# rkhosrowshahi/MO-VAE

Hardware: AMD Instinct MI355X
Metric: training images/sec (higher is better)
Workload: dtype f32

## Files before the change

include/movae.h:

```cpp
#ifndef MOVAE_H
#define MOVAE_H

#include <stddef.h>
#include <stdint.h>

#ifdef __cplusplus
extern "C" {
#endif

typedef void* movae_stream_t;

enum movae_act { MOVAE_ACT_NONE = 0, MOVAE_ACT_LRELU = 1, MOVAE_ACT_RELU = 2, MOVAE_ACT_TANH = 3, MOVAE_ACT_SIGMOID = 4 };
enum movae_recon { MOVAE_RECON_MSE = 0, MOVAE_RECON_BCE = 1, MOVAE_RECON_L1 = 2, MOVAE_RECON_SMOOTH_L1 = 3 };
enum movae_mgda_norm { MOVAE_MGDA_NONE = 0, MOVAE_MGDA_L2 = 1, MOVAE_MGDA_LOSS = 2, MOVAE_MGDA_LOSS_PLUS = 3 };
enum movae_upgrad_norm { MOVAE_UPGRAD_TRACE = 0, MOVAE_UPGRAD_MIN_L2 = 1, MOVAE_UPGRAD_COSINE = 2 };
enum movae_amtl_scale { MOVAE_AMTL_MIN = 0, MOVAE_AMTL_MEDIAN = 1, MOVAE_AMTL_RMSE = 2 };

int movae_version(void);
const char* movae_last_error(void);

int movae_nchw_to_nhwc(const float* src, float* dst, int n, int c, int h, int w, movae_stream_t stream);
int movae_nhwc_to_nchw(const float* src, float* dst, int n, int c, int h, int w, movae_stream_t stream);

int movae_conv2d_fwd(const float* x, const float* w, const float* bias, float* y,
                     int n, int hi, int wi, int ci, int ho, int wo, int co, int kh, int kw, int stride, int pad,
                     int act, float slope, void* ws, size_t ws_bytes, movae_stream_t stream);
int movae_conv2d_dgrad(const float* dy, const float* w, float* dx,
                       int n, int hi, int wi, int ci, int ho, int wo, int co, int kh, int kw, int stride, int pad,
                       void* ws, size_t ws_bytes, movae_stream_t stream);
int movae_conv2d_wgrad(const float* dy, const float* x, float* dw, float* dbias,
                       int n, int hi, int wi, int ci, int ho, int wo, int co, int kh, int kw, int stride, int pad,
                       int accumulate, void* ws, size_t ws_bytes, movae_stream_t stream);
int movae_conv2d_wgrad_grouped(int groups, const float* dy, const float* x, float* const* dw, float* const* dbias,
                               int n, int hi, int wi, int ci, int ho, int wo, int co, int kh, int kw, int stride, int pad,
                               int accumulate, void* ws, size_t ws_bytes, movae_stream_t stream);
int movae_convT2d_fwd(const float* x, const float* w, const float* bias, float* y,
                      int n, int hi, int wi, int ci, int ho, int wo, int co, int kh, int kw, int stride, int pad,
                      int act, float slope, void* ws, size_t ws_bytes, movae_stream_t stream);
int movae_convT2d_dgrad(const float* dy, const float* w, float* dx,
                        int n, int hi, int wi, int ci, int ho, int wo, int co, int kh, int kw, int stride, int pad,
                        void* ws, size_t ws_bytes, movae_stream_t stream);
int movae_convT2d_wgrad(const float* dy, const float* x, float* dw, float* dbias,
                        int n, int hi, int wi, int ci, int ho, int wo, int co, int kh, int kw, int stride, int pad,
                        int accumulate, void* ws, size_t ws_bytes, movae_stream_t stream);
int movae_conv2d_dgrad_wgrad_grouped(int groups, const float* dy, const float* w, const float* x, float* dx, float* const* dw,
                                     float* const* dbias, int n, int hi, int wi, int ci, int ho, int wo, int co, int kh, int kw,
                                     int stride, int pad, int accumulate, void* ws, size_t ws_bytes, movae_stream_t stream);
int movae_convT2d_dgrad_wgrad_grouped(int groups, const float* dy, const float* w, const float* x, float* dx, float* const* dw,
                                      float* const* dbias, int n, int hi, int wi, int ci, int ho, int wo, int co, int kh, int kw,
                                      int stride, int pad, int accumulate, void* ws, size_t ws_bytes, movae_stream_t stream);
int movae_convT2d_wgrad_grouped(int groups, const float* dy, const float* x, float* const* dw, float* const* dbias,
                                int n, int hi, int wi, int ci, int ho, int wo, int co, int kh, int kw, int stride, int pad,
                                int accumulate, void* ws, size_t ws_bytes, movae_stream_t stream);
int movae_linear_pair_fwd(const float* x, const float* w1, const float* b1, const float* w2, const float* b2, float* y1, float* y2,
                          int m, int n, int k, movae_stream_t stream);
int movae_linear_pair_bwd(int groups, const float* dy1, const float* dy2, const float* w1, const float* w2, const float* x, float* dx,
                          float* const* dw1, float* const* dw2, float* const* db1, float* const* db2, int m, int n, int k,
                          movae_stream_t stream);

size_t movae_bn_ws_bytes(int rows, int c);
int movae_bn_act_fwd(const float* y, const float* gamma, const float* beta, float* out,
                     float* save_mean, float* save_rstd, float* running_mean, float* running_var,
                     long long* num_batches_tracked,
                     int rows, int c, float eps, float momentum, int training, int act, float slope,
                     void* ws, size_t ws_bytes, movae_stream_t stream);
int movae_bn_act_bwd(const float* dout, const float* y, const float* gamma, const float* beta,
                     const float* save_mean, const float* save_rstd, float* dy, float* dgamma, float* dbeta,
                     int rows, int c, int act, float slope, int accumulate,
                     void* ws, size_t ws_bytes, movae_stream_t stream);

int movae_bn_act_bwd_grouped(int groups, const float* dout, const float* y, const float* gamma, const float* beta,
                             const float* save_mean, const float* save_rstd, float* dy,
                             float* const* dgamma, float* const* dbeta,
                             int rows, int c, int act, float slope, int accumulate,
                             void* ws, size_t ws_bytes, movae_stream_t stream);

int movae_act_fwd(const float* x, float* y, size_t n, int act, float slope, movae_stream_t stream);
int movae_act_bwd(const float* dy, const float* out, float* dx, size_t n, int act, float slope, movae_stream_t stream);
int movae_act_bwd_bias_grouped(int groups, const float* dy, const float* out, float* dpre, float* const* dbias,
                               int rows, int c, int act, float slope, int accumulate,
                               void* ws, size_t ws_bytes, movae_stream_t stream);
int movae_add(const float* a, const float* b, float* y, size_t n, movae_stream_t stream);
int movae_axpby(float alpha, const float* a, float beta, const float* b, float* y, size_t n, movae_stream_t stream);
int movae_copy_channels(const float* src, float* dst, int rows, int c_src, int c_dst, int src_off, int dst_off, int c_copy, movae_stream_t stream);
int movae_colsum(const float* x, float* out, int rows, int c, int accumulate, void* ws, size_t ws_bytes, movae_stream_t stream);

int movae_reparam_fwd(const float* mu, const float* log_var, const float* eps, float* z, size_t n, movae_stream_t stream);
int movae_reparam_rng_fwd(const float* mu, const float* log_var, float* eps, float* z, size_t n, unsigned long long* state, int advance,
                          movae_stream_t stream);
int movae_reparam_prior_rng_fwd(const float* mu, const float* log_var, float* eps, float* z, size_t n, float* prior, size_t n_prior,
                                unsigned long long* state, int advance, movae_stream_t stream);
int movae_reparam_bwd(const float* dz, const float* log_var, const float* eps, float* dmu, float* dlog_var, size_t n, movae_stream_t stream);

size_t movae_reduce_ws_bytes(size_t n);
int movae_recon_loss_fwd(const float* recons, const float* inputs, float* out, size_t n, int kind, float scale,
                         void* ws, size_t ws_bytes, movae_stream_t stream);
int movae_recon_loss_bwd(const float* recons, const float* inputs, const float* gscale_dev, float* drecons,
                         size_t n, int kind, float scale, movae_stream_t stream);
int movae_recon_loss_bwd_act(const float* recons, const float* inputs, const float* gscale_dev, float* dpre, size_t n, int kind,
                             float scale, int act, float slope, movae_stream_t stream);
int movae_kl_fwd(const float* mu, const float* log_var, float* out, int b, int d, float scale,
                 void* ws, size_t ws_bytes, movae_stream_t stream);
int movae_combine_losses_fwd(int nterms, const float* const* terms, int nout, const float* coef, float* iter_dev, float anneal_steps,
                             int anneal_row, int training, float* out, float* anneal_out, movae_stream_t stream);
int movae_combine_losses_bwd(int nterms, int nout, const float* const* g, const float* coef, const float* anneal_dev, int anneal_row,
                             float* gterms, movae_stream_t stream);
int movae_vae_losses_fwd(const float* recons, const float* inputs, size_t n, int kind, float rec_scale,
                         const float* mu, const float* log_var, int b, int d, float kl_scale, float* out,
                         void* ws, size_t ws_bytes, movae_stream_t stream);
int movae_recursive_losses_fwd(const float* recons, const float* inputs, size_t n, int kind, const float* mu_hat, const float* log_var_hat,
                               const float* z_prior, const float* mu_gen, int b, int d, float w_rec, float w_kl, float w_cyc,
                               float* iter_dev, float anneal_host, float anneal_steps, int training, float* out, float* anneal_out,
                               void* ws, size_t ws_bytes, movae_stream_t stream);
int movae_recursive_losses_bwd(const float* recons, const float* inputs, size_t n, int kind, const float* mu_hat, const float* log_var_hat,
                               const float* z_prior, const float* mu_gen, int b, int d, float w_rec, float w_kl, float w_cyc,
                               const float* anneal_dev, const float* g_rec, const float* g_kl, const float* g_cyc, const float* g_tot,
                               float* drecons, float* dmu_hat, float* dlog_var_hat, float* dmu_gen, movae_stream_t stream);
int movae_sphere_latents_fwd(const float* z, float* e, float* u, const float* sigma_in, int sigma_rows, float sigma_val, int fixed_sigma,
                             unsigned long long* state, int advance, int b, int l, float angle_max_deg, float mix_prob, float mix_min_deg,
                             float mix_max_deg, float radius, float eps, float* v, float* v_noisy, float* v_noisy_small, float* sigma,
                             float* sigma_sub, float* inv_rms, movae_stream_t stream);
int movae_sphere_latents_bwd(const float* v, const float* e, const float* sigma, const float* sigma_sub, const float* inv_rms,
                             const float* g_v, const float* g_noisy, const float* g_small, float* dz, int b, int l, float radius,
                             movae_stream_t stream);
size_t movae_sphere_losses_ws_bytes(size_t n, int b);
int movae_sphere_losses_fwd(const float* recons, const float* inputs, const float* x_noisy, const float* recons_sg, size_t n, const float* v,
                            const float* v_enc_dec, int b, int l, float lam_rec, float w_rec_sl1, float lam_con, float w_con_sl1,
                            float lam_lat, float* out, void* ws, size_t ws_bytes, movae_stream_t stream);
int movae_sphere_losses_bwd(const float* recons, const float* inputs, const float* x_noisy, const float* recons_sg, size_t n, const float* v,
                            const float* v_enc_dec, int b, int l, float lam_rec, float w_rec_sl1, float lam_con, float w_con_sl1,
                            float lam_lat, const float* g_rec, const float* g_con, const float* g_lat, const float* g_tot, float* drecons,
                            float* dx_noisy, float* dv, float* dv_enc_dec, movae_stream_t stream);
int movae_kl_bwd(const float* mu, const float* log_var, const float* gscale_dev, float* dmu, float* dlog_var,
                 int b, int d, float scale, movae_stream_t stream);
int movae_tc_decomp_fwd(const float* z, const float* mu, const float* log_var, const float* log_iw, float* out,
                        float* lse_joint, float* lse_marg, int b, int d, void* ws, size_t ws_bytes, movae_stream_t stream);
int movae_tc_decomp_bwd(const float* z, const float* mu, const float* log_var, const float* log_iw,
                        const float* lse_joint, const float* lse_marg, const float* g,
                        float* dz, float* dmu, float* dlog_var, int b, int d, movae_stream_t stream);

enum movae_edge_match {
    MOVAE_EDGE_MAG = 0, MOVAE_EDGE_SIGNED_MSE = 1, MOVAE_EDGE_MAXNORM = 2, MOVAE_EDGE_ANGLE = 3, MOVAE_EDGE_MASKED = 4,
    MOVAE_EDGE_COSINE = 5
};
int movae_edge_weights(const float* inputs, float* w_raw, float* wmax, int n, int h, int w, int c,
                       void* ws, size_t ws_bytes, movae_stream_t stream);
int movae_edge_weighted_mse_fwd(const float* recons, const float* inputs, const float* w_raw, const float* wmax, float* out,
                                int n, int h, int w, int c, float scale, void* ws, size_t ws_bytes, movae_stream_t stream);
int movae_edge_weighted_mse_bwd(const float* recons, const float* inputs, const float* w_raw, const float* wmax,
                                const float* gscale_dev, float* drecons, int n, int h, int w, int c, float scale,
                                movae_stream_t stream);
int movae_edge_match_fwd(const float* recons, const float* inputs, float* out, int n, int h, int w, int c, float scale,
                         int mode, float* stats, void* ws, size_t ws_bytes, movae_stream_t stream);
int movae_edge_match_bwd(const float* recons, const float* inputs, const float* gscale_dev, float* drecons, float* tmp_a,
                         float* tmp_b, int n, int h, int w, int c, float scale, int mode, const float* stats,
                         movae_stream_t stream);

int movae_vq_nearest_fwd(const float* x, const float* e, float* q, int64_t* idx, float* sse, int32_t* used_count,
                         int rows, int k, int d, void* ws, size_t ws_bytes, movae_stream_t stream);
int movae_vq_nearest_fwd_mse(const float* x, const float* e, float* q, int64_t* idx, float* sse, int32_t* used_count, float* mse2,
                             int rows, int k, int d, void* ws, size_t ws_bytes, movae_stream_t stream);
size_t movae_vq_bwd_ws_bytes(int rows, int k, int d);
int movae_vq_bwd(const float* x, const float* q, const int64_t* idx, const float* dq, const float* gc, const float* ge,
                 float* dx, float* de, int rows, int k, int d, void* ws, size_t ws_bytes, movae_stream_t stream);

#define MOVAE_MAX_K 8
size_t movae_gram_ws_bytes(int k, size_t m);
int movae_gram(const float* J, size_t ldj, int k, size_t m, float* G, void* ws, size_t ws_bytes, movae_stream_t stream);
int movae_weights_upgrad(const float* G, int k, float norm_eps, float reg_eps, const float* pref, float* w, movae_stream_t stream);
int movae_weights_upgrad_norm(const float* G, int k, int norm_mode, float norm_eps, float reg_eps, const float* pref, float* w,
                              movae_stream_t stream);
int movae_gram_upgrad(const float* J, size_t ldj, int k, size_t m, float* G, int norm_mode, float norm_eps, float reg_eps,
                      const float* pref, float* w, int dual, void* ws, size_t ws_bytes, movae_stream_t stream);
int movae_weights_mgda(const float* G, int k, int norm, const float* losses, float epsilon, int max_iters,
                       float* w, int32_t* info, movae_stream_t stream);
int movae_weights_mgda_stable(const float* G, int k, int norm, const float* losses, float epsilon, int max_iters,
                              float min_eigenvalue, float* w, int32_t* info, movae_stream_t stream);
int movae_weights_amtl(const float* G, int k, int scale_mode, const float* pref, float* w, movae_stream_t stream);
int movae_weights_dualproj(const float* G, int k, float norm_eps, float reg_eps, const float* pref, float* w, movae_stream_t stream);
int movae_weights_pcgrad(const float* G, int k, const int32_t* perm, float* w, movae_stream_t stream);
int movae_weights_imtlg(const float* G, int k, float* w, movae_stream_t stream);
int movae_weights_cagrad(const float* G, int k, float c, float norm_eps, float* w, movae_stream_t stream);
int movae_weights_const(int k, float value, float* w, movae_stream_t stream);
int movae_combine(const float* J, size_t ldj, int k, size_t m, const float* w, float* g, int accumulate, movae_stream_t stream);
int movae_gd_similarity(const float* J, size_t ldj, int k, size_t m, const float* w, float* out,
                        void* ws, size_t ws_bytes, movae_stream_t stream);

int movae_adam_step(float* p, const float* g, float* m, float* v, size_t n, float lr, float beta1, float beta2,
                    float eps, float weight_decay, int decoupled_wd, int step, movae_stream_t stream);
int movae_adam_multi(int n_tensors, float* const* p, const float* const* g, float* const* m, float* const* v,
                     const size_t* numel, float lr, float beta1, float beta2, float eps, float weight_decay,
                     int decoupled_wd, int step, float* hyper_dev, movae_stream_t stream);
int movae_clip_grad_norm_multi(int n_tensors, float* const* g, const size_t* numel, float max_norm, float* total_sumsq_dev,
                               void* ws, size_t ws_bytes, movae_stream_t stream);
int movae_sumsq(const float* x, size_t n, float* out, void* ws, size_t ws_bytes, movae_stream_t stream);
int movae_scale_by_clip(float* g, size_t n, const float* sumsq_dev, float max_norm, movae_stream_t stream);

#define MOVAE_DTYPE_F32 0
#define MOVAE_DTYPE_BF16 1
int movae_set_compute_dtype(int dtype);

int movae_reduce_defer(int on);
int movae_reduce_flush(void);
int movae_reduce_defer_stats(long long* out3, int reset);
long long movae_reduce_defer_max_bytes(long long bytes);

int movae_bench_main_kernel_only(int on);
const char* movae_bench_last_kernel(void);
int movae_bench_force_split(int s);
int movae_bench_kgemm_bn_fin(int mode);
int movae_bench_force_kgemm(int mode);
int movae_bench_big_tile_min(int n);

typedef struct movae_fuse {
    const float* in_scale;
    const float* in_shift;
    float in_slope;
    float* stats;
    size_t stats_cap;
    int stats_parts;
    const float* bn_y;
    const float* bn_scale;
    const float* bn_shift;
    float bn_slope;
    float* bn_part;
    size_t bn_cap;
    int bn_ppg;
    const float* ep_act_y;
    int ep_act;
    float ep_slope;
    int ep_act_done;
    const float* ep_res;
    const float* fin_gamma;
    const float* fin_beta;
    float fin_eps;
    float fin_momentum;
    float* fin_out;
    float* fin_running_mean;
    float* fin_running_var;
    long long* fin_nbt;
    int fin_done;
} movae_fuse_t;
int movae_conv2d_fwd_f(const float* x, const float* w, const float* bias, float* y,
                       int n, int hi, int wi, int ci, int ho, int wo, int co, int kh, int kw, int stride, int pad,
                       int act, float slope, void* ws, size_t ws_bytes, movae_stream_t stream, movae_fuse_t* fuse);
int movae_convT2d_fwd_f(const float* x, const float* w, const float* bias, float* y,
                        int n, int hi, int wi, int ci, int ho, int wo, int co, int kh, int kw, int stride, int pad,
                        int act, float slope, void* ws, size_t ws_bytes, movae_stream_t stream, movae_fuse_t* fuse);
int movae_conv2d_wgrad_grouped_f(int groups, const float* dy, const float* x, float* const* dw, float* const* dbias,
                                 int n, int hi, int wi, int ci, int ho, int wo, int co, int kh, int kw, int stride, int pad,
                                 int accumulate, void* ws, size_t ws_bytes, movae_stream_t stream, const movae_fuse_t* fuse);
int movae_convT2d_wgrad_grouped_f(int groups, const float* dy, const float* x, float* const* dw, float* const* dbias,
                                  int n, int hi, int wi, int ci, int ho, int wo, int co, int kh, int kw, int stride, int pad,
                                  int accumulate, void* ws, size_t ws_bytes, movae_stream_t stream, const movae_fuse_t* fuse);
int movae_conv2d_dgrad_wgrad_grouped_f(int groups, const float* dy, const float* w, const float* x, float* dx,
                                       float* const* dw, float* const* dbias,
                                       int n, int hi, int wi, int ci, int ho, int wo, int co, int kh, int kw, int stride, int pad,
                                       int accumulate, void* ws, size_t ws_bytes, movae_stream_t stream, const movae_fuse_t* fuse);
int movae_convT2d_dgrad_wgrad_grouped_f(int groups, const float* dy, const float* w, const float* x, float* dx,
                                        float* const* dw, float* const* dbias,
                                        int n, int hi, int wi, int ci, int ho, int wo, int co, int kh, int kw, int stride, int pad,
                                        int accumulate, void* ws, size_t ws_bytes, movae_stream_t stream, const movae_fuse_t* fuse);
int movae_conv2d_dgrad_f(const float* dy, const float* w, float* dx,
                         int n, int hi, int wi, int ci, int ho, int wo, int co, int kh, int kw, int stride, int pad,
                         void* ws, size_t ws_bytes, movae_stream_t stream, movae_fuse_t* fuse, int groups);
int movae_convT2d_dgrad_f(const float* dy, const float* w, float* dx,
                          int n, int hi, int wi, int ci, int ho, int wo, int co, int kh, int kw, int stride, int pad,
                          void* ws, size_t ws_bytes, movae_stream_t stream, movae_fuse_t* fuse, int groups);
int movae_bn_bwd_finalize(const float* bn_part, size_t bn_cap, int ppg, int groups, int rows, int c, const float* gamma,
                          const float* save_mean, const float* save_rstd, float* const* dgamma, float* const* dbeta, float* coef,
                          int accumulate, movae_stream_t stream);
int movae_bn_bwd_apply(const float* dout, const float* y, const float* scale, const float* shift, float slope, const float* coef,
                       float* dy, int groups, size_t rows, int c, movae_stream_t stream);
int movae_bn_bwd_finalize_apply(const float* bn_part, size_t bn_cap, int ppg, int groups, size_t rows, int c, const float* gamma,
                                const float* save_mean, const float* save_rstd, float* const* dgamma, float* const* dbeta, float* coef,
                                int accumulate, const float* dout, const float* y, const float* scale, const float* shift, float slope,
                                float* dy, movae_stream_t stream);
int movae_bn_finalize(const float* stats, size_t stats_cap, int parts, int rows, int c, const float* gamma, const float* beta, float eps,
                      float momentum, float* save_mean, float* save_rstd, float* scale, float* shift, float* running_mean,
                      float* running_var, long long* num_batches_tracked, movae_stream_t stream);
int movae_bn_stats(const float* y, int rows, int c, float* stats, size_t stats_cap, int* parts_out, movae_stream_t stream);
int movae_scale_shift_act(const float* y, const float* scale, const float* shift, float* out, size_t rows, int c, float slope,
                          movae_stream_t stream);

int movae_embedding_fwd(const float* weight, const int64_t* idx, float* y, size_t rows, int k, int d, movae_stream_t stream);
int movae_embedding_bwd(const float* dy, const int64_t* idx, float* dweight, int rows, int k, int d,
                        void* ws, size_t ws_bytes, movae_stream_t stream);
int movae_gated_residual_fwd(const float* res, const float* gate, const float* feat, float* out, size_t n, movae_stream_t stream);
int movae_gated_residual_bwd(const float* dout, const float* gate, const float* feat, float* dgate, float* dfeat, size_t n,
                             movae_stream_t stream);
int movae_mul(const float* a, const float* b, float* y, size_t n, movae_stream_t stream);
size_t movae_cross_entropy_ws_bytes(size_t rows);
int movae_cross_entropy_fwd(const float* logits, const int64_t* target, float* loss, float* lse, size_t rows, int k,
                            void* ws, size_t ws_bytes, movae_stream_t stream);
int movae_cross_entropy_bwd(const float* logits, const int64_t* target, const float* lse, const float* gscale_dev, float* dlogits,
                            size_t rows, int k, movae_stream_t stream);

int movae_causal_attn_fwd(const float* q, const float* k, const float* v, long ld, float* out, float* lse, int B, int heads, int L,
                          int hd, float p, unsigned long long seed, unsigned long long draw, movae_stream_t stream);
size_t movae_causal_attn_ws_bytes(int B, int heads, int L);
int movae_causal_attn_bwd(const float* q, const float* k, const float* v, long ld, const float* out, const float* dout, const float* lse,
                          float* dq, float* dk, float* dv, int B, int heads, int L, int hd, float p, unsigned long long seed,
                          unsigned long long draw, void* ws, size_t ws_bytes, movae_stream_t stream);
int movae_causal_attn_dropout_mask(uint8_t* keep, int BH, int L, float p, unsigned long long seed, unsigned long long draw,
                                   movae_stream_t stream);

int movae_attn_fwd(const float* q, const float* k, const float* v, long ld, const float* rope_cos, const float* rope_sin, float* out,
                   float* lse, int B, int heads, int L, int hd, float p, movae_stream_t stream);
size_t movae_attn_ws_bytes(int B, int heads, int L);
int movae_attn_bwd(const float* q, const float* k, const float* v, long ld, const float* rope_cos, const float* rope_sin, const float* out,
                   const float* dout, const float* lse, float* dq, float* dk, float* dv, int B, int heads, int L, int hd, float p, void* ws,
                   size_t ws_bytes, movae_stream_t stream);

int movae_rownorm_fwd(const float* x, const float* weight, const float* bias, const float* pos, int pos_rows, float* out, float* mean,
                      float* rstd, long rows, int d, int mode, float eps, movae_stream_t stream);
size_t movae_rownorm_ws_bytes(long rows, int d);
int movae_rownorm_bwd(const float* dy, const float* x, const float* weight, const float* mean, const float* rstd, float* dx, float* dweight,
                      float* dbias, long rows, int d, int mode, void* ws, size_t ws_bytes, movae_stream_t stream);
int movae_bias_gelu_fwd(const float* x, const float* bias, float* y, long rows, int c, movae_stream_t stream);
int movae_bias_gelu_bwd(const float* dy, const float* x, const float* bias, float* dx, long rows, int c, movae_stream_t stream);
int movae_unpatchify_act_fwd(const float* x, float* out, int b, int h, int w, int c, int patch, movae_stream_t stream);
int movae_unpatchify_act_bwd(const float* dout, const float* out, float* dx, int b, int h, int w, int c, int patch, movae_stream_t stream);
int movae_add_rows_bcast(const float* x, const float* pos, float* y, long rows, int pos_rows, int d, movae_stream_t stream);

size_t movae_recon_metrics_ws_bytes(int n, int c, int h, int w);
int movae_recon_metrics(const float* real, long long rs_n, long long rs_c, long long rs_h, long long rs_w,
                        const float* recon, long long ps_n, long long ps_c, long long ps_h, long long ps_w,
                        int n, int c, int h, int w, int window_size, float max_val, float* out, void* ws, size_t ws_bytes,
                        movae_stream_t stream);

size_t movae_vgg_prep_ws_bytes(int g);
int movae_vgg_prep_fwd(int g, const float* const* x, float* const* y, int* flags, size_t n, void* ws, size_t ws_bytes,
                       movae_stream_t stream);
int movae_vgg_prep_bwd(int g, const float* const* dy, const float* const* x, const int* flags, float* const* dx, size_t n,
                       movae_stream_t stream);
int movae_maxpool2x2_fwd(const float* x, float* y, int n, int h, int w, int c, movae_stream_t stream);
int movae_maxpool2x2_bwd(const float* dy, const float* x, const float* y, float* dx, int n, int h, int w, int c, movae_stream_t stream);

size_t movae_lpips_ws_bytes(int n, int h, int w, int c);
int movae_lpips_layer(const float* f1, const float* f2, int n, int h, int w, int c, float scale, double* partials,
                      size_t partials_bytes, movae_stream_t stream);
int movae_lpips_finalize(int layers, const double* const* partials, const int* h, const int* w, const int* c, int n, float* out,
                         movae_stream_t stream);

int movae_batch_u8(const uint8_t* store, const int* idx, int b, int h, int w, int c, const float* lut, int flip,
// ... 7 lines not shown
```

mo-vae_amd/_lib.py:

```python
import ctypes as C
import os
import threading

import torch

HERE = os.path.dirname(os.path.abspath(__file__))
LIB_PATH = os.path.join(HERE, "libmovae_hip.so")

ACT = {"none": 0, None: 0, "lrelu": 1, "relu": 2, "tanh": 3, "sigmoid": 4}
RECON = {"mse": 0, "bce": 1, "l1": 2, "smooth_l1": 3}
UPGRAD_NORM = {"trace": 0, "min_l2": 1, "cosine": 2}
EDGE_MATCH = {"mag": 0, "signed_mse": 1, "maxnorm": 2, "angle": 3, "masked": 4, "cosine": 5}
MGDA_NORM = {"none": 0, "l2": 1, "loss": 2, "loss+": 3}
AMTL_SCALE = {"min": 0, "median": 1, "rmse": 2}
MAX_K = 8

_p, _i, _f, _z, _l = C.c_void_p, C.c_int, C.c_float, C.c_size_t, C.c_long

class MovaeFuse(C.Structure):
    _fields_ = [("in_scale", C.c_void_p), ("in_shift", C.c_void_p), ("in_slope", C.c_float), ("stats", C.c_void_p),
                ("stats_cap", C.c_size_t), ("stats_parts", C.c_int),
                ("bn_y", C.c_void_p), ("bn_scale", C.c_void_p), ("bn_shift", C.c_void_p), ("bn_slope", C.c_float), ("bn_part", C.c_void_p),
                ("bn_cap", C.c_size_t), ("bn_ppg", C.c_int),
                ("ep_act_y", C.c_void_p), ("ep_act", C.c_int), ("ep_slope", C.c_float), ("ep_act_done", C.c_int),
                ("ep_res", C.c_void_p),
                ("fin_gamma", C.c_void_p), ("fin_beta", C.c_void_p), ("fin_eps", C.c_float), ("fin_momentum", C.c_float),
                ("fin_out", C.c_void_p), ("fin_running_mean", C.c_void_p), ("fin_running_var", C.c_void_p), ("fin_nbt", C.c_void_p),
                ("fin_done", C.c_int)]


_conv_fwd = [_p, _p, _p, _p] + [_i] * 11 + [_i, _f, _p, _z, _p]
_conv_dgrad = [_p, _p, _p] + [_i] * 11 + [_p, _z, _p]
_conv_wgrad = [_p, _p, _p, _p] + [_i] * 11 + [_i, _p, _z, _p]

SIGNATURES = {
    "movae_version": ([], _i),
    "movae_last_error": ([], C.c_char_p),
    "movae_nchw_to_nhwc": ([_p, _p, _i, _i, _i, _i, _p], _i),
    "movae_nhwc_to_nchw": ([_p, _p, _i, _i, _i, _i, _p], _i),
    "movae_conv2d_fwd": (_conv_fwd, _i),
    "movae_conv2d_dgrad": (_conv_dgrad, _i),
    "movae_conv2d_wgrad": (_conv_wgrad, _i),
    "movae_convT2d_fwd": (_conv_fwd, _i),
    "movae_convT2d_dgrad": (_conv_dgrad, _i),
    "movae_convT2d_wgrad": (_conv_wgrad, _i),
    "movae_conv2d_wgrad_grouped": ([_i] + _conv_wgrad, _i),
    "movae_convT2d_wgrad_grouped": ([_i] + _conv_wgrad, _i),
    "movae_conv2d_dgrad_wgrad_grouped": ([_i, _p, _p, _p, _p, _p, _p] + [_i] * 11 + [_i, _p, _z, _p], _i),
    "movae_convT2d_dgrad_wgrad_grouped": ([_i, _p, _p, _p, _p, _p, _p] + [_i] * 11 + [_i, _p, _z, _p], _i),
    "movae_bn_ws_bytes": ([_i, _i], _z),
    "movae_bn_act_fwd": ([_p] * 9 + [_i, _i, _f, _f, _i, _i, _f, _p, _z, _p], _i),
    "movae_bn_act_bwd": ([_p] * 9 + [_i, _i, _i, _f, _i, _p, _z, _p], _i),
    "movae_bn_act_bwd_grouped": ([_i] + [_p] * 9 + [_i, _i, _i, _f, _i, _p, _z, _p], _i),
    "movae_act_fwd": ([_p, _p, _z, _i, _f, _p], _i),
    "movae_act_bwd": ([_p, _p, _p, _z, _i, _f, _p], _i),
    "movae_act_bwd_bias_grouped": ([_i, _p, _p, _p, _p, _i, _i, _i, _f, _i, _p, _z, _p], _i),
    "movae_add": ([_p, _p, _p, _z, _p], _i),
    "movae_axpby": ([_f, _p, _f, _p, _p, _z, _p], _i),
    "movae_copy_channels": ([_p, _p, _i, _i, _i, _i, _i, _i, _p], _i),
    "movae_colsum": ([_p, _p, _i, _i, _i, _p, _z, _p], _i),
    "movae_reparam_fwd": ([_p, _p, _p, _p, _z, _p], _i),
    "movae_reparam_rng_fwd": ([_p, _p, _p, _p, _z, _p, _i, _p], _i),
    "movae_reparam_bwd": ([_p, _p, _p, _p, _p, _z, _p], _i),
    "movae_reparam_prior_rng_fwd": ([_p, _p, _p, _p, _z, _p, _z, _p, _i, _p], _i),
    "movae_reduce_ws_bytes": ([_z], _z),
    "movae_recon_loss_fwd": ([_p, _p, _p, _z, _i, _f, _p, _z, _p], _i),
    "movae_recon_loss_bwd": ([_p, _p, _p, _p, _z, _i, _f, _p], _i),
    "movae_recon_loss_bwd_act": ([_p, _p, _p, _p, _z, _i, _f, _i, _f, _p], _i),
    "movae_kl_fwd": ([_p, _p, _p, _i, _i, _f, _p, _z, _p], _i),
    "movae_combine_losses_fwd": ([_i, _p, _i, _p, _p, _f, _i, _i, _p, _p, _p], _i),
    "movae_combine_losses_bwd": ([_i, _i, _p, _p, _p, _i, _p, _p], _i),
    "movae_vae_losses_fwd": ([_p, _p, _z, _i, _f, _p, _p, _i, _i, _f, _p, _p, _z, _p], _i),
    "movae_kl_bwd": ([_p, _p, _p, _p, _p, _i, _i, _f, _p], _i),
    "movae_recursive_losses_fwd": ([_p, _p, _z, _i, _p, _p, _p, _p, _i, _i, _f, _f, _f, _p, _f, _f, _i, _p, _p, _p, _z, _p], _i),
    "movae_recursive_losses_bwd": ([_p, _p, _z, _i, _p, _p, _p, _p, _i, _i, _f, _f, _f] + [_p] * 9 + [_p], _i),
    "movae_sphere_latents_fwd": ([_p, _p, _p, _p, _i, _f, _i, _p, _i, _i, _i, _f, _f, _f, _f, _f, _f] + [_p] * 6 + [_p], _i),
    "movae_sphere_latents_bwd": ([_p] * 9 + [_i, _i, _f, _p], _i),
    "movae_sphere_losses_ws_bytes": ([_z, _i], _z),
    "movae_sphere_losses_fwd": ([_p, _p, _p, _p, _z, _p, _p, _i, _i, _f, _f, _f, _f, _f, _p, _p, _z, _p], _i),
    "movae_sphere_losses_bwd": ([_p, _p, _p, _p, _z, _p, _p, _i, _i, _f, _f, _f, _f, _f] + [_p] * 8 + [_p], _i),
    "movae_tc_decomp_fwd": ([_p] * 7 + [_i, _i, _p, _z, _p], _i),
    "movae_tc_decomp_bwd": ([_p] * 10 + [_i, _i, _p], _i),
    "movae_edge_weights": ([_p, _p, _p, _i, _i, _i, _i, _p, _z, _p], _i),
    "movae_edge_weighted_mse_fwd": ([_p, _p, _p, _p, _p, _i, _i, _i, _i, _f, _p, _z, _p], _i),
    "movae_edge_weighted_mse_bwd": ([_p, _p, _p, _p, _p, _p, _i, _i, _i, _i, _f, _p], _i),
    "movae_edge_match_fwd": ([_p, _p, _p, _i, _i, _i, _i, _f, _i, _p, _p, _z, _p], _i),
    "movae_edge_match_bwd": ([_p, _p, _p, _p, _p, _p, _i, _i, _i, _i, _f, _i, _p, _p], _i),
    "movae_vq_nearest_fwd": ([_p] * 6 + [_i, _i, _i, _p, _z, _p], _i),
    "movae_vq_nearest_fwd_mse": ([_p] * 7 + [_i, _i, _i, _p, _z, _p], _i),
    "movae_vq_bwd_ws_bytes": ([_i, _i, _i], _z),
    "movae_vq_bwd": ([_p] * 8 + [_i, _i, _i, _p, _z, _p], _i),
    "movae_gram_ws_bytes": ([_i, _z], _z),
    "movae_gram": ([_p, _z, _i, _z, _p, _p, _z, _p], _i),
    "movae_weights_upgrad": ([_p, _i, _f, _f, _p, _p, _p], _i),
    "movae_weights_upgrad_norm": ([_p, _i, _i, _f, _f, _p, _p, _p], _i),
    "movae_gram_upgrad": ([_p, _z, _i, _z, _p, _i, _f, _f, _p, _p, _i, _p, _z, _p], _i),
    "movae_weights_mgda": ([_p, _i, _i, _p, _f, _i, _p, _p, _p], _i),
    "movae_weights_mgda_stable": ([_p, _i, _i, _p, _f, _i, _f, _p, _p, _p], _i),
    "movae_weights_amtl": ([_p, _i, _i, _p, _p, _p], _i),
    "movae_weights_dualproj": ([_p, _i, _f, _f, _p, _p, _p], _i),
    "movae_weights_pcgrad": ([_p, _i, _p, _p, _p], _i),
    "movae_weights_imtlg": ([_p, _i, _p, _p], _i),
    "movae_weights_cagrad": ([_p, _i, _f, _f, _p, _p], _i),
    "movae_weights_const": ([_i, _f, _p, _p], _i),
    "movae_combine": ([_p, _z, _i, _z, _p, _p, _i, _p], _i),
    "movae_gd_similarity": ([_p, _z, _i, _z, _p, _p, _p, _z, _p], _i),
    "movae_adam_step": ([_p, _p, _p, _p, _z, _f, _f, _f, _f, _f, _i, _i, _p], _i),
    "movae_adam_multi": ([_i, _p, _p, _p, _p, _p, _f, _f, _f, _f, _f, _i, _i, _p, _p], _i),
    "movae_clip_grad_norm_multi": ([_i, _p, _p, _f, _p, _p, _z, _p], _i),
    "movae_sumsq": ([_p, _z, _p, _p, _z, _p], _i),
    "movae_scale_by_clip": ([_p, _z, _p, _f, _p], _i),
    "movae_conv2d_fwd_f": (_conv_fwd + [_p], _i),
    "movae_convT2d_fwd_f": (_conv_fwd + [_p], _i),
    "movae_conv2d_wgrad_grouped_f": ([_i] + _conv_wgrad + [_p], _i),
    "movae_convT2d_wgrad_grouped_f": ([_i] + _conv_wgrad + [_p], _i),
    "movae_conv2d_dgrad_wgrad_grouped_f": ([_i, _p, _p, _p, _p, _p, _p] + [_i] * 11 + [_i, _p, _z, _p, _p], _i),
    "movae_convT2d_dgrad_wgrad_grouped_f": ([_i, _p, _p, _p, _p, _p, _p] + [_i] * 11 + [_i, _p, _z, _p, _p], _i),
    "movae_conv2d_dgrad_f": (_conv_dgrad + [_p, _i], _i),
    "movae_convT2d_dgrad_f": (_conv_dgrad + [_p, _i], _i),
    "movae_bn_bwd_finalize": ([_p, _z, _i, _i, _i, _i, _p, _p, _p, _p, _p, _p, _i, _p], _i),
    "movae_bn_bwd_apply": ([_p, _p, _p, _p, _f, _p, _p, _i, _z, _i, _p], _i),
    "movae_linear_pair_fwd": ([_p, _p, _p, _p, _p, _p, _p, _i, _i, _i, _p], _i),
    "movae_linear_pair_bwd": ([_i, _p, _p, _p, _p, _p, _p, _p, _p, _p, _p, _i, _i, _i, _p], _i),
    "movae_bn_bwd_finalize_apply": ([_p, _z, _i, _i, _z, _i, _p, _p, _p, _p, _p, _p, _i, _p, _p, _p, _p, _f, _p, _p], _i),
    "movae_bn_finalize": ([_p, _z, _i, _i, _i, _p, _p, _f, _f, _p, _p, _p, _p, _p, _p, _p, _p], _i),
    "movae_bn_stats": ([_p, _i, _i, _p, _z, _p, _p], _i),
    "movae_scale_shift_act": ([_p, _p, _p, _p, _z, _i, _f, _p], _i),
    "movae_embedding_fwd": ([_p, _p, _p, _z, _i, _i, _p], _i),
    "movae_embedding_bwd": ([_p, _p, _p, _i, _i, _i, _p, _z, _p], _i),
    "movae_gated_residual_fwd": ([_p, _p, _p, _p, _z, _p], _i),
    "movae_gated_residual_bwd": ([_p, _p, _p, _p, _p, _z, _p], _i),
    "movae_mul": ([_p, _p, _p, _z, _p], _i),
    "movae_cross_entropy_ws_bytes": ([_z], _z),
    "movae_cross_entropy_fwd": ([_p, _p, _p, _p, _z, _i, _p, _z, _p], _i),
    "movae_cross_entropy_bwd": ([_p, _p, _p, _p, _p, _z, _i, _p], _i),
    "movae_causal_attn_fwd": ([_p, _p, _p, _l, _p, _p, _i, _i, _i, _i, _f, C.c_ulonglong, C.c_ulonglong, _p], _i),
    "movae_causal_attn_ws_bytes": ([_i, _i, _i], _z),
    "movae_causal_attn_bwd": ([_p, _p, _p, _l, _p, _p, _p, _p, _p, _p, _i, _i, _i, _i, _f, C.c_ulonglong, C.c_ulonglong, _p, _z, _p], _i),
    "movae_causal_attn_dropout_mask": ([_p, _i, _i, _f, C.c_ulonglong, C.c_ulonglong, _p], _i),
    "movae_attn_fwd": ([_p, _p, _p, _l, _p, _p, _p, _p, _i, _i, _i, _i, _f, _p], _i),
    "movae_attn_ws_bytes": ([_i, _i, _i], _z),
    "movae_attn_bwd": ([_p, _p, _p, _l, _p, _p, _p, _p, _p, _p, _p, _p, _i, _i, _i, _i, _f, _p, _z, _p], _i),
    "movae_rownorm_fwd": ([_p, _p, _p, _p, _i, _p, _p, _p, _l, _i, _i, _f, _p], _i),
    "movae_rownorm_ws_bytes": ([_l, _i], _z),
    "movae_rownorm_bwd": ([_p, _p, _p, _p, _p, _p, _p, _p, _l, _i, _i, _p, _z, _p], _i),
    "movae_bias_gelu_fwd": ([_p, _p, _p, _l, _i, _p], _i),
    "movae_bias_gelu_bwd": ([_p, _p, _p, _p, _l, _i, _p], _i),
    "movae_unpatchify_act_fwd": ([_p, _p, _i, _i, _i, _i, _i, _p], _i),
    "movae_unpatchify_act_bwd": ([_p, _p, _p, _i, _i, _i, _i, _i, _p], _i),
    "movae_add_rows_bcast": ([_p, _p, _p, _l, _i, _i, _p], _i),
    "movae_vgg_prep_ws_bytes": ([_i], _z),
    "movae_vgg_prep_fwd": ([_i, _p, _p, _p, _z, _p, _z, _p], _i),
    "movae_vgg_prep_bwd": ([_i, _p, _p, _p, _p, _z, _p], _i),
    "movae_maxpool2x2_fwd": ([_p, _p, _i, _i, _i, _i, _p], _i),
    "movae_maxpool2x2_bwd": ([_p, _p, _p, _p, _i, _i, _i, _i, _p], _i),
    "movae_recon_metrics_ws_bytes": ([_i, _i, _i, _i], _z),
    "movae_recon_metrics": ([_p, C.c_longlong, C.c_longlong, C.c_longlong, C.c_longlong, _p, C.c_longlong, C.c_longlong, C.c_longlong,
                             C.c_longlong, _i, _i, _i, _i, _i, _f, _p, _p, _z, _p], _i),
    "movae_lpips_ws_bytes": ([_i, _i, _i, _i], _z),
    "movae_lpips_layer": ([_p, _p, _i, _i, _i, _i, _f, _p, _z, _p], _i),
    "movae_lpips_finalize": ([_i, _p, _p, _p, _p, _i, _p, _p], _i),
    "movae_batch_u8": ([_p, _p, _i, _i, _i, _i, _p, _i, C.c_ulonglong, C.c_ulonglong, _p, _p], _i),
    "movae_bench_main_kernel_only": ([_i], _i),
    "movae_bench_last_kernel": ([], C.c_char_p),
    "movae_reduce_defer": ([_i], _i),
    "movae_reduce_flush": ([], _i),
    "movae_reduce_defer_stats": ([_p, _i], _i),
    "movae_reduce_defer_max_bytes": ([C.c_longlong], C.c_longlong),
    "movae_bench_force_split": ([_i], _i),
    "movae_bench_kgemm_bn_fin": ([_i], _i),
    "movae_bench_force_kgemm": ([_i], _i),
    "movae_bench_big_tile_min": ([_i], _i),
    "movae_set_compute_dtype": ([_i], _i),
}

_lib = None
_lock = threading.Lock()


def load():
    global _lib
    if _lib is not None:
        return _lib
    with _lock:
        if _lib is not None:
            return _lib
        from . import build as _build

        have_hipcc = False
        try:
            _build._hipcc()
            have_hipcc = os.path.isdir(_build.CSRC)
        except RuntimeError:
            pass
        if have_hipcc and os.environ.get("MOVAE_NO_REBUILD") != "1":
            try:
                _build.build(verbose=False)
            except Exception as e:
                if not os.path.exists(LIB_PATH):
                    raise RuntimeError(
                        f"libmovae_hip.so is missing at {LIB_PATH} and could not be built ({e}); "
                        "the MI355X kernels are required -- there is no CPU fallback") from e
                raise RuntimeError(f"csrc/ changed but rebuilding libmovae_hip.so failed: {e}") from e
        elif not os.path.exists(LIB_PATH):
            raise RuntimeError(f"libmovae_hip.so is missing at {LIB_PATH} and hipcc is not available to build it; "
                               "the MI355X kernels are required -- there is no CPU fallback")
        try:
            lib = C.CDLL(LIB_PATH)
        except OSError as e:
            raise RuntimeError(f"cannot load {LIB_PATH}: {e}; the MI355X kernels are required") from e
        for name, (args, res) in SIGNATURES.items():
            fn = getattr(lib, name)
            fn.argtypes = args
            fn.restype = res
        _lib = lib
    return _lib


DTYPES = {"fp32": 0, "f32": 0, "float32": 0, "bf16": 1, "bfloat16": 1}


def set_compute_dtype(name):
    if name not in DTYPES:
        raise ValueError(f"compute dtype must be one of {sorted(set(DTYPES))}, got {name!r}")
    prev = load().movae_set_compute_dtype(DTYPES[name])
    return "bf16" if prev == 1 else "fp32"


def compute_dtype():
    lib = load()
    prev = lib.movae_set_compute_dtype(DTYPES["fp32"])
    lib.movae_set_compute_dtype(prev)
    return "bf16" if prev == 1 else "fp32"


TRACE = None

DEFER_ON = [False]
DEFER_PASS = frozenset(
    [f"movae_conv{t}2d_{k}" for t in ("", "T") for k in ("dgrad", "dgrad_f", "wgrad_grouped", "wgrad_grouped_f", "dgrad_wgrad_grouped",
                                                       "dgrad_wgrad_grouped_f")] +
    ["movae_bn_bwd_finalize", "movae_bn_bwd_apply", "movae_bn_bwd_finalize_apply", "movae_bn_act_bwd", "movae_bn_act_bwd_grouped",
     "movae_act_bwd", "movae_act_bwd_bias_grouped", "movae_colsum", "movae_add", "movae_axpby", "movae_copy_channels", "movae_mul",
     "movae_nchw_to_nhwc", "movae_nhwc_to_nchw", "movae_reparam_bwd", "movae_kl_bwd", "movae_recon_loss_bwd", "movae_recon_loss_bwd_act", "movae_recursive_losses_bwd",
     "movae_tc_decomp_bwd", "movae_sphere_latents_bwd", "movae_sphere_losses_bwd",
     "movae_combine_losses_bwd", "movae_vq_bwd", "movae_linear_pair_bwd", "movae_edge_weighted_mse_bwd", "movae_edge_match_bwd",
     "movae_gated_residual_bwd", "movae_attn_bwd", "movae_rownorm_bwd", "movae_bias_gelu_bwd", "movae_unpatchify_act_bwd",
     "movae_vgg_prep_bwd", "movae_maxpool2x2_bwd"])
_defer_arena = [0]


def defer_arm(device):
    _defer_arena[0] ^= 1
    w = workspace(device, slot=2 + _defer_arena[0])
    load().movae_reduce_defer(1)
    return w.data_ptr(), w.numel()


def defer_flush():
    if _lib is not None:
        check(load().movae_reduce_flush(), "movae_reduce_flush")
# ... 49 lines not shown
```

mo-vae_amd/aggregation.py:

```python
import os

import torch
import torch.nn as tnn

from . import _lib as L


def _st(t):
    return L.stream_ptr(t.device)


def _check_matrix(J):
    if J.dim() != 2:
        raise ValueError(f"Parameter `matrix` should be a tensor of dimension 2. Found `matrix.shape = {tuple(J.shape)}`.")
    if J.shape[0] > L.MAX_K:
        raise ValueError(f"at most {L.MAX_K} objectives are supported on device, got {J.shape[0]}")
    L.require_gpu(J)
    if J.dtype != torch.float32 or J.stride(1) != 1:
        raise ValueError("the Jacobian must be fp32 with unit column stride")


FUSE_GRAM = os.environ.get("MOVAE_FUSE_GRAM", "1") != "0"


def compute_gramian(J):
    _check_matrix(J)
    k, m = J.shape
    G = torch.empty((k, k), dtype=torch.float32, device=J.device)
    ws = L.workspace(J.device)
    L.call("movae_gram", J.data_ptr(), J.stride(0) if k > 1 else max(J.stride(0), m), k, m, G.data_ptr(),
                                ws.data_ptr(), ws.numel(), _st(J))
    return G


def combine(J, w):
    _check_matrix(J)
    k, m = J.shape
    g = torch.empty(m, dtype=torch.float32, device=J.device)
    L.call("movae_combine", J.data_ptr(), J.stride(0) if k > 1 else max(J.stride(0), m), k, m, w.data_ptr(),
                                   g.data_ptr(), 0, _st(J))
    return g


def gd_similarity(J, w):
    _check_matrix(J)
    k, m = J.shape
    out = torch.empty((), dtype=torch.float32, device=J.device)
    ws = L.workspace(J.device)
    L.call("movae_gd_similarity", J.data_ptr(), J.stride(0) if k > 1 else max(J.stride(0), m), k, m, w.data_ptr(),
                                         out.data_ptr(), ws.data_ptr(), ws.numel(), _st(J))
    return out


def _pref_tensor(pref, device):
    if pref is None:
        return None
    return torch.as_tensor(pref, dtype=torch.float32).to(device).contiguous()


class Weighting(tnn.Module):

    def forward(self, gramian):
        raise NotImplementedError


class _FromJacobian(tnn.Module):

    def __init__(self, gramian_weighting):
        super().__init__()
        self.gramian_weighting = gramian_weighting

    def forward(self, J):
        gw = self.gramian_weighting
        fused = getattr(gw, "from_jacobian", None)
        if fused is not None and FUSE_GRAM and not gw._forward_hooks and not gw._forward_pre_hooks:
            self.last_gramian, w = fused(J)
            return w
        self.last_gramian = compute_gramian(J)
        return gw(self.last_gramian)


class GramianWeightedAggregator(tnn.Module):
    def __init__(self, gramian_weighting):
        super().__init__()
        self.gramian_weighting = gramian_weighting
        self.weighting = _FromJacobian(gramian_weighting)

    def forward(self, J):
        w = self.weighting(J)
        return combine(J, w)


class UPGradWeighting(Weighting):

    def __init__(self, pref_vector=None, norm_eps=1e-4, reg_eps=1e-4, norm="trace"):
        super().__init__()
        self.pref_vector, self.norm_eps, self.reg_eps, self.norm = pref_vector, norm_eps, reg_eps, norm

    def _mode(self):
        return self.norm

    def forward(self, G):
        k = G.shape[0]
        w = torch.empty(k, dtype=torch.float32, device=G.device)
        pref = _pref_tensor(self.pref_vector, G.device)
        L.call("movae_weights_upgrad_norm", G.data_ptr(), k, L.UPGRAD_NORM[self._mode()], float(self.norm_eps),
               float(self.reg_eps), L.ptr(pref), w.data_ptr(), _st(G))
        return w

    def from_jacobian(self, J):
        _check_matrix(J)
        k, m = J.shape
        G = torch.empty((k, k), dtype=torch.float32, device=J.device)
        w = torch.empty(k, dtype=torch.float32, device=J.device)
        pref = _pref_tensor(self.pref_vector, J.device)
        ws = L.workspace(J.device)
        L.call("movae_gram_upgrad", J.data_ptr(), J.stride(0) if k > 1 else max(J.stride(0), m), k, m, G.data_ptr(),
               L.UPGRAD_NORM[self._mode()], float(self.norm_eps), float(self.reg_eps), L.ptr(pref), w.data_ptr(), 0, ws.data_ptr(),
               ws.numel(), _st(J))
        return G, w


class _PNUPGradWeighting(UPGradWeighting):

    def __init__(self, pref_vector=None, prob=0.5, norm_eps=1e-4, reg_eps=1e-4):
        super().__init__(pref_vector, norm_eps, reg_eps, norm="min_l2")
        self.prob = prob

    def _mode(self):
        return "cosine" if torch.rand(1).item() < self.prob else "min_l2"


class UPGrad(GramianWeightedAggregator):

    def __init__(self, pref_vector=None, norm_eps=0.0001, reg_eps=0.0001, solver="quadprog"):
        super().__init__(UPGradWeighting(pref_vector, norm_eps, reg_eps))
        self._pref_vector, self._norm_eps, self._reg_eps = pref_vector, norm_eps, reg_eps

    def __repr__(self):
        return f"UPGrad(pref_vector={self._pref_vector!r}, norm_eps={self._norm_eps}, reg_eps={self._reg_eps})"


class NUPGrad(GramianWeightedAggregator):

    def __init__(self, pref_vector=None, norm_eps=0.0001, reg_eps=0.0001, solver="quadprog"):
        super().__init__(UPGradWeighting(pref_vector, norm_eps, reg_eps, norm="min_l2"))
        self._pref_vector, self._norm_eps, self._reg_eps = pref_vector, norm_eps, reg_eps

    def __repr__(self):
        return f"NUPGrad(pref_vector={self._pref_vector!r}, norm_eps={self._norm_eps}, reg_eps={self._reg_eps}, solver='quadprog')"


class PNUPGrad(GramianWeightedAggregator):

    def __init__(self, pref_vector=None, prob=0.5, norm_eps=0.0001, reg_eps=0.0001, solver="quadprog"):
        super().__init__(_PNUPGradWeighting(pref_vector, prob, norm_eps, reg_eps))
        self._pref_vector, self._prob, self._norm_eps, self._reg_eps = pref_vector, prob, norm_eps, reg_eps

    def __repr__(self):
        return (f"PNUPGrad(pref_vector={self._pref_vector!r}, prob={self._prob}, norm_eps={self._norm_eps}, "
                f"reg_eps={self._reg_eps}, solver='quadprog')")


class MGDAWeighting(Weighting):
    def __init__(self, norm_type="none", epsilon=1e-5, max_iters=250, stable=False, min_eigenvalue_eps=1e-10):
        super().__init__()
        if norm_type not in ("none", "l2", "loss", "loss+"):
            raise ValueError("Parameter `norm_type` should be 'none', 'l2', 'loss', or 'loss+'. Found "
                             f"`norm_type = {norm_type!r}`.")
        self.norm_type, self.epsilon, self.max_iters = norm_type, epsilon, max_iters
        self.stable, self.min_eigenvalue_eps = stable, min_eigenvalue_eps
        self._losses = None
        self._info = None

    def set_losses(self, losses):
        if losses.dim() != 1:
            raise ValueError(f"Parameter `losses` should be a 1D tensor. Found `losses.shape = {losses.shape}`.")
        self._losses = losses.detach()

    @property
    def convergence_count(self):
        return None if self._info is None else int(self._info.item())

    def forward(self, G):
        k = G.shape[0]
        losses = None
        if self.norm_type in ("loss", "loss+"):
            if self._losses is None:
                raise RuntimeError(f"Losses must be set before calling forward() when using norm_type='{self.norm_type}'. "
                                   "Call set_losses() first.")
            if self._losses.shape[0] != k:
                raise ValueError(f"Number of losses ({self._losses.shape[0]}) must match the number of rows in the gramian ({k}).")
            losses = self._losses.to(device=G.device, dtype=torch.float32).contiguous()
        w = torch.empty(k, dtype=torch.float32, device=G.device)
        self._info = torch.empty(1, dtype=torch.int32, device=G.device)
        if self.stable:
            L.call("movae_weights_mgda_stable", G.data_ptr(), k, L.MGDA_NORM[self.norm_type], L.ptr(losses), float(self.epsilon),
                   int(self.max_iters), float(self.min_eigenvalue_eps), w.data_ptr(), self._info.data_ptr(), _st(G))
        else:
            L.call("movae_weights_mgda", G.data_ptr(), k, L.MGDA_NORM[self.norm_type], L.ptr(losses), float(self.epsilon),
                   int(self.max_iters), w.data_ptr(), self._info.data_ptr(), _st(G))
        return w


class StableMGDA(GramianWeightedAggregator):

    def __init__(self, norm_type="none", epsilon=1e-5, max_iters=250, min_eigenvalue_eps=1e-10):
        w = MGDAWeighting(norm_type, epsilon, max_iters, True, min_eigenvalue_eps)
        super().__init__(w)
        self._mgda_weighting = w

    @property
    def mgda_weighting(self):
        return self._mgda_weighting

    def set_losses(self, losses):
        self._mgda_weighting.set_losses(losses)


class MGDA(GramianWeightedAggregator):
    def __init__(self, norm_type="none", epsilon=1e-5, max_iters=250, stable=False, min_eigenvalue_eps=1e-10):
        w = MGDAWeighting(norm_type, epsilon, max_iters, stable, min_eigenvalue_eps)
        super().__init__(w)
        self._mgda_weighting = w
        self._norm_type, self._epsilon, self._max_iters, self._stable = norm_type, epsilon, max_iters, stable

    @property
    def mgda_weighting(self):
        return self._mgda_weighting

    def set_losses(self, losses):
        self._mgda_weighting.set_losses(losses)

    def __repr__(self):
        return (f"MGDA(norm_type={self._norm_type!r}, epsilon={self._epsilon}, max_iters={self._max_iters}, "
                f"stable={self._stable})")


class AlignedMTLWeighting(Weighting):
    def __init__(self, pref_vector=None, scale_mode="min"):
        super().__init__()
        self._pref_vector, self._scale_mode = pref_vector, scale_mode

# ... 220 lines not shown
```

mo-vae_amd/autojac.py:

```python
import os

import torch

from . import ops

BATCHED_VJP = os.environ.get("MOVAE_BATCHED_VJP", "1") != "0"


def _leaf_tensors(roots, excluded=()):
    stop = {t.grad_fn for t in excluded if t.grad_fn is not None}
    seen, leaves, stack = set(), [], [t.grad_fn for t in roots if t.grad_fn is not None]
    while stack:
        fn = stack.pop()
        if fn is None or fn in seen or fn in stop:
            continue
        seen.add(fn)
        var = getattr(fn, "variable", None)
        if var is not None:
            if var.requires_grad:
                leaves.append(var)
            continue
        stack.extend(nf for nf, _ in fn.next_functions)
    out, ids = [], set()
    for v in leaves:
# ... 110 lines not shown
                self.copied.add(dst.data_ptr())
                if g.data_ptr() != dst.data_ptr():
                    dst.copy_(_mem_flat(g))


def _group(t, g):
    return None if t is None else t[g]


def _dense(t):
    if t.is_contiguous():
        return True
    order = sorted(range(t.dim()), key=lambda i: (-t.stride(i), -t.shape[i]))
    return t.permute(order).is_contiguous()


def _restack(lst):
    t0 = lst[0]
    if not isinstance(t0, torch.Tensor) or t0.numel() == 0 or not _dense(t0):
        return lst
    nbytes = t0.numel() * t0.element_size()
    base = t0.untyped_storage().data_ptr()
    for g, t in enumerate(lst):
        if (not isinstance(t, torch.Tensor) or t.shape != t0.shape or t.dtype != t0.dtype or t.stride() != t0.stride() or
                t.untyped_storage().data_ptr() != base or t.data_ptr() != t0.data_ptr() + g * nbytes):
            return lst
    return t0.as_strided((len(lst),) + tuple(t0.shape), (t0.numel(),) + tuple(t0.stride()), t0.storage_offset())


def _accumulate_stacked(a, b, G):
    if a is None:
        return b
    if isinstance(a, (list, tuple)) or isinstance(b, (list, tuple)):
        return [a[g] + b[g] for g in range(G)]
    return a + b


def _expected_shape(node, input_nr):
    var = getattr(node, "variable", None)
    if var is not None:
        return tuple(var.shape)
    meta = getattr(node, "_input_metadata", None)
    if meta is not None and input_nr < len(meta):
        return tuple(meta[input_nr].shape)
    return None


def _fit_groups(t, shape, G):
    if shape is None:
        return t
    if isinstance(t, (list, tuple)):
        return [x if x is None or tuple(x.shape) == shape else x.sum_to_size(shape) for x in t]
    if tuple(t.shape[1:]) == shape:
        return t
    return [t[g].sum_to_size(shape) for g in range(G)]


@torch.no_grad()
def _batched_pullback(features, feat_grads, rows, jb):
    G = len(rows)
    roots = []
    for f, feat in enumerate(features):
        fn = feat.grad_fn
        if fn is None:
            continue
        gs = [feat_grads[g][f] for g in range(G)]
        if all(x is None for x in gs):
            continue
        ref = next(x for x in gs if x is not None)
        gs = [x if x is not None else torch.zeros_like(ref) for x in gs]
        roots.append((fn, feat.output_nr, _restack(gs)))
    deps, seen, stack = {}, set(), [fn for fn, _, _ in roots]
    while stack:
        fn = stack.pop()
        if fn in seen:
            continue
        seen.add(fn)
        for nf, _ in fn.next_functions:
            if nf is not None:
                deps[nf] = deps.get(nf, 0) + 1
                stack.append(nf)
    pending = {}
    for fn, nr, gs in roots:
        slot = pending.setdefault(fn, {})
        slot[nr] = _accumulate_stacked(slot.get(nr), gs, G)
    ready = [fn for fn in {r[0] for r in roots} if deps.get(fn, 0) == 0]
    col = {id(p): (p, off) for p, off in zip(jb.params, jb.offsets)}
    ops.GRAD_SINK_ROWS = [jb.sinks(r) for r in rows]
    try:
        while ready:
            fn = ready.pop()
            got = pending.pop(fn, {})
            var = getattr(fn, "variable", None)
            outs = None
            if var is not None:
                ent = col.get(id(var))
                if ent is not None and 0 in got:
                    p, off = ent
                    for g in range(G):
                        src = _group(got[0], g)
                        dst = jb.buf[rows[g]][off: off + p.numel()]
                        jb.copied.add(dst.data_ptr())
                        if src.data_ptr() != dst.data_ptr():
                            dst.copy_(_mem_flat(src))
                continue
            edges = list(fn.next_functions)
            if got:
                n_in = max(got) + 1
                args = [got.get(i) for i in range(n_in)]
                cls = getattr(fn, "_forward_cls", None)
                if cls is not None:
                    args += [None] * (len(getattr(fn, "_input_metadata", ())) - len(args))
                    if hasattr(cls, "backward_batched"):
                        outs = cls.backward_batched(fn, G, *args)
                    else:
                        per = []
                        for g in range(G):
                            r = cls.backward(fn, *[_group(a, g) for a in args])
                            per.append(r if isinstance(r, tuple) else (r,))
                        outs = tuple(None if all(per[g][i] is None for g in range(G)) else [per[g][i] for g in range(G)]
                                     for i in range(len(per[0])))
                    if not isinstance(outs, tuple):
                        outs = (outs,)
                    need = [i for i, nd in enumerate(fn.needs_input_grad) if nd]
                    live = [j for j, (nf, _) in enumerate(edges) if nf is not None]
                    if len(need) != len(live):
                        raise NotImplementedError("cannot align backward outputs with graph edges")
                    aligned = [None] * len(edges)
                    for j, i in zip(live, need):
                        aligned[j] = outs[i] if i < len(outs) else None
                    outs = tuple(aligned)
                else:
                    per = []
                    for g in range(G):
                        r = fn(*[_group(a, g) for a in args])
                        per.append(r if isinstance(r, tuple) else (r,))
                    outs = tuple(None if all(per[g][i] is None for g in range(G)) else _restack([per[g][i] for g in range(G)])
                                 for i in range(len(per[0])))
            for i, (nf, nr) in enumerate(edges):
                if nf is None:
                    continue
                o = outs[i] if outs is not None and i < len(outs) else None
                if o is not None:
                    o = _fit_groups(o, _expected_shape(nf, nr), G)
                    slot = pending.setdefault(nf, {})
                    slot[nr] = _accumulate_stacked(slot.get(nr), o, G)
                deps[nf] -= 1
                if deps[nf] == 0:
                    ready.append(nf)
    finally:
        ops.GRAD_SINK_ROWS = None


def _aggregate_into_grads(jb, aggregator):
    g = aggregator(jb.J)
    for p, off in zip(jb.params, jb.offsets):
        _accumulate(p, _view_like(g[off: off + p.numel()], p))
    return g


class _MtlState:
    __slots__ = ("jb", "feat_diff", "feat_grads", "shared_params", "aggregator", "task_params", "device")


def mtl_backward_begin(losses, features, aggregator, tasks_params=None, shared_params=None):
    losses, features = list(losses), list(features)
    if len(losses) == 0:
        raise ValueError("`losses` cannot be empty")
    if len(features) == 0:
        raise ValueError("`features` cannot be empty.")
    if shared_params is None:
        shared_params = _leaf_tensors(features)
    if tasks_params is None:
        tasks_params = [_leaf_tensors([l], excluded=features) for l in losses]
    if len(tasks_params) != len(losses):
        raise ValueError("`losses` and `tasks_params` should have the same size.")
    st = _MtlState()
    st.shared_params = list(shared_params)
    st.aggregator = aggregator
    st.jb = JacobianBuffer.persistent(st.shared_params, len(losses), features[0].device)
    st.feat_diff = [f for f in features if f.requires_grad]
    st.feat_grads = []
    st.task_params = []
    cot = [torch.empty_strided((len(losses),) + tuple(f.shape), (f.numel(),) + tuple(f.stride()), dtype=f.dtype, device=f.device)
           if _dense(f) else None for f in st.feat_diff]
    for i, (loss, tp) in enumerate(zip(losses, tasks_params)):
        tp = list(tp)
        seed = _ones_like(loss) if loss.dim() == 0 and loss.dtype == torch.float32 else None
        ops.GRAD_ACCUM.clear()
        ops.GRAD_ACCUM_TAKEN.clear()
        if i > 0:
            ops.GRAD_ACCUM.update({p.data_ptr(): p.grad for p in tp if p.grad is not None})
        ops.COT_SINK.clear()
        ops.COT_SINK.update({f.data_ptr(): c[i] for f, c in zip(st.feat_diff, cot) if c is not None})
        ops.GRAD_SINK.clear()
        owned = {}
        for p in tp:
            if p.grad is None:
                buf = ops.GRAD_SINK[p.data_ptr()] = _task_grad_buffer(p)
                owned[buf.data_ptr()] = p
        n_w, n_z = len(ops.SINK_LOG), len(ops.SINK_ZERO_LOG)
        try:
            with ops.deferred_reduces():
                got = torch.autograd.grad(loss, tp + st.feat_diff, grad_outputs=seed, retain_graph=True, allow_unused=True)
        finally:
            for ptr in ops.SINK_LOG[n_w:]:
                if ptr in owned:
                    owned[ptr]._movae_grad_written = True
            for ptr in ops.SINK_ZERO_LOG[n_z:]:
                if ptr in owned and getattr(owned[ptr], "_movae_grad_written", False):
                    owned[ptr]._movae_grad_buf.zero_()
                    owned[ptr]._movae_grad_written = False
            ops.GRAD_SINK.clear()
            ops.COT_SINK.clear()
            ops.GRAD_ACCUM.clear()
            taken = frozenset(ops.GRAD_ACCUM_TAKEN)
            ops.GRAD_ACCUM_TAKEN.clear()
        for p, g in zip(tp, got[: len(tp)]):
            if g is not None:
                _accumulate(p, g, taken)
                st.task_params.append(p)
        st.feat_grads.append(got[len(tp):])
    return st


def _task_grad_buffer(p):
    buf = getattr(p, "_movae_grad_buf", None)
    if buf is None or buf.numel() != p.numel() or buf.device != p.device:
        buf = torch.zeros(p.numel(), dtype=p.dtype, device=p.device)
        p._movae_grad_buf, p._movae_grad_written = buf, False
    return buf


def mtl_backward_finish(st):
    with ops.deferred_reduces():
        return _mtl_backward_finish(st)


def _mtl_backward_finish(st):
    jb, feat_diff, feat_grads, shared_params = st.jb, st.feat_diff, st.feat_grads, st.shared_params
    live_rows = [i for i, gf in enumerate(feat_grads) if any(g is not None for g in gf)]
    batched = BATCHED_VJP and shared_params and len(live_rows) > 1
    if batched:
        try:
            _batched_pullback(feat_diff, [feat_grads[i] for i in live_rows], live_rows, jb)
        except NotImplementedError:
            batched = False
    for i in ([] if batched else live_rows):
        gf = feat_grads[i]
        live = [(f, g) for f, g in zip(feat_diff, gf) if g is not None]
        if not live or not shared_params:
            continue
        ops.GRAD_SINK.clear()
        ops.GRAD_SINK.update(jb.sinks(i))
        try:
            js = torch.autograd.grad([f for f, _ in live], shared_params, grad_outputs=[g for _, g in live],
                                     retain_graph=True, allow_unused=True)
        finally:
            ops.GRAD_SINK.clear()
        jb.write_row(i, js)
    if shared_params:
        jb.settle()
        _aggregate_into_grads(jb, st.aggregator)


def mtl_backward(losses, features, aggregator, tasks_params=None, shared_params=None, retain_graph=False,
                 parallel_chunk_size=None):
    st = mtl_backward_begin(losses, features, aggregator, tasks_params, shared_params)
    mtl_backward_finish(st)
    if not retain_graph:
        del st


def backward(tensors, aggregator, inputs=None, retain_graph=False, parallel_chunk_size=None):
    tensors = list(tensors) if isinstance(tensors, (list, tuple)) else [tensors]
    if len(tensors) == 0:
        raise ValueError("`tensors` cannot be empty")
    if inputs is None:
        inputs = _leaf_tensors(tensors)
    inputs = list(inputs)
    if not inputs:
        return
    jb = JacobianBuffer(inputs, len(tensors), tensors[0].device)
    for i, t in enumerate(tensors):
        js = torch.autograd.grad(t, inputs, retain_graph=True, allow_unused=True)
        jb.write_row(i, js)
    _aggregate_into_grads(jb, aggregator)


BATCHED_FULL_JACOBIAN = os.environ.get("MOVAE_BATCHED_FULL_JACOBIAN", "0") == "1"


def backward_through(tensors, aggregator, inputs=None):
    tensors = list(tensors)
    if len(tensors) == 0:
        raise ValueError("`tensors` cannot be empty")
    if inputs is None:
        inputs = _leaf_tensors(tensors)
    inputs = list(inputs)
    if not inputs:
        return
    K = len(tensors)
    jb = JacobianBuffer(inputs, K, tensors[0].device)
    node = tensors[0].grad_fn
    cls = getattr(node, "_forward_cls", None)
    done = False
    if (BATCHED_FULL_JACOBIAN and BATCHED_VJP and K > 1 and hasattr(cls, "input_cotangents")
# ... 13 lines not shown
```

mo-vae_amd/csrc/agg.hip:

```cpp
#include "common.h"
#include <stdlib.h>

namespace {

constexpr int MAXK = MOVAE_MAX_K;
inline int gram_blocks(size_t m) {
    static const size_t cap = (size_t)env_long("MOVAE_GRAM_BLOCKS", 1024);
    size_t g = (m + 2047) / 2048;
    return (int)(g > cap ? cap : (g < 1 ? 1 : g));
}

template <int K, bool VEC>
__global__ __launch_bounds__(256) void gram_partial(const float* __restrict__ J, long ldj, long m, double* __restrict__ part) {
    constexpr int NP = K * (K + 1) / 2;
    double acc[NP];
#pragma unroll
    for (int q = 0; q < NP; ++q) acc[q] = 0.0;
    const long stride = (long)gridDim.x * blockDim.x;
    if (VEC) {
        const long nv = m / 4;
        for (long c = (long)blockIdx.x * blockDim.x + threadIdx.x; c < nv; c += stride) {
            f32x4 v[K];
#pragma unroll
            for (int i = 0; i < K; ++i) v[i] = reinterpret_cast<const f32x4*>(J + i * ldj)[c];
            int q = 0;
#pragma unroll
            for (int i = 0; i < K; ++i)
#pragma unroll
                for (int j = i; j < K; ++j) {
                    const f32x4 p = v[i] * v[j];
                    acc[q] += (double)p[0] + (double)p[1] + (double)p[2] + (double)p[3];
                    ++q;
                }
        }
        if (blockIdx.x == 0 && threadIdx.x == 0)
            for (long c = nv * 4; c < m; ++c) {
                int q = 0;
                for (int i = 0; i < K; ++i)
                    for (int j = i; j < K; ++j) acc[q++] += (double)(J[i * ldj + c] * J[j * ldj + c]);
            }
    } else {
        for (long c = (long)blockIdx.x * blockDim.x + threadIdx.x; c < m; c += stride) {
            float v[K];
#pragma unroll
            for (int i = 0; i < K; ++i) v[i] = J[i * ldj + c];
            int q = 0;
#pragma unroll
            for (int i = 0; i < K; ++i)
#pragma unroll
                for (int j = i; j < K; ++j) acc[q++] += (double)(v[i] * v[j]);
        }
    }
    __shared__ double sh[4];
#pragma unroll
    for (int q = 0; q < NP; ++q) {
        const double s = block_sum_256(acc[q], sh);
        if (threadIdx.x == 0) part[(long)blockIdx.x * NP + q] = s;
    }
}

__global__ __launch_bounds__(64) void gram_final(const double* __restrict__ part, int nblk, int K, float* __restrict__ G) {
    const int NP = K * (K + 1) / 2;
    const int q = blockIdx.x;
    double s = 0.0;
    for (int b = threadIdx.x; b < nblk; b += 64) s += part[(long)b * NP + q];
    s = wave_sum(s);
    if (threadIdx.x != 0) return;
    int i = 0, rem = q;
    while (rem >= K - i) {
        rem -= K - i;
        ++i;
    }
    const int j = i + rem;
    G[i * K + j] = (float)s;
    G[j * K + i] = (float)s;
}

template <int K, bool VEC>
__global__ __launch_bounds__(256) void combine_k(const float* __restrict__ J, long ldj, long m, const float* __restrict__ w,
                                                 float* __restrict__ g, int accumulate) {
    float wv[K];
#pragma unroll
    for (int i = 0; i < K; ++i) wv[i] = w[i];
    const long stride = (long)gridDim.x * blockDim.x;
    if (VEC) {
        const long nv = m / 4;
        for (long c = (long)blockIdx.x * blockDim.x + threadIdx.x; c < nv; c += stride) {
            f32x4 s = accumulate ? reinterpret_cast<const f32x4*>(g)[c] : f32x4{0.f, 0.f, 0.f, 0.f};
#pragma unroll
            for (int i = 0; i < K; ++i) s += wv[i] * reinterpret_cast<const f32x4*>(J + i * ldj)[c];
            reinterpret_cast<f32x4*>(g)[c] = s;
        }
        if (blockIdx.x == 0 && threadIdx.x == 0)
            for (long c = nv * 4; c < m; ++c) {
                float s = accumulate ? g[c] : 0.f;
                for (int i = 0; i < K; ++i) s += wv[i] * J[i * ldj + c];
                g[c] = s;
            }
    } else {
        for (long c = (long)blockIdx.x * blockDim.x + threadIdx.x; c < m; c += stride) {
            float s = accumulate ? g[c] : 0.f;
#pragma unroll
            for (int i = 0; i < K; ++i) s += wv[i] * J[i * ldj + c];
            g[c] = s;
        }
    }
}

__global__ __launch_bounds__(256) void similarity_partial(const float* __restrict__ J, long ldj, int K, long m,
                                                          const float* __restrict__ w, double* __restrict__ part) {
    __shared__ double sh[4];
    double ab = 0.0, aa = 0.0, bb = 0.0;
    const long stride = (long)gridDim.x * blockDim.x;
    for (long c = (long)blockIdx.x * blockDim.x + threadIdx.x; c < m; c += stride) {
        float a = 0.f, b = 0.f;
        for (int i = 0; i < K; ++i) {
            const float v = J[i * ldj + c];
            a += w[i] * v;
            b += v;
        }
        b /= (float)K;
        ab += (double)a * b;
        aa += (double)a * a;
        bb += (double)b * b;
    }
    ab = block_sum_256(ab, sh);
    aa = block_sum_256(aa, sh);
    bb = block_sum_256(bb, sh);
    if (threadIdx.x == 0) {
        part[blockIdx.x * 3 + 0] = ab;
        part[blockIdx.x * 3 + 1] = aa;
        part[blockIdx.x * 3 + 2] = bb;
    }
}

__global__ void similarity_final(const double* __restrict__ part, int nblk, float* __restrict__ out) {
    if (threadIdx.x != 0) return;
    double ab = 0, aa = 0, bb = 0;
    for (int b = 0; b < nblk; ++b) {
        ab += part[b * 3];
        aa += part[b * 3 + 1];
        bb += part[b * 3 + 2];
    }
    const double na = fmax(sqrt(aa), 1e-8), nb = fmax(sqrt(bb), 1e-8);
    out[0] = (float)(ab / (na * nb));
}

template <int KT>
__global__ __launch_bounds__(64) void upgrad_k(const float* __restrict__ Gptr, int norm_mode, float norm_eps, float reg_eps,
                                               const float* __restrict__ pref, float* __restrict__ wout, int dual,
                                               const double* __restrict__ gpart, int gnb, float* __restrict__ Gout) {
    constexpr int K = KT;
    const int lane = threadIdx.x;
    float Gin[K * K];
    if (gpart) {
        constexpr int NP = K * (K + 1) / 2;
        int q = 0;
#pragma unroll
        for (int i = 0; i < K; ++i)
#pragma unroll
            for (int j = i; j < K; ++j, ++q) {
                double s = 0.0;
                for (int b = lane; b < gnb; b += 64) s += gpart[(long)b * NP + q];
                s = wave_sum(s);
                Gin[i * K + j] = Gin[j * K + i] = (float)s;
            }
        if (lane == 0 && Gout)
#pragma unroll
            for (int i = 0; i < K * K; ++i) Gout[i] = Gin[i];
    } else {
#pragma unroll
        for (int i = 0; i < K * K; ++i) Gin[i] = Gptr[i];
    }
    double G[K][K];
    if (norm_mode == 0) {
        double tr = 0.0;
#pragma unroll
        for (int i = 0; i < K; ++i) tr += (double)Gin[i * K + i];
        const bool zero = tr < (double)norm_eps;
#pragma unroll
        for (int i = 0; i < K; ++i)
#pragma unroll
            for (int j = 0; j < K; ++j) G[i][j] = zero ? 0.0 : (double)Gin[i * K + j] / tr;
    } else {
        float l2[K], sf[K];
        float amin = 0.f;
        bool any = false;
#pragma unroll
        for (int i = 0; i < K; ++i) {
            l2[i] = sqrtf(fmaxf(Gin[i * K + i], norm_eps));
            if (l2[i] > norm_eps && (!any || l2[i] < amin)) {
                amin = l2[i];
                any = true;
            }
        }
#pragma unroll
        for (int i = 0; i < K; ++i) sf[i] = (any && l2[i] > norm_eps) ? amin / l2[i] : 0.f;
#pragma unroll
        for (int i = 0; i < K; ++i)
#pragma unroll
            for (int j = 0; j < K; ++j) {
                const float g = Gin[i * K + j];
                G[i][j] = norm_mode == 1 ? (double)(g * (sf[i] * sf[j])) : (double)(g / (l2[i] * l2[j]));
            }
    }
#pragma unroll
    for (int i = 0; i < K; ++i) G[i][i] += (double)reg_eps;
    double u[K], wsum[K];
#pragma unroll
    for (int i = 0; i < K; ++i) {
        u[i] = pref ? (double)pref[i] : 1.0 / K;
        wsum[i] = 0.0;
    }
    constexpr int nsub = 1 << K;
    for (int row = 0; row < (dual ? 1 : K); ++row) {
        double c[K];
#pragma unroll
        for (int i = 0; i < K; ++i) {
            double acc = 0.0;
#pragma unroll
            for (int j = 0; j < K; ++j) acc += G[i][j] * ((dual || j == row) ? u[j] : 0.0);
            c[i] = acc;
        }
        double best_viol = 1e300;
        int best_mask = 0;
        double best_v[K];
#pragma unroll
        for (int i = 0; i < K; ++i) best_v[i] = 0.0;
        for (int mask = lane; mask < nsub; mask += 64) {
            double L[K][K], y[K], v[K];
            bool ok = true;
#pragma unroll
            for (int a = 0; a < K; ++a) {
                const bool fa = mask >> a & 1;
#pragma unroll
                for (int b = 0; b <= a; ++b) {
                    const bool fb = mask >> b & 1;
                    double s = (fa && fb) ? G[a][b] : (a == b ? 1.0 : 0.0);
#pragma unroll
                    for (int q = 0; q < b; ++q) s -= L[a][q] * L[b][q];
                    if (a == b) {
                        if (s <= 0.0) {
                            ok = false;
                            s = 1.0;
                        }
                        L[a][a] = sqrt(s);
                    } else {
                        L[a][b] = s / L[b][b];
                    }
                }
            }
#pragma unroll
            for (int a = 0; a < K; ++a) {
                double s = (mask >> a & 1) ? -c[a] : 0.0;
#pragma unroll
                for (int q = 0; q < a; ++q) s -= L[a][q] * y[q];
                y[a] = s / L[a][a];
            }
#pragma unroll
            for (int a = K - 1; a >= 0; --a) {
                double s = y[a];
#pragma unroll
                for (int q = a + 1; q < K; ++q) s -= L[q][a] * v[q];
                v[a] = s / L[a][a];
            }
            double viol = ok ? 0.0 : 1e200;
#pragma unroll
            for (int i = 0; i < K; ++i) {
                if (mask >> i & 1) {
                    viol = fmax(viol, -v[i]);
                } else {
                    v[i] = 0.0;
                    double gr = c[i];
#pragma unroll
                    for (int j = 0; j < K; ++j) gr += G[i][j] * ((mask >> j & 1) ? v[j] : 0.0);
                    viol = fmax(viol, -gr);
                }
            }
            if (viol < best_viol) {
                best_viol = viol;
                best_mask = mask;
#pragma unroll
                for (int i = 0; i < K; ++i) best_v[i] = v[i];
            }
        }
        for (int o = 32; o > 0; o >>= 1) {
            const double ov = __shfl_xor(best_viol, o, 64);
            const int om = __shfl_xor(best_mask, o, 64);
            double tmp[K];
#pragma unroll
            for (int i = 0; i < K; ++i) tmp[i] = __shfl_xor(best_v[i], o, 64);
            if (ov < best_viol || (ov == best_viol && om < best_mask)) {
                best_viol = ov;
                best_mask = om;
#pragma unroll
                for (int i = 0; i < K; ++i) best_v[i] = tmp[i];
            }
        }
#pragma unroll
        for (int i = 0; i < K; ++i) wsum[i] += best_v[i] + ((dual || i == row) ? u[i] : 0.0);
    }
    if (lane == 0)
#pragma unroll
        for (int i = 0; i < K; ++i) wout[i] = (float)wsum[i];
}

template <int KT>
__global__ __launch_bounds__(64) void cagrad_k(const float* __restrict__ Gin, float c, float norm_eps, float* __restrict__ wout) {
    constexpr int K = KT;
    const int lane = threadIdx.x;
    double G[K][K], b[K];
    double tr = 0.0, uGu = 0.0;
#pragma unroll
    for (int i = 0; i < K; ++i) {
#pragma unroll
        for (int j = 0; j < K; ++j) {
            G[i][j] = 0.5 * ((double)Gin[i * K + j] + (double)Gin[j * K + i]);
            uGu += G[i][j];
        }
        tr += G[i][i];
    }
    uGu /= (double)K * K;
    const double kappa = (double)c * sqrt(fmax(uGu, 0.0)), jitter = 1e-14 * tr;
#pragma unroll
    for (int i = 0; i < K; ++i) {
        double acc = 0.0;
#pragma unroll
        for (int j = 0; j < K; ++j) acc += G[i][j];
        b[i] = acc / K;
    }
    double best_viol = 1e300;
    int best_mask = 0;
    double best_w[K];
#pragma unroll
    for (int i = 0; i < K; ++i) best_w[i] = 0.0;
    for (int mask = lane + 1; mask < (1 << K); mask += 64) {
        double L[K][K], yp[K], yq[K], p[K], q[K], w[K];
        bool ok = true;
#pragma unroll
        for (int a = 0; a < K; ++a) {
            const bool fa = mask >> a & 1;
#pragma unroll
            for (int bb = 0; bb <= a; ++bb) {
                const bool fb = mask >> bb & 1;
                double s = (fa && fb) ? G[a][bb] + (a == bb ? jitter : 0.0) : (a == bb ? 1.0 : 0.0);
#pragma unroll
                for (int r = 0; r < bb; ++r) s -= L[a][r] * L[bb][r];
                if (a == bb) {
                    if (s <= 0.0) {
                        ok = false;
                        s = 1.0;
                    }
                    L[a][a] = sqrt(s);
                } else {
                    L[a][bb] = s / L[bb][bb];
                }
            }
        }
#pragma unroll
        for (int a = 0; a < K; ++a) {
            const bool fa = mask >> a & 1;
            double sp = fa ? 1.0 : 0.0, sq = fa ? b[a] : 0.0;
#pragma unroll
            for (int r = 0; r < a; ++r) {
                sp -= L[a][r] * yp[r];
                sq -= L[a][r] * yq[r];
            }
            yp[a] = sp / L[a][a];
            yq[a] = sq / L[a][a];
        }
#pragma unroll
        for (int a = K - 1; a >= 0; --a) {
            double sp = yp[a], sq = yq[a];
#pragma unroll
            for (int r = a + 1; r < K; ++r) {
                sp -= L[r][a] * p[r];
                sq -= L[r][a] * q[r];
            }
            p[a] = sp / L[a][a];
            q[a] = sq / L[a][a];
        }
        double A = 0.0, B = 0.0, C = 0.0;
#pragma unroll
        for (int i = 0; i < K; ++i)
            if (mask >> i & 1) {
                A += p[i];
                B += q[i];
                C += b[i] * q[i];
            }
        const double disc = B * B - A * (C - kappa * kappa);
        ok = ok && disc >= 0.0 && A > 0.0;
        const double lam = ok ? (B + sqrt(disc)) / A : 0.0, den = lam * A - B;
        ok = ok && den > 0.0;
#pragma unroll
        for (int i = 0; i < K; ++i) w[i] = (ok && (mask >> i & 1)) ? (lam * p[i] - q[i]) / den : 0.0;
        double Gw[K], wGw = 0.0;
#pragma unroll
        for (int i = 0; i < K; ++i) {
            double acc = 0.0;
#pragma unroll
            for (int j = 0; j < K; ++j) acc += G[i][j] * w[j];
            Gw[i] = acc;
            wGw += w[i] * acc;
        }
        const double t = sqrt(fmax(wGw, 0.0));
        ok = ok && t > 0.0;
        double viol = ok ? 0.0 : 1e200;
        if (ok) {
#pragma unroll
            for (int i = 0; i < K; ++i) {
                if (mask >> i & 1) viol = fmax(viol, -w[i]);
                else viol = fmax(viol, -(b[i] + kappa * Gw[i] / t - lam));
            }
        }
        if (viol < best_viol) {
            best_viol = viol;
            best_mask = mask;
#pragma unroll
            for (int i = 0; i < K; ++i) best_w[i] = w[i];
        }
    }
    for (int o = 32; o > 0; o >>= 1) {
        const double ov = __shfl_xor(best_viol, o, 64);
        const int om = __shfl_xor(best_mask, o, 64);
        double tmp[K];
#pragma unroll
        for (int i = 0; i < K; ++i) tmp[i] = __shfl_xor(best_w[i], o, 64);
        if (ov < best_viol || (ov == best_viol && om < best_mask)) {
            best_viol = ov;
            best_mask = om;
#pragma unroll
            for (int i = 0; i < K; ++i) best_w[i] = tmp[i];
        }
    }
    if (lane == 0) {
        double wGw = 0.0;
#pragma unroll
        for (int i = 0; i < K; ++i)
#pragma unroll
            for (int j = 0; j < K; ++j) wGw += best_w[i] * G[i][j] * best_w[j];
        const double gw = sqrt(fmax(wGw, 0.0));
        const bool mean = kappa <= (double)norm_eps || best_viol >= 1e199 || gw <= (double)norm_eps;
#pragma unroll
        for (int i = 0; i < K; ++i) wout[i] = (float)(mean ? 1.0 / K : 1.0 / K + kappa / gw * best_w[i]);
    }
}

inline void launch_cagrad(const float* G, int k, float c, float norm_eps, float* w, hipStream_t st) {
#define MOVAE_CAG(KV) hipLaunchKernelGGL((cagrad_k<KV>), dim3(1), dim3(64), 0, st, G, c, norm_eps, w)
    switch (k) {
        case 1: MOVAE_CAG(1); break;
        case 2: MOVAE_CAG(2); break;
        case 3: MOVAE_CAG(3); break;
        case 4: MOVAE_CAG(4); break;
// ... 190 lines not shown
int launch_combine_k(const float* J, size_t ldj, size_t m, const float* w, float* g, int acc, bool vec, hipStream_t st) {
    const int nb = gram_blocks(m);
    if (vec)
        hipLaunchKernelGGL((combine_k<K, true>), dim3(nb), dim3(256), 0, st, J, (long)ldj, (long)m, w, g, acc);
    else
        hipLaunchKernelGGL((combine_k<K, false>), dim3(nb), dim3(256), 0, st, J, (long)ldj, (long)m, w, g, acc);
    MOVAE_CHECK_LAUNCH("combine");
    return MOVAE_OK;
}

#define DISPATCH_K(k, CALL)                                      \
    switch (k) {                                                 \
        case 1: return CALL(1);                                  \
        case 2: return CALL(2);                                  \
        case 3: return CALL(3);                                  \
        case 4: return CALL(4);                                  \
        case 5: return CALL(5);                                  \
        case 6: return CALL(6);                                  \
        case 7: return CALL(7);                                  \
        case 8: return CALL(8);                                  \
        default: break;                                          \
    }

__global__ __launch_bounds__(64) void pcgrad_k(const float* __restrict__ G, int K, const int32_t* __restrict__ perm,
                                               float* __restrict__ wout) {
    if (threadIdx.x != 0) return;
    float w[MAXK];
    for (int i = 0; i < K; ++i) w[i] = 0.f;
    for (int i = 0; i < K; ++i) {
        float cur[MAXK];
        for (int q = 0; q < K; ++q) cur[q] = q == i ? 1.f : 0.f;
        for (int t = 0; t < K; ++t) {
            const int j = perm[i * K + t];
            if (j == i || j < 0 || j >= K) continue;
            float ip = 0.f;
            for (int q = 0; q < K; ++q) ip += G[j * K + q] * cur[q];
            if (ip < 0.f) cur[j] -= ip / G[j * K + j];
        }
        for (int q = 0; q < K; ++q) w[q] += cur[q];
    }
    for (int i = 0; i < K; ++i) wout[i] = w[i];
}

__global__ __launch_bounds__(64) void imtlg_k(const float* __restrict__ Gin, int K, float* __restrict__ wout) {
    if (threadIdx.x != 0) return;
    double A[MAXK][MAXK], V[MAXK][MAXK], d[MAXK], v[MAXK];
    for (int i = 0; i < K; ++i)
        for (int j = 0; j < K; ++j) {
            A[i][j] = 0.5 * ((double)Gin[i * K + j] + (double)Gin[j * K + i]);
            V[i][j] = i == j ? 1.0 : 0.0;
        }
    for (int i = 0; i < K; ++i) d[i] = sqrt(fmax((double)Gin[i * K + i], 0.0));
    jacobi_eigh(A, V, K);
    double lmax = 0.0;
    for (int i = 0; i < K; ++i) lmax = fmax(lmax, fabs(A[i][i]));
    const double cut = (double)K * 1.1920928955078125e-07 * lmax;
    for (int i = 0; i < K; ++i) v[i] = 0.0;
    for (int e = 0; e < K; ++e) {
        if (fabs(A[e][e]) <= cut) continue;
        double proj = 0.0;
        for (int i = 0; i < K; ++i) proj += V[i][e] * d[i];
        proj /= A[e][e];
        for (int i = 0; i < K; ++i) v[i] += V[i][e] * proj;
    }
    double sum = 0.0;
    for (int i = 0; i < K; ++i) sum += v[i];
    for (int i = 0; i < K; ++i) wout[i] = fabs(sum) < 1e-12 ? 0.f : (float)(v[i] / sum);
}


}

extern "C" {

size_t movae_gram_ws_bytes(int k, size_t m) {
    if (k <= 0) return 0;
    return MOVAE_WS_HEADER_BYTES + (size_t)gram_blocks(m) * (size_t)(k * (k + 1) / 2) * sizeof(double);
}

int movae_gram(const float* J, size_t ldj, int k, size_t m, float* G, void* ws, size_t ws_bytes, movae_stream_t stream) {
    MOVAE_WS_SCRATCH(ws, ws_bytes);
    MOVAE_CHECK_ARG(J && G && m > 0 && ldj >= m, "movae_gram: bad argument");
    MOVAE_CHECK_ARG(k >= 1 && k <= MAXK, "movae_gram: k=%d outside 1..%d", k, MAXK);
    MOVAE_CHECK_ARG(ws && ws_bytes >= movae_gram_ws_bytes(k, m), "movae_gram: workspace too small");
    hipStream_t st = (hipStream_t)stream;
    double* part = static_cast<double*>(ws);
    const int nb = gram_blocks(m);
    const bool vec = (ldj % 4 == 0) && (reinterpret_cast<uintptr_t>(J) & 15) == 0;
    int rc = MOVAE_EINVAL;
#define CALL_GRAM(KK) launch_gram_k<KK>(J, ldj, m, part, nb, vec, st)
    rc = [&]() -> int { DISPATCH_K(k, CALL_GRAM) return MOVAE_EINVAL; }();
#undef CALL_GRAM
    if (rc) return rc;
    hipLaunchKernelGGL(gram_final, dim3(k * (k + 1) / 2), dim3(64), 0, st, part, nb, k, G);
    MOVAE_CHECK_LAUNCH("gram_final");
    return MOVAE_OK;
}

int movae_combine(const float* J, size_t ldj, int k, size_t m, const float* w, float* g, int accumulate, movae_stream_t stream) {
    MOVAE_CHECK_ARG(J && w && g && m > 0 && ldj >= m, "movae_combine: bad argument");
    MOVAE_CHECK_ARG(k >= 1 && k <= MAXK, "movae_combine: k=%d outside 1..%d", k, MAXK);
    hipStream_t st = (hipStream_t)stream;
    const bool vec = (ldj % 4 == 0) && ((reinterpret_cast<uintptr_t>(J) | reinterpret_cast<uintptr_t>(g)) & 15) == 0;
#define CALL_COMB(KK) launch_combine_k<KK>(J, ldj, m, w, g, accumulate, vec, st)
    return [&]() -> int { DISPATCH_K(k, CALL_COMB) return MOVAE_EINVAL; }();
#undef CALL_COMB
}

int movae_gd_similarity(const float* J, size_t ldj, int k, size_t m, const float* w, float* out, void* ws, size_t ws_bytes,
                        movae_stream_t stream) {
    MOVAE_WS_SCRATCH(ws, ws_bytes);
    MOVAE_CHECK_ARG(J && w && out && m > 0 && k >= 1 && k <= MAXK, "movae_gd_similarity: bad argument");
    const int nb = gram_blocks(m);
    MOVAE_CHECK_ARG(ws && ws_bytes >= (size_t)nb * 3 * sizeof(double), "movae_gd_similarity: workspace too small");
    double* part = static_cast<double*>(ws);
    hipLaunchKernelGGL(similarity_partial, dim3(nb), dim3(256), 0, (hipStream_t)stream, J, (long)ldj, k, (long)m, w, part);
    MOVAE_CHECK_LAUNCH("similarity_partial");
    hipLaunchKernelGGL(similarity_final, dim3(1), dim3(64), 0, (hipStream_t)stream, part, nb, out);
    MOVAE_CHECK_LAUNCH("similarity_final");
    return MOVAE_OK;
}

int movae_weights_upgrad_norm(const float* G, int k, int norm_mode, float norm_eps, float reg_eps, const float* pref, float* w,
                              movae_stream_t stream) {
    MOVAE_CHECK_ARG(G && w, "movae_weights_upgrad: null pointer");
    MOVAE_CHECK_ARG(k >= 1 && k <= MAXK, "movae_weights_upgrad: k=%d outside 1..%d", k, MAXK);
    MOVAE_CHECK_ARG(norm_mode >= 0 && norm_mode <= 2, "movae_weights_upgrad: unknown normalisation %d", norm_mode);
    launch_upgrad(G, k, norm_mode, norm_eps, reg_eps, pref, w, 0, (hipStream_t)stream);
    MOVAE_CHECK_LAUNCH("upgrad");
    return MOVAE_OK;
}

int movae_gram_upgrad(const float* J, size_t ldj, int k, size_t m, float* G, int norm_mode, float norm_eps, float reg_eps,
                      const float* pref, float* w, int dual, void* ws, size_t ws_bytes, movae_stream_t stream) {
    MOVAE_WS_SCRATCH(ws, ws_bytes);
    MOVAE_CHECK_ARG(J && G && w && m > 0 && ldj >= m, "movae_gram_upgrad: bad argument");
    MOVAE_CHECK_ARG(k >= 1 && k <= MAXK, "movae_gram_upgrad: k=%d outside 1..%d", k, MAXK);
    MOVAE_CHECK_ARG(norm_mode >= 0 && norm_mode <= 2, "movae_gram_upgrad: unknown normalisation %d", norm_mode);
    MOVAE_CHECK_ARG(ws && ws_bytes >= movae_gram_ws_bytes(k, m), "movae_gram_upgrad: workspace too small");
    hipStream_t st = (hipStream_t)stream;
    double* part = static_cast<double*>(ws);
    const int nb = gram_blocks(m);
    const bool vec = (ldj % 4 == 0) && (reinterpret_cast<uintptr_t>(J) & 15) == 0;
    int rc = MOVAE_EINVAL;
#define CALL_GRAM(KK) launch_gram_k<KK>(J, ldj, m, part, nb, vec, st)
    rc = [&]() -> int { DISPATCH_K(k, CALL_GRAM) return MOVAE_EINVAL; }();
#undef CALL_GRAM
    if (rc) return rc;
    launch_upgrad(nullptr, k, norm_mode, norm_eps, reg_eps, pref, w, dual ? 1 : 0, st, part, nb, G);
    MOVAE_CHECK_LAUNCH("upgrad (with the Gramian's final fold)");
    return MOVAE_OK;
}

int movae_weights_dualproj(const float* G, int k, float norm_eps, float reg_eps, const float* pref, float* w, movae_stream_t stream) {
    MOVAE_CHECK_ARG(G && w, "movae_weights_dualproj: null pointer");
    MOVAE_CHECK_ARG(k >= 1 && k <= MAXK, "movae_weights_dualproj: k=%d outside 1..%d", k, MAXK);
    launch_upgrad(G, k, 0, norm_eps, reg_eps, pref, w, 1, (hipStream_t)stream);
    MOVAE_CHECK_LAUNCH("dualproj");
    return MOVAE_OK;
}

int movae_weights_cagrad(const float* G, int k, float c, float norm_eps, float* w, movae_stream_t stream) {
    MOVAE_CHECK_ARG(G && w, "movae_weights_cagrad: null pointer");
    MOVAE_CHECK_ARG(k >= 1 && k <= MAXK, "movae_weights_cagrad: k=%d outside 1..%d", k, MAXK);
    MOVAE_CHECK_ARG(c >= 0.f, "Parameter `c` should be a non-negative float. Found `c = %g`.", (double)c);
    launch_cagrad(G, k, c, norm_eps, w, (hipStream_t)stream);
    MOVAE_CHECK_LAUNCH("cagrad");
    return MOVAE_OK;
}

int movae_weights_pcgrad(const float* G, int k, const int32_t* perm, float* w, movae_stream_t stream) {
    MOVAE_CHECK_ARG(G && w && perm, "movae_weights_pcgrad: null pointer");
    MOVAE_CHECK_ARG(k >= 1 && k <= MAXK, "movae_weights_pcgrad: k=%d outside 1..%d", k, MAXK);
    hipLaunchKernelGGL(pcgrad_k, dim3(1), dim3(64), 0, (hipStream_t)stream, G, k, perm, w);
    MOVAE_CHECK_LAUNCH("pcgrad");
    return MOVAE_OK;
}

int movae_weights_imtlg(const float* G, int k, float* w, movae_stream_t stream) {
    MOVAE_CHECK_ARG(G && w, "movae_weights_imtlg: null pointer");
    MOVAE_CHECK_ARG(k >= 1 && k <= MAXK, "movae_weights_imtlg: k=%d outside 1..%d", k, MAXK);
    hipLaunchKernelGGL(imtlg_k, dim3(1), dim3(64), 0, (hipStream_t)stream, G, k, w);
    MOVAE_CHECK_LAUNCH("imtlg");
    return MOVAE_OK;
}

int movae_weights_upgrad(const float* G, int k, float norm_eps, float reg_eps, const float* pref, float* w, movae_stream_t stream) {
    return movae_weights_upgrad_norm(G, k, MOVAE_UPGRAD_TRACE, norm_eps, reg_eps, pref, w, stream);
}

int movae_weights_mgda_stable(const float* G, int k, int norm, const float* losses, float epsilon, int max_iters, float min_eigenvalue,
                              float* w, int32_t* info, movae_stream_t stream) {
    MOVAE_CHECK_ARG(G && w, "movae_weights_mgda: null pointer");
    MOVAE_CHECK_ARG(k >= 1 && k <= MAXK, "movae_weights_mgda: k=%d outside 1..%d", k, MAXK);
    MOVAE_CHECK_ARG(norm >= 0 && norm <= 3, "movae_weights_mgda: unknown norm %d", norm);
    MOVAE_CHECK_ARG(!(norm >= MOVAE_MGDA_LOSS && !losses),
                    "Losses must be set before calling forward() when using norm_type='loss'/'loss+'");
    hipLaunchKernelGGL(mgda_k, dim3(1), dim3(64), 0, (hipStream_t)stream, G, k, norm, losses, epsilon, max_iters, w, info, 1,
                       min_eigenvalue);
    MOVAE_CHECK_LAUNCH("mgda");
    return MOVAE_OK;
}

int movae_weights_mgda(const float* G, int k, int norm, const float* losses, float epsilon, int max_iters, float* w,
                       int32_t* info, movae_stream_t stream) {
    MOVAE_CHECK_ARG(G && w, "movae_weights_mgda: null pointer");
    MOVAE_CHECK_ARG(k >= 1 && k <= MAXK, "movae_weights_mgda: k=%d outside 1..%d", k, MAXK);
    MOVAE_CHECK_ARG(norm >= 0 && norm <= 3, "movae_weights_mgda: unknown norm %d", norm);
    MOVAE_CHECK_ARG(!(norm >= MOVAE_MGDA_LOSS && !losses),
                    "Losses must be set before calling forward() when using norm_type='loss'/'loss+'");
    hipLaunchKernelGGL(mgda_k, dim3(1), dim3(64), 0, (hipStream_t)stream, G, k, norm, losses, epsilon, max_iters, w, info, 0, 0.f);
    MOVAE_CHECK_LAUNCH("mgda");
    return MOVAE_OK;
}

int movae_weights_amtl(const float* G, int k, int scale_mode, const float* pref, float* w, movae_stream_t stream) {
    MOVAE_CHECK_ARG(G && w, "movae_weights_amtl: null pointer");
    MOVAE_CHECK_ARG(k >= 1 && k <= MAXK, "movae_weights_amtl: k=%d outside 1..%d", k, MAXK);
    MOVAE_CHECK_ARG(scale_mode >= 0 && scale_mode <= 2, "Invalid scale_mode=%d. Expected 'min', 'median', or 'rmse'.", scale_mode);
    hipLaunchKernelGGL(amtl_k, dim3(1), dim3(64), 0, (hipStream_t)stream, G, k, scale_mode, pref, w);
    MOVAE_CHECK_LAUNCH("amtl");
    return MOVAE_OK;
}

int movae_weights_const(int k, float value, float* w, movae_stream_t stream) {
    MOVAE_CHECK_ARG(w && k >= 1 && k <= MAXK, "movae_weights_const: bad argument");
    hipLaunchKernelGGL(const_k, dim3(1), dim3(64), 0, (hipStream_t)stream, k, value, w);
    MOVAE_CHECK_LAUNCH("const_w");
    return MOVAE_OK;
}

}
```

mo-vae_amd/csrc/conv_thin.h:

```cpp
#pragma once

namespace thin {

__device__ __forceinline__ void thin_in_tile_out(float* __restrict__ Wl, float* __restrict__ Y, int M, int t, float* __restrict__ stats,
                                                 const BnBwd& bb, const ActMul& am, int N, int n0, int bx) {
    float* yb = Y + (long)bx * 256 * N + n0;
    const long rows_left = (long)M - (long)bx * 256;
    if (stats) {
        const int c = t & 31, r0 = (t >> 5) * 32;
        float sm = 0.f, sq = 0.f;
        for (int r = 0; r < 32; ++r)
            if (r0 + r < rows_left) {
                const float v = Wl[(r0 + r) * 33 + c];
                sm += v;
                sq = fmaf(v, v, sq);
            }
        sm += __shfl_xor(sm, 32, 64);
        sq += __shfl_xor(sq, 32, 64);
        if ((t & 63) < 32) {
            const long pidx = (long)bx * 4 + (t >> 6);
            stats[(pidx * 2 + 0) * 32 + c] = sm;
            stats[(pidx * 2 + 1) * 32 + c] = sq;
        }
    }
// ... 893 lines not shown
    const int lane = t & 63, half = lane >> 5, l31 = lane & 31, wave = t >> 6;
    int delta[NT];
    float keep[NT];
#pragma unroll
    for (int u = 0; u < NT; ++u) {
        const int n = u * 32 + l31, nn = n < NA ? n : 0;
        const int tap = nn / TC, j = nn - tap * TC, kh = tap / KW, kw = tap - kh * KW;
        delta[u] = ((REV ? KH - 1 - kh : kh) * BW + (REV ? KW - 1 - kw : kw)) * 4 + j;
        keep[u] = n < NA ? 1.f : 0.f;
    }
    f32x16 acc[NT];
#pragma unroll
    for (int u = 0; u < NT; ++u)
#pragma unroll
        for (int r = 0; r < 16; ++r) acc[u][r] = 0.f;
    const int step = REV ? 1 : stride;
    const int tw_shift = __ffs(TW) - 1;
    constexpr int WPF = 8, TPF = 5;
    f32x4 wv[WPF];
    float tv[TPF][TC];
    unsigned wok = 0;
    const int q = t & 7;
    auto fetch = [&](int tile) {
        int b = tile;
        const int tw = b % tiles_w;
        b /= tiles_w;
        const int th = b % tiles_h, img = b / tiles_h;
        const int y0 = th * TH, x0 = tw * TW;
        const float* Wb = Wide + (long)img * Hw * Ww * Cw + c0 + q * 4;
        wok = 0;
#pragma unroll
        for (int u = 0; u < WPF; ++u) {
            const int pix = (t >> 3) + 32 * u;
            const int py = fdiv(pix, fd_tw), px = pix - py * TW;
            const int y = y0 + py, x = x0 + px;
            const bool ok = pix < npix && y < Hw && x < Ww;
            wv[u] = ok ? *reinterpret_cast<const f32x4*>(Wb + ((long)y * Ww + x) * Cw) : f32x4{0.f, 0.f, 0.f, 0.f};
            wok |= ok ? 1u << u : 0u;
        }
        const float* Tb = Thin + (long)img * Ht * Wt * TC;
        const int ty0 = REV ? y0 + pad - (KH - 1) : y0 * stride - pad, tx0 = REV ? x0 + pad - (KW - 1) : x0 * stride - pad;
#pragma unroll
        for (int u = 0; u < TPF; ++u) {
            const int pix = t + 256 * u;
            const int r = fdiv(pix, fd_bw), c = pix - r * BW;
            const int y = ty0 + r, x = tx0 + c;
            const bool ok = pix < BH * BW && y >= 0 && y < Ht && x >= 0 && x < Wt;
            const float* src = Tb + ((long)y * Wt + x) * TC;
#pragma unroll
            for (int j = 0; j < TC; ++j) tv[u][j] = ok ? src[j] : 0.f;
        }
    };
    f32x4 nsc = f32x4{1.f, 1.f, 1.f, 1.f}, nsh = f32x4{0.f, 0.f, 0.f, 0.f};
    if (nrm.scale) {
        nsc = *reinterpret_cast<const f32x4*>(nrm.scale + c0 + q * 4);
        nsh = *reinterpret_cast<const f32x4*>(nrm.shift + c0 + q * 4);
    }
    if (t < 8) *reinterpret_cast<f32x4*>(wideT + npix * 32 + t * 4) = f32x4{0.f, 0.f, 0.f, 0.f};
    float csum[TC];
#pragma unroll
    for (int j = 0; j < TC; ++j) csum[j] = 0.f;
    const bool cs_here = REV && cs_on && by == 0;
    if (bx < ntiles) fetch(bx);
    for (int tile = bx; tile < ntiles; tile += gdx) {
        __syncthreads();
#pragma unroll
        for (int u = 0; u < WPF; ++u) {
            const int pix = (t >> 3) + 32 * u;
            f32x4 v = wv[u];
            if (nrm.scale && (wok >> u & 1)) v = norm_apply(v, nsc, nsh, nrm.slope);
            if (pix < npix) *reinterpret_cast<f32x4*>(wideT + pix * 32 + q * 4) = v;
        }
        int oy0 = 0, ox0 = 0;
        if (cs_here) {
            int b = tile;
            const int tw = b % tiles_w;
            b /= tiles_w;
            const int th = b % tiles_h;
            oy0 = min(TH, Hw - th * TH), ox0 = min(TW, Ww - tw * TW);
        }
#pragma unroll
        for (int u = 0; u < TPF; ++u) {
            const int pix = t + 256 * u;
            f32x4 v = f32x4{0.f, 0.f, 0.f, 0.f};
#pragma unroll
            for (int j = 0; j < TC; ++j) v[j] = tv[u][j];
            if (pix < BH * BW) *reinterpret_cast<f32x4*>(thinF + pix * 4) = v;
            if (cs_here) {
                const int r = fdiv(pix, fd_bw), c = pix - r * BW;
                const int ry = r - (KH - 1 - pad), rx = c - (KW - 1 - pad);
                if (pix < BH * BW && ry >= 0 && ry < oy0 && rx >= 0 && rx < ox0) {
#pragma unroll
                    for (int j = 0; j < TC; ++j) csum[j] += tv[u][j];
                }
            }
        }
        if (tile + gdx < ntiles) fetch(tile + gdx);
        __syncthreads();
        for (int p = 2 * wave + half; p < npix; p += 32) {
            float a[4], bv[4][NT];
#pragma unroll
            for (int k = 0; k < 4; ++k) {
                const int pk = p + 8 * k;
                a[k] = wideT[pk * 32 + l31];
                const int base = __mul24(__mul24(pk >> tw_shift, step), BW) + __mul24(pk & (TW - 1), step);
#pragma unroll
                for (int u = 0; u < NT; ++u) bv[k][u] = thinF[base * 4 + delta[u]] * keep[u];
            }
#pragma unroll
            for (int k = 0; k < 4; ++k)
#pragma unroll
                for (int u = 0; u < NT; ++u) acc[u] = __builtin_amdgcn_mfma_f32_32x32x2f32(a[k], bv[k][u], acc[u], 0, 0, 0);
        }
    }
    __syncthreads();
#pragma unroll
    for (int u = 0; u < NT; ++u)
#pragma unroll
        for (int r = 0; r < 16; ++r) wideT[((wave * NT + u) * 16 + r) * 64 + lane] = acc[u][r];
    __syncthreads();
    const int N = TAPS * Cb;
    float* out = slab + (long)bx * row_stride;
    if (cs_here) {
        __shared__ float csr[4][TC];
#pragma unroll
        for (int j = 0; j < TC; ++j) {
            float v = csum[j];
#pragma unroll
            for (int off = 32; off > 0; off >>= 1) v += __shfl_xor(v, off, 64);
            if (lane == 0) csr[wave][j] = v;
        }
        __syncthreads();
        if (t < TC) out[(long)Cs * N + t] = (csr[0][t] + csr[1][t]) + (csr[2][t] + csr[3][t]);
    }
    for (int idx = t; idx < NT * 1024; idx += 256) {
        const int u = idx >> 10, r = (idx >> 6) & 15, ln = idx & 63;
        const int n = u * 32 + (ln & 31);
        if (n >= NA) continue;
        float v = 0.f;
#pragma unroll
        for (int w = 0; w < 4; ++w) v += wideT[((w * NT + u) * 16 + r) * 64 + ln];
        const int m = (r & 3) + 8 * (r >> 2) + 4 * (ln >> 5);
        const int tap = n / TC, j = n - tap * TC, c = c0 + m;
        const long o = REV ? ((long)j * TAPS + tap) * Cb + c : ((long)c * TAPS + tap) * Cb + j;
        out[o] = v;
    }
}

template <int TC, int KH, int KW, bool REV>
__global__ __launch_bounds__(256) void thin_wgrad_mfma_k(const float* __restrict__ Wide, const float* __restrict__ Thin,
                                                         float* __restrict__ slab, int Hw, int Ww, int Cw, int Ht, int Wt,
                                                         int stride, int pad, int TH, int TW, int tiles_h, int tiles_w,
                                                         int Cs, int Cb, long wide_gs, long thin_gs, long slab_gs, Norm nrm, int ntiles,
                                                         FastDiv fd_tw, FastDiv fd_bw, int cs_on, long row_stride) {
    thin_wgrad_mfma_body<TC, KH, KW, REV>(Wide, Thin, slab, Hw, Ww, Cw, Ht, Wt, stride, pad, TH, TW, tiles_h, tiles_w, Cs, Cb, wide_gs,
                                          thin_gs, slab_gs, nrm, ntiles, fd_tw, fd_bw, cs_on, row_stride, blockIdx.x, blockIdx.y,
                                          blockIdx.z, gridDim.x);
}

inline bool thin_in_ok(const Geom& g) { return g.Cr <= 4 && g.Nn >= 8 && g.KH * g.KW * g.Cr * 64 * 4 <= 48 * 1024; }

template <bool BWD>
int launch_thin_in(const float* X, const float* W, float* Y, const Geom& g, const Epilogue& ep, hipStream_t st) {
    const long Ml = (long)g.Nimg * g.Ho * g.Wo;
    const int M = (int)Ml, K = g.KH * g.KW * g.Cr;
    const bool n32 = g.Nn == 32;
    dim3 grid(ceil_div(M, 256), 1);
    float* stats = nullptr;
    if (!BWD && n32 && ep.act == MOVAE_ACT_NONE) stats = fuse_stats_claim((long)grid.x * 4, 32);
    BnBwd bb{};
    if (BWD && n32 && g_fuse.bn_y && ep.act == MOVAE_ACT_NONE && !ep.bias && M % g_fuse.bn_groups == 0 && (M / g_fuse.bn_groups) % 256 == 0) {
        const long rpg = M / g_fuse.bn_groups;
        if (float* part = fuse_bn_claim(rpg / 256 * 4, 32))
            bb = BnBwd{g_fuse.bn_y, g_fuse.bn_scale, g_fuse.bn_shift, g_fuse.bn_slope, part, (int)rpg, (int)(rpg / 256 * 4)};
    }
    static const bool valu_only = getenv("MOVAE_THIN_IN_VALU") != nullptr;
    const int hw = g.Ho * g.Wo;
    const bool k33 = g.KH == 3 && g.KW == 3, k44 = g.KH == 4 && g.KW == 4;
    bool mfma = !valu_only && g.Nn % 32 == 0 && g.Cr == 3 && (k33 || k44) && (!BWD || g.stride == 1) && hw % 256 == 0 &&
                (256 % g.Wo == 0 || g.Wo % 256 == 0) && g.wrow == 0 && (reinterpret_cast<uintptr_t>(Y) & 15) == 0;
    const int ncols = g.Wo < 256 ? g.Wo : 256, nrows = 256 / ncols;
    const int RH = BWD ? nrows + g.KH - 1 : (nrows - 1) * g.stride + g.KH;
    const int RW = BWD ? ncols + g.KW - 1 : (ncols - 1) * g.stride + g.KW;
    size_t lf = (size_t)RH * RW * 3 + (BWD ? 0 : 32 * (g.KH * g.KW * 3 | 1));
    if (lf < 256 * 33) lf = 256 * 33;
    mfma = mfma && lf * sizeof(float) <= 60 * 1024;
    ActMul am{nullptr, 0, 0.f, 0, 0, nullptr};
    if ((g_fuse.am.y || g_fuse.am.res) && (n32 || mfma) && ep.act == MOVAE_ACT_NONE && (!ep.bias || !g_fuse.am.y) && !bb.y && !stats &&
        M % g_fuse.am_groups == 0 && (reinterpret_cast<uintptr_t>(Y) & 15) == 0) {
        am = g_fuse.am;
        am.per_group = (long)(M / g_fuse.am_groups) * g.Nn;
        g_fuse.am_done = true;
    }
    if (mfma) {
        grid.y = g.Nn / 32;
#define MOVAE_TI(K)                                                                                                                \
    hipLaunchKernelGGL((thin_in_mfma_k<K, K, BWD>), grid, dim3(256), lf * sizeof(float), st, X, W, ep.bias, Y, g, M, ep.act, ep.slope,  \
                       stats, bb, am, ncols, RH, RW, fastdiv_make(RW * 3), fastdiv_make(3), fastdiv_make(ncols), fastdiv_make(hw),  \
                       fastdiv_make(g.Wo))
        if (k33) MOVAE_TI(3); else MOVAE_TI(4);
#undef MOVAE_TI
        g_last_kernel = k33 ? (BWD ? "thin_in_mfma_k<3,3,true>" : "thin_in_mfma_k<3,3,false>")
                            : (BWD ? "thin_in_mfma_k<4,4,true>" : "thin_in_mfma_k<4,4,false>");
        MOVAE_CHECK_LAUNCH("thin_in_mfma");
        return MOVAE_OK;
    }
    if (g.Nn > 32) {
        grid.y = ceil_div(g.Nn, 64);
        hipLaunchKernelGGL((thin_in_k<64, BWD>), grid, dim3(256), (size_t)K * 64 * sizeof(float), st, X, W, ep.bias, Y, g, M,
                           ep.act, ep.slope, (float*)nullptr, BnBwd{}, ActMul{nullptr, 0, 0.f, 0, 0, nullptr});
        g_last_kernel = BWD ? "thin_in_k<64,true>" : "thin_in_k<64,false>";
    } else {
        size_t lds_floats = (size_t)K * 32;
        if (n32 && lds_floats < 256 * 33) lds_floats = 256 * 33;
        hipLaunchKernelGGL((thin_in_k<32, BWD>), grid, dim3(256), lds_floats * sizeof(float), st, X, W, ep.bias, Y, g, M,
                           ep.act, ep.slope, stats, bb, am);
        g_last_kernel = BWD ? "thin_in_k<32,true>" : "thin_in_k<32,false>";
    }
    MOVAE_CHECK_LAUNCH("thin_in");
    return MOVAE_OK;
}

inline bool thin_out_ok(const Geom& g, const float* X) {
    return g.Nn <= 4 && g.Cr % 4 == 0 && (reinterpret_cast<uintptr_t>(X) & 15) == 0 &&
           (size_t)4 * g.KH * g.KW * g.Cr * sizeof(float) <= 60 * 1024;
}

int launch_thin_out_fwd(const float* X, const float* W, float* Y, const Geom& g, const Epilogue& ep, hipStream_t st) {
    const int M = g.Nimg * g.Ho * g.Wo, K = g.KH * g.KW * g.Cr;
    hipLaunchKernelGGL((thin_out_fwd_k<4>), dim3(ceil_div(M, 256)), dim3(256), (size_t)4 * K * sizeof(float), st, X, W, ep.bias,
                       Y, g, M, ep.act, ep.slope);
    g_last_kernel = "thin_out_fwd_k<4>";
    MOVAE_CHECK_LAUNCH("thin_out_fwd");
    return MOVAE_OK;
}

template <bool BWD>
inline bool thin_out_tile_plan(const Geom& g, const float* X, int& TH, int& TW, int& IH, int& IW, int& CC, int& PPT) {
    if (g.Nn > 4 || g.Cr % 4 != 0 || (reinterpret_cast<uintptr_t>(X) & 15) != 0) return false;
    if (BWD && g.stride != 2) return false;
    if (g.KH * g.KW > 16) return false;
    TW = g.Wo < 32 ? (BWD ? (g.Wo + 1) / 2 * 2 : g.Wo) : 32;
    if (TW < 1) return false;
    const long px_total = (long)g.Nimg * g.Ho * g.Wo;
    static const int force_ppt = env_long("MOVAE_THIN_PPT", 0);
    for (int ppt = force_ppt ? force_ppt : (px_total >= 200000L ? 2 : 1); ppt >= 1; --ppt) {
        int th = 256 * ppt / TW;
        if (BWD) th = th / 2 * 2;
        if (th < (BWD ? 2 : 1)) continue;
        if (BWD && (256 * ppt) % (TW * 2) != 0) continue;
        if (!BWD && (256 * ppt) % TW != 0) continue;
        for (int cc = 32; cc >= 16; cc -= 16) {
            const int ih = BWD ? (th + g.KH - 2) / 2 + 2 : (th - 1) * g.stride + g.KH;
            const int iw = BWD ? (TW + g.KW - 2) / 2 + 2 : (TW - 1) * g.stride + g.KW;
            const long bytes = ((long)ih * iw * (cc + 4) + (long)g.KH * g.KW * 4 * cc) * 4;
            if (bytes <= 62 * 1024) {
                TH = th; IH = ih; IW = iw; CC = cc; PPT = ppt;
                return true;
            }
        }
    }
    return false;
}

template <bool BWD>
int launch_thin_out_tile(const float* X, const float* W, float* Y, const Geom& g, const Epilogue& ep, hipStream_t st, bool* handled) {
    static const bool valu_only = getenv("MOVAE_THIN_OUT_VALU") != nullptr;
    if (!BWD && !valu_only && g.Nn == 3 && g.Cr % 32 == 0 && g.stride == 1 && g.KH == 3 && g.KW == 3 && g.wrow == 0 &&
        g.Ho == g.Hi + 2 * g.pad - 2 && g.Wo == g.Wi + 2 * g.pad - 2 &&
        ((reinterpret_cast<uintptr_t>(X) | reinterpret_cast<uintptr_t>(W) | reinterpret_cast<uintptr_t>(g_fuse.nrm.scale) |
          reinterpret_cast<uintptr_t>(g_fuse.nrm.shift)) & 15) == 0) {
        const int tiles_h = ceil_div(g.Ho, 8), tiles_w = ceil_div(g.Wo, 32);
        const long nblk = (long)g.Nimg * tiles_h * tiles_w;
        if (nblk <= 0x7fffffffL) {
            constexpr int NG = (10 * 34 + 31) / 32;
            if (g.Cr == 32)
                hipLaunchKernelGGL((thin_out_mfma_k<3, 3, true>), dim3((unsigned)nblk), dim3(256), (size_t)NG * 32 * 27 * sizeof(float), st,
                                   X, W, ep.bias, Y, g, tiles_h, tiles_w, ep.act, ep.slope, g_fuse.nrm);
            else
                hipLaunchKernelGGL((thin_out_mfma_k<3, 3, false>), dim3((unsigned)nblk), dim3(256), (size_t)NG * 32 * 27 * sizeof(float), st,
                                   X, W, ep.bias, Y, g, tiles_h, tiles_w, ep.act, ep.slope, g_fuse.nrm);
            g_last_kernel = g.Cr == 32 ? "thin_out_mfma_k<3,3,true>" : "thin_out_mfma_k<3,3,false>";
            MOVAE_CHECK_LAUNCH("thin_out_mfma");
            *handled = true;
            return MOVAE_OK;
        }
    }
    if (BWD && !valu_only && g.Nn == 3 && g.Cr % 32 == 0 && g.stride == 2 && g.KH == 4 && g.KW == 4 && g.pad == 1 && g.Ho == 2 * g.Hi &&
        g.Wo == 2 * g.Wi && ((reinterpret_cast<uintptr_t>(X) | reinterpret_cast<uintptr_t>(g_fuse.nrm.scale) |
                              reinterpret_cast<uintptr_t>(g_fuse.nrm.shift)) & 15) == 0) {
        const int tiles_h = ceil_div(g.Hi, 8), tiles_w = ceil_div(g.Wi, 32);
        const long nblk = (long)g.Nimg * tiles_h * tiles_w;
        const size_t wt = (size_t)48 * (g.Cr + 4), pt = (size_t)11 * 32 * 49;
        const size_t shb = (wt > pt ? wt : pt) * sizeof(float);
        if (nblk <= 0x7fffffffL && shb <= 80 * 1024) {
            hipLaunchKernelGGL(thin_outT_mfma_k, dim3((unsigned)nblk), dim3(256), shb, st, X, W, ep.bias, Y, g, tiles_h, tiles_w, ep.act,
                               ep.slope, g_fuse.nrm);
            g_last_kernel = "thin_outT_mfma_k";
            MOVAE_CHECK_LAUNCH("thin_outT_mfma");
            *handled = true;
            return MOVAE_OK;
        }
    }
    int TH, TW, IH, IW, CC, PPT;
    *handled = thin_out_tile_plan<BWD>(g, X, TH, TW, IH, IW, CC, PPT);
    if (!*handled) return MOVAE_OK;
    const int tiles_h = ceil_div(g.Ho, TH), tiles_w = ceil_div(g.Wo, TW);
    const long nblk = (long)g.Nimg * tiles_h * tiles_w;
    if (nblk > 0x7fffffffL) {
        *handled = false;
        return MOVAE_OK;
    }
    const size_t shb = ((size_t)IH * IW * (CC + 4) + (size_t)g.KH * g.KW * 4 * CC) * sizeof(float);
#define MOVAE_TO(CCV, PPTV)                                                                                                                            \
    do {                                                                                                                                               \
        hipLaunchKernelGGL((thin_out_tile_k<BWD, CCV, PPTV>), dim3((unsigned)nblk), dim3(256), shb, st, X, W, ep.bias, Y, g, TH, TW, tiles_h,          \
                           tiles_w, IH, IW, ep.act, ep.slope, g_fuse.nrm);                                                                             \
        g_last_kernel = BWD ? "thin_out_tile_k<true," #CCV "," #PPTV ">" : "thin_out_tile_k<false," #CCV "," #PPTV ">";                                \
    } while (0)
    if (CC == 32) {
        if (PPT == 2) MOVAE_TO(32, 2); else MOVAE_TO(32, 1);
    } else {
        if (PPT == 2) MOVAE_TO(16, 2); else MOVAE_TO(16, 1);
    }
#undef MOVAE_TO
    MOVAE_CHECK_LAUNCH("thin_out_tile");
    return MOVAE_OK;
}

inline bool thin_wgrad_ok(const WGeom& g) { return g.Cs <= 4 || g.Cb <= 4; }

int launch_thin_wgrad(const float* S, const float* Bg, float* dW, const WGeom& g, int K, int accumulate, void* ws,
                      size_t ws_bytes, hipStream_t st);

int launch_thin_wgrad_grouped(const float* S, const float* Bg, float* const* dW, int G, long s_gs, long b_gs, const WGeom& g, int K,
                              int accumulate, void* ws, size_t ws_bytes, hipStream_t st, float* const* colsum = nullptr,
                              bool* colsum_done = nullptr);

int launch_thin_wgrad_impl(const float* S, const float* Bg, float* const* dW, int G, long s_gs, long b_gs, const WGeom& g, int K,
                           int accumulate, void* ws, size_t ws_bytes, hipStream_t st, bool* handled, float* const* colsum = nullptr,
                           bool* colsum_done = nullptr) {
    const int M = g.Cs, N = g.KH * g.KW * g.Cb;
    *handled = true;
    const bool thin_small = g.Cs <= 4;
    const int wide = thin_small ? g.Cb : g.Cs;
    {
        const int tc = thin_small ? g.Cs : g.Cb;
        const bool k33 = g.KH == 3 && g.KW == 3, k44 = g.KH == 4 && g.KW == 4;
        const bool aligned = (reinterpret_cast<uintptr_t>(thin_small ? Bg : S) & 15) == 0;
        if ((k33 || k44) && wide % 32 == 0 && tc == 3 && aligned && (!thin_small || g.stride == 1) && ws) {
            const int Hw = thin_small ? g.Hb : g.Hs, Ww = thin_small ? g.Wb : g.Ws;
            const int Ht = thin_small ? g.Hs : g.Hb, Wt = thin_small ? g.Ws : g.Wb;
            const int TW = Ww < 32 ? Ww : 32;
            static const int tile_px = env_long("MOVAE_THIN_TILE_PX", 256);
            int TH = tile_px / TW;
            if (TH < 1) TH = 1;
            if (TH > Hw) TH = Hw;
            const int TH0 = TH;
            const int taps = g.KH * g.KW, na = taps * 3;
            static const bool mfma_env = !getenv("MOVAE_THIN_WGRAD_SWEEP");
            bool use_mfma = mfma_env;
            auto lds_bytes = [&](int th, int tw) {
                const int bh = thin_small ? th + g.KH - 1 : (th - 1) * g.stride + g.KH;
                const int bw = thin_small ? tw + g.KW - 1 : (tw - 1) * g.stride + g.KW;
                long tile_f = (long)th * tw * 32, fold_f = 8L * 32 * ((na + 1) / 2);
                if (use_mfma) tile_f += 32, fold_f = 4L * ((na + 31) / 32) * 1024;
                const long wide_f = tile_f > fold_f ? tile_f : fold_f;
                return (wide_f + (long)bh * bw * 4) * 4;
            };
            auto thin_px = [&](int th, int tw) {
                return (thin_small ? th + g.KH - 1 : (th - 1) * g.stride + g.KH) * (thin_small ? tw + g.KW - 1 : (tw - 1) * g.stride + g.KW);
            };
            while ((lds_bytes(TH, TW) > 60 * 1024 || (use_mfma && (TH * TW > 256 || thin_px(TH, TW) > 1280))) && TH > 1) TH = (TH + 1) / 2;
            if (use_mfma && !(TH * TW <= 256 && thin_px(TH, TW) <= 1280 && (TW & (TW - 1)) == 0 && (TH * TW) % 32 == 0)) {
                use_mfma = false;
                TH = TH0;
                while (lds_bytes(TH, TW) > 60 * 1024 && TH > 1) TH = (TH + 1) / 2;
            }
            const int tiles_h = ceil_div(Hw, TH), tiles_w = ceil_div(Ww, TW);
            const long ntiles = (long)g.Nimg * tiles_h * tiles_w;
            static const int persist = env_long("MOVAE_THIN_PERSIST", 768);
            long nblk = ntiles;
            if (use_mfma) {
                const long cap = persist / ((long)(wide / 32) * G) > 64 ? persist / ((long)(wide / 32) * G) : 64;
                if (nblk > cap) nblk = cap;
            }
            static const long cs_min = env_long("MOVAE_THIN_CS_MIN", 1L << 18);
            bool cs_on = use_mfma && thin_small && colsum && g.Hs == g.Hb && g.Ws == g.Wb && (long)K >= cs_min;
            for (int i = 0; cs_on && i < G; ++i) cs_on = colsum[i] != nullptr;
            const long row = (long)M * N + (cs_on ? M : 0);
            const size_t per1 = (size_t)row * sizeof(float);
            if (lds_bytes(TH, TW) <= 60 * 1024 && ntiles <= 0x7fffffffL && per1 * (size_t)nblk * G <= ws_bytes) {
                float* slab = static_cast<float*>(ws);
                const dim3 grid((unsigned)nblk, wide / 32, G);
                const long slab_gs = (long)nblk * row;
                const long wide_gs = thin_small ? b_gs : s_gs, thin_gs = thin_small ? s_gs : b_gs;
                const size_t shb = (size_t)lds_bytes(TH, TW);
                const float* Wd = thin_small ? Bg : S;
                const float* Tn = thin_small ? S : Bg;
                Norm wide_nrm{nullptr, nullptr, 1.f};
                if (fuse_norm()) {
                    if (g_fuse.nrm_side != (thin_small ? 2 : 1)) {
                        movae_set_error("thin wgrad: the fused input transform applies to the wide operand only");
                        return MOVAE_EUNSUPPORTED;
                    }
                    wide_nrm = g_fuse.nrm;
                }
#define MOVAE_SW(K, REVV)                                                                                                                              \
    do {                                                                                                                                               \
        hipLaunchKernelGGL((thin_wgrad_sweep_k<3, K, K, REVV>), grid, dim3(256), shb, st, Wd, Tn, slab, Hw, Ww, wide, Ht, Wt, g.stride,                \
                           g.pad, TH, TW, tiles_h, tiles_w, g.Cs, g.Cb, wide_gs, thin_gs, slab_gs, wide_nrm);                                          \
        g_last_kernel = "thin_wgrad_sweep_k<3," #K "," #K "," #REVV ">";                                                                               \
    } while (0)
#define MOVAE_MF(K, REVV)                                                                                                                              \
    do {                                                                                                                                               \
        hipLaunchKernelGGL((thin_wgrad_mfma_k<3, K, K, REVV>), grid, dim3(256), shb, st, Wd, Tn, slab, Hw, Ww, wide, Ht, Wt, g.stride,                 \
                           g.pad, TH, TW, tiles_h, tiles_w, g.Cs, g.Cb, wide_gs, thin_gs, slab_gs, wide_nrm, (int)ntiles, fastdiv_make(TW),            \
                           fastdiv_make(thin_small ? TW + g.KW - 1 : (TW - 1) * g.stride + g.KW), cs_on ? 1 : 0, row);                                 \
        g_last_kernel = "thin_wgrad_mfma_k<3," #K "," #K "," #REVV ">";                                                                                \
    } while (0)
                if (use_mfma) {
                    if (thin_small) {
                        if (k33) MOVAE_MF(3, true); else MOVAE_MF(4, true);
                    } else {
                        if (k33) MOVAE_MF(3, false); else MOVAE_MF(4, false);
                    }
                } else if (thin_small) {
                    if (k33) MOVAE_SW(3, true); else MOVAE_SW(4, true);
                } else {
                    if (k33) MOVAE_SW(3, false); else MOVAE_SW(4, false);
                }
#undef MOVAE_SW
#undef MOVAE_MF
                MOVAE_CHECK_LAUNCH("thin_wgrad_sweep");
                {
                    RGroups rg{};
                    for (int i = 0; i < G; ++i) rg.out[i] = dW[i], rg.out2[i] = cs_on ? colsum[i] : nullptr;
                    rg.slab_gs = slab_gs;
                    if (int rc = launch_reduce_groups(slab, rg, G, (long)M * N, cs_on ? M : 0, (int)nblk, N, nullptr, 0, 0.f, accumulate, st,
                                                      ActMul{nullptr, 0, 0.f, 0, 0, nullptr}, true))
                        return rc;
                }
                if (colsum_done) *colsum_done = cs_on;
                return MOVAE_OK;
            }
        }
    }
    *handled = false;
    MOVAE_NO_NORM("thin wgrad (non-sweep kernels)");
    return MOVAE_OK;
}

int launch_thin_wgrad_grouped(const float* S, const float* Bg, float* const* dW, int G, long s_gs, long b_gs, const WGeom& g, int K,
                              int accumulate, void* ws, size_t ws_bytes, hipStream_t st, float* const* colsum, bool* colsum_done) {
    bool handled = false;
    if (int rc = launch_thin_wgrad_impl(S, Bg, dW, G, s_gs, b_gs, g, K, accumulate, ws, ws_bytes, st, &handled, colsum, colsum_done))
        return rc;
    if (handled) return MOVAE_OK;
    for (int i = 0; i < G; ++i)
        if (int rc = launch_thin_wgrad(S + i * s_gs, Bg + i * b_gs, dW[i], g, K, accumulate, ws, ws_bytes, st)) return rc;
    return MOVAE_OK;
}

int launch_thin_wgrad(const float* S, const float* Bg, float* dW, const WGeom& g, int K, int accumulate, void* ws,
                      size_t ws_bytes, hipStream_t st) {
    const int M = g.Cs, N = g.KH * g.KW * g.Cb;
    const bool thin_small = g.Cs <= 4;
    const int wide = thin_small ? g.Cb : g.Cs;
    {
        float* one[1] = {dW};
        bool handled = false;
        if (int rc = launch_thin_wgrad_impl(S, Bg, one, 1, 0, 0, g, K, accumulate, ws, ws_bytes, st, &handled)) return rc;
        if (handled) return MOVAE_OK;
    }
    {
        int TW = g.Ws < 32 ? g.Ws : 32, TH = g.Hs < 16 ? g.Hs : 16;
        auto lds_floats = [&](int th, int tw) {
            return (long)th * tw * g.Cs + (long)((th - 1) * g.stride + g.KH) * ((tw - 1) * g.stride + g.KW) * g.Cb;
        };
        while (lds_floats(TH, TW) * 4 > 48 * 1024 && (TH > 1 || TW > 1)) {
            if (TH >= TW && TH > 1) TH = (TH + 1) / 2;
            else TW = (TW + 1) / 2;
        }
        const int tiles_h = ceil_div(g.Hs, TH), tiles_w = ceil_div(g.Ws, TW);
        const long nblk = (long)g.Nimg * tiles_h * tiles_w;
        const size_t per1 = (size_t)M * N * sizeof(float);
        if (lds_floats(TH, TW) * 4 <= 48 * 1024 && nblk <= 65535L * 16 && ws && per1 * (size_t)nblk <= ws_bytes) {
            const int items = g.KH * g.KW * wide;
            int nth = ceil_div(items, 64) * 64;
            if (nth > 1024) nth = 1024;
            float* slab = static_cast<float*>(ws);
            const size_t shb = (size_t)lds_floats(TH, TW) * sizeof(float);
            const int tc = thin_small ? g.Cs : g.Cb;
#define MOVAE_TW(SM, TCV)                                                                                                                              \
    do {                                                                                                                                               \
        hipLaunchKernelGGL((thin_wgrad_tiled_k<SM, TCV>), dim3((unsigned)nblk), dim3(nth), shb, st, S, Bg, slab, g, TH, TW,                            \
                           tiles_h, tiles_w);                                                                                                          \
        g_last_kernel = "thin_wgrad_tiled_k<" #SM "," #TCV ">";                                                                                        \
    } while (0)
            if (thin_small) {
                if (tc == 1) MOVAE_TW(true, 1); else if (tc == 2) MOVAE_TW(true, 2); else if (tc == 3) MOVAE_TW(true, 3); else MOVAE_TW(true, 4);
            } else {
                if (tc == 1) MOVAE_TW(false, 1); else if (tc == 2) MOVAE_TW(false, 2); else if (tc == 3) MOVAE_TW(false, 3); else MOVAE_TW(false, 4);
            }
#undef MOVAE_TW
            MOVAE_CHECK_LAUNCH("thin_wgrad_tiled");
            return launch_reduce(slab, dW, (long)M * N, (int)nblk, N, nullptr, 0, 0.f, accumulate, st);
        }
    }
    int WL = 1;
    while (WL < wide && WL < 256) WL *= 2;
    const int PL = 256 / WL;
    int nch = ceil_div(K, PL * 16);
    if (nch > 1024) nch = 1024;
    const size_t per = (size_t)M * N * sizeof(float);
    while (nch > 1 && per * nch > ws_bytes) nch /= 2;
    if (!ws || per * nch > ws_bytes) {
        movae_set_error("thin wgrad: workspace too small");
        return MOVAE_EINVAL;
    }
    const int chunk = ceil_div(K, nch);
    nch = ceil_div(K, chunk);
    float* slab = static_cast<float*>(ws);
    dim3 grid(nch, g.KH * g.KW);
    if (thin_small)
        hipLaunchKernelGGL((thin_wgrad_k<true>), grid, dim3(256), 0, st, S, Bg, slab, g, K, chunk, WL);
    else
        hipLaunchKernelGGL((thin_wgrad_k<false>), grid, dim3(256), 0, st, S, Bg, slab, g, K, chunk, WL);
    g_last_kernel = thin_small ? "thin_wgrad_k<true>" : "thin_wgrad_k<false>";
    MOVAE_CHECK_LAUNCH("thin_wgrad_k");
    return launch_reduce(slab, dW, (long)M * N, nch, N, nullptr, 0, 0.f, accumulate, st);
}

}
```

mo-vae_amd/csrc/optim.hip:

```cpp
#include "common.h"

namespace {

__global__ __launch_bounds__(256) void adam_k(float* __restrict__ p, const float* __restrict__ g, float* __restrict__ m,
                                              float* __restrict__ v, long n, float lr, float b1, float b2, float eps,
                                              float wd, int decoupled, float bc1, float bc2_sqrt) {
    const long stride = (long)gridDim.x * blockDim.x;
    for (long i = (long)blockIdx.x * blockDim.x + threadIdx.x; i < n; i += stride) {
        float gi = g[i], pi = p[i];
        if (wd != 0.f) {
            if (decoupled) pi *= 1.f - lr * wd;
            else gi += wd * pi;
        }
        const float mi = m[i] + (gi - m[i]) * (1.f - b1);
        const float vi = v[i] * b2 + (1.f - b2) * gi * gi;
        m[i] = mi;
        v[i] = vi;
        const float denom = sqrtf(vi) / bc2_sqrt + eps;
        p[i] = pi - (lr / bc1) * (mi / denom);
    }
}

constexpr int ADAM_MT = 64;
struct AdamTable {
    float* p[ADAM_MT];
    const float* g[ADAM_MT];
    float* m[ADAM_MT];
    float* v[ADAM_MT];
    unsigned n[ADAM_MT];
    unsigned first[ADAM_MT + 1];
};
constexpr unsigned ADAM_BLK = 4096;

__device__ __forceinline__ void adam_one(float& pi, float gi, float& mi, float& vi, float lr, float b1, float b2, float eps,
                                         float wd, int decoupled, float step_size, float bc2_sqrt) {
    if (wd != 0.f) {
        if (decoupled) pi *= 1.f - lr * wd;
        else gi += wd * pi;
    }
    mi = mi + (gi - mi) * (1.f - b1);
    vi = vi * b2 + (1.f - b2) * gi * gi;
    const float denom = sqrtf(vi) / bc2_sqrt + eps;
    pi = pi - step_size * (mi / denom);
}

__device__ unsigned g_adam_done = 0;

__global__ __launch_bounds__(256) void adam_multi_k(AdamTable tab, int cnt, float lr, float b1, float b2, float eps, float wd,
                                                    int decoupled, float bc1, float bc2_sqrt, float* __restrict__ hyper, int tick) {
    int t = 0;
    while (t + 1 < cnt && blockIdx.x >= tab.first[t + 1]) ++t;
    const unsigned n = tab.n[t], base = (blockIdx.x - tab.first[t]) * ADAM_BLK;
    float step_f = 0.f;
    if (hyper) {
        step_f = hyper[0] + 1.f;
        const double step = (double)step_f;
        lr = hyper[1];
        bc1 = (float)(1.0 - pow((double)b1, step));
        bc2_sqrt = (float)sqrt(1.0 - pow((double)b2, step));
    }
    const float step_size = lr / bc1;
    float* __restrict__ p = tab.p[t];
    const float* __restrict__ g = tab.g[t];
    float* __restrict__ m = tab.m[t];
    float* __restrict__ v = tab.v[t];
    const bool vec = ((reinterpret_cast<uintptr_t>(p) | reinterpret_cast<uintptr_t>(g) | reinterpret_cast<uintptr_t>(m) |
                       reinterpret_cast<uintptr_t>(v)) & 15) == 0;
    if (vec && base + ADAM_BLK <= n) {
        f32x4 pv[4], mv[4], vv[4], gv[4];
#pragma unroll
        for (int u = 0; u < 4; ++u) {
            const unsigned i = base + u * 1024u + threadIdx.x * 4;
            pv[u] = *reinterpret_cast<f32x4*>(p + i), mv[u] = *reinterpret_cast<f32x4*>(m + i), vv[u] = *reinterpret_cast<f32x4*>(v + i);
            gv[u] = *reinterpret_cast<const f32x4*>(g + i);
        }
#pragma unroll
        for (int u = 0; u < 4; ++u) {
            const unsigned i = base + u * 1024u + threadIdx.x * 4;
#pragma unroll
            for (int j = 0; j < 4; ++j) {
                float pj = pv[u][j], mj = mv[u][j], vj = vv[u][j];
                adam_one(pj, gv[u][j], mj, vj, lr, b1, b2, eps, wd, decoupled, step_size, bc2_sqrt);
                pv[u][j] = pj; mv[u][j] = mj; vv[u][j] = vj;
            }
            *reinterpret_cast<f32x4*>(p + i) = pv[u];
            *reinterpret_cast<f32x4*>(m + i) = mv[u];
            *reinterpret_cast<f32x4*>(v + i) = vv[u];
        }
    } else
    for (unsigned u = 0; u < 4; ++u) {
        const unsigned i = base + u * 1024u + threadIdx.x * 4;
        if (i >= n) break;
        if (vec && i + 4 <= n) {
            f32x4 pv = *reinterpret_cast<f32x4*>(p + i), mv = *reinterpret_cast<f32x4*>(m + i), vv = *reinterpret_cast<f32x4*>(v + i);
            const f32x4 gv = *reinterpret_cast<const f32x4*>(g + i);
#pragma unroll
            for (int j = 0; j < 4; ++j) {
                float pj = pv[j], mj = mv[j], vj = vv[j];
                adam_one(pj, gv[j], mj, vj, lr, b1, b2, eps, wd, decoupled, step_size, bc2_sqrt);
                pv[j] = pj; mv[j] = mj; vv[j] = vj;
            }
            *reinterpret_cast<f32x4*>(p + i) = pv;
            *reinterpret_cast<f32x4*>(m + i) = mv;
            *reinterpret_cast<f32x4*>(v + i) = vv;
        } else {
            const unsigned e = min(i + 4, n);
            for (unsigned k = i; k < e; ++k) {
                float pj = p[k], mj = m[k], vj = v[k];
                adam_one(pj, g[k], mj, vj, lr, b1, b2, eps, wd, decoupled, step_size, bc2_sqrt);
                p[k] = pj; m[k] = mj; v[k] = vj;
            }
        }
    }
    if (hyper) {
        __syncthreads();
        if (threadIdx.x == 0) {
            const unsigned done = atomicAdd(&g_adam_done, 1u);
            if (done == gridDim.x - 1) {
                g_adam_done = 0;
                if (tick) hyper[0] = step_f;
            }
        }
    }
}

__global__ __launch_bounds__(256) void sumsq_partial(const float* __restrict__ x, long n, double* __restrict__ part) {
    __shared__ double sh[4];
    double s = 0.0;
    const long stride = (long)gridDim.x * blockDim.x;
    for (long i = (long)blockIdx.x * blockDim.x + threadIdx.x; i < n; i += stride) s += (double)x[i] * x[i];
    s = block_sum_256(s, sh);
    if (threadIdx.x == 0) part[blockIdx.x] = s;
}

__global__ __launch_bounds__(256) void sumsq_final(const double* __restrict__ part, int nblk, float* __restrict__ out) {
    __shared__ double sh[4];
    double s = 0.0;
    for (int i = threadIdx.x; i < nblk; i += 256) s += part[i];
    s = block_sum_256(s, sh);
    if (threadIdx.x == 0) out[0] = (float)s;
}

__global__ void clip_scale_k(float* __restrict__ g, long n, const float* __restrict__ sumsq, float max_norm) {
    const float coef = fminf(max_norm / (sqrtf(sumsq[0]) + 1e-6f), 1.f);
    const long stride = (long)gridDim.x * blockDim.x;
    for (long i = (long)blockIdx.x * blockDim.x + threadIdx.x; i < n; i += stride) g[i] *= coef;
}

struct ClipTable {
    float* g[ADAM_MT];
    unsigned n[ADAM_MT];
};

__global__ __launch_bounds__(256) void sumsq_multi_k(ClipTable tab, double* __restrict__ part) {
    __shared__ double sh[4];
    const float* __restrict__ g = tab.g[blockIdx.y];
    const unsigned n = tab.n[blockIdx.y];
    double s = 0.0;
    for (unsigned i = blockIdx.x * 256u + threadIdx.x; i < n; i += gridDim.x * 256u) s += (double)g[i] * g[i];
    s = block_sum_256(s, sh);
    if (threadIdx.x == 0) part[blockIdx.y * gridDim.x + blockIdx.x] = s;
}

__global__ __launch_bounds__(256) void sumsq_multi_final(const double* __restrict__ part, int nparts, float* __restrict__ sumsq,
                                                         int accumulate) {
    __shared__ double sh[4];
    double s = 0.0;
    for (int i = threadIdx.x; i < nparts; i += 256) s += part[i];
    s = block_sum_256(s, sh);
    if (threadIdx.x == 0) sumsq[0] = accumulate ? sumsq[0] + (float)s : (float)s;
}

__global__ __launch_bounds__(256) void clip_multi_k(ClipTable tab, const float* __restrict__ sumsq, float max_norm) {
    const float coef = fminf(max_norm / (sqrtf(sumsq[0]) + 1e-6f), 1.f);
    if (coef >= 1.f) return;
    float* __restrict__ g = tab.g[blockIdx.y];
    const unsigned n = tab.n[blockIdx.y];
    for (unsigned i = blockIdx.x * 256u + threadIdx.x; i < n; i += gridDim.x * 256u) g[i] *= coef;
}

inline int blocks_for(size_t n) {
    size_t b = (n + 1023) / 1024;
    return (int)(b > 2048 ? 2048 : (b < 1 ? 1 : b));
}

}

extern "C" {

int movae_adam_step(float* p, const float* g, float* m, float* v, size_t n, float lr, float beta1, float beta2, float eps,
                    float weight_decay, int decoupled_wd, int step, movae_stream_t stream) {
    MOVAE_CHECK_ARG(p && g && m && v && n > 0 && step >= 1, "movae_adam_step: bad argument");
    const double bc1 = 1.0 - pow((double)beta1, step), bc2 = 1.0 - pow((double)beta2, step);
    hipLaunchKernelGGL(adam_k, dim3(blocks_for(n)), dim3(256), 0, (hipStream_t)stream, p, g, m, v, (long)n, lr, beta1, beta2, eps,
                       weight_decay, decoupled_wd, (float)bc1, (float)sqrt(bc2));
    MOVAE_CHECK_LAUNCH("adam");
    return MOVAE_OK;
}

int movae_adam_multi(int n_tensors, float* const* p, const float* const* g, float* const* m, float* const* v, const size_t* numel,
                     float lr, float beta1, float beta2, float eps, float weight_decay, int decoupled_wd, int step,
                     float* hyper_dev, movae_stream_t stream) {
    MOVAE_CHECK_ARG(n_tensors >= 0 && (n_tensors == 0 || (p && g && m && v && numel)), "movae_adam_multi: null table");
    MOVAE_CHECK_ARG(hyper_dev || step >= 1, "movae_adam_multi: step must be >= 1 when no device counter is given");
    float bc1 = 1.f, bc2_sqrt = 1.f;
    if (!hyper_dev) {
        bc1 = (float)(1.0 - pow((double)beta1, step));
        bc2_sqrt = (float)sqrt(1.0 - pow((double)beta2, step));
    }
    for (int t0 = 0; t0 < n_tensors; t0 += ADAM_MT) {
        AdamTable tab;
        const int cnt = n_tensors - t0 < ADAM_MT ? n_tensors - t0 : ADAM_MT;
        unsigned nblk = 0;
        for (int i = 0; i < cnt; ++i) {
            MOVAE_CHECK_ARG(p[t0 + i] && g[t0 + i] && m[t0 + i] && v[t0 + i], "movae_adam_multi: null tensor");
            MOVAE_CHECK_ARG(numel[t0 + i] > 0 && numel[t0 + i] < 0xffffffffUL, "movae_adam_multi: tensor size out of range");
            tab.p[i] = p[t0 + i]; tab.g[i] = g[t0 + i]; tab.m[i] = m[t0 + i]; tab.v[i] = v[t0 + i];
            tab.n[i] = (unsigned)numel[t0 + i];
            tab.first[i] = nblk;
            nblk += (unsigned)((numel[t0 + i] + ADAM_BLK - 1) / ADAM_BLK);
        }
        for (int i = cnt; i < ADAM_MT; ++i) { tab.p[i] = nullptr; tab.g[i] = nullptr; tab.m[i] = nullptr; tab.v[i] = nullptr; tab.n[i] = 0; }
        for (int i = cnt; i <= ADAM_MT; ++i) tab.first[i] = nblk;
        hipLaunchKernelGGL(adam_multi_k, dim3(nblk), dim3(256), 0, (hipStream_t)stream, tab, cnt, lr, beta1, beta2, eps, weight_decay,
                           decoupled_wd, bc1, bc2_sqrt, hyper_dev, t0 + ADAM_MT >= n_tensors ? 1 : 0);
        MOVAE_CHECK_LAUNCH("adam_multi");
    }
    return MOVAE_OK;
}

int movae_clip_grad_norm_multi(int n_tensors, float* const* g, const size_t* numel, float max_norm, float* total_sumsq_dev, void* ws,
                               size_t ws_bytes, movae_stream_t stream) {
    MOVAE_WS_SCRATCH(ws, ws_bytes);
    MOVAE_CHECK_ARG(n_tensors >= 1 && g && numel && total_sumsq_dev && max_norm > 0.f, "movae_clip_grad_norm_multi: bad argument");
    constexpr int BX = 32;
    MOVAE_CHECK_ARG(ws && ws_bytes >= (size_t)ADAM_MT * BX * sizeof(double), "movae_clip_grad_norm_multi: workspace too small");
    double* part = static_cast<double*>(ws);
    hipStream_t st = (hipStream_t)stream;
    for (int pass = 0; pass < 2; ++pass)
        for (int t0 = 0; t0 < n_tensors; t0 += ADAM_MT) {
            ClipTable tab;
            const int cnt = n_tensors - t0 < ADAM_MT ? n_tensors - t0 : ADAM_MT;
            for (int i = 0; i < ADAM_MT; ++i) {
                tab.g[i] = i < cnt ? g[t0 + i] : nullptr;
                tab.n[i] = i < cnt ? (unsigned)numel[t0 + i] : 0;
                if (i < cnt) MOVAE_CHECK_ARG(g[t0 + i] && numel[t0 + i] < 0xffffffffUL, "movae_clip_grad_norm_multi: bad tensor");
            }
            if (pass == 0) {
                hipLaunchKernelGGL(sumsq_multi_k, dim3(BX, cnt), dim3(256), 0, st, tab, part);
                MOVAE_CHECK_LAUNCH("sumsq_multi");
                hipLaunchKernelGGL(sumsq_multi_final, dim3(1), dim3(256), 0, st, part, BX * cnt, total_sumsq_dev, t0 > 0 ? 1 : 0);
                MOVAE_CHECK_LAUNCH("sumsq_multi_final");
            } else {
                hipLaunchKernelGGL(clip_multi_k, dim3(BX, cnt), dim3(256), 0, st, tab, total_sumsq_dev, max_norm);
                MOVAE_CHECK_LAUNCH("clip_multi");
            }
        }
    return MOVAE_OK;
}

int movae_sumsq(const float* x, size_t n, float* out, void* ws, size_t ws_bytes, movae_stream_t stream) {
    MOVAE_WS_SCRATCH(ws, ws_bytes);
    MOVAE_CHECK_ARG(x && out && n > 0, "movae_sumsq: bad argument");
    const int nb = blocks_for(n);
    MOVAE_CHECK_ARG(ws && ws_bytes >= (size_t)nb * sizeof(double), "movae_sumsq: workspace too small");
    double* part = static_cast<double*>(ws);
    hipLaunchKernelGGL(sumsq_partial, dim3(nb), dim3(256), 0, (hipStream_t)stream, x, (long)n, part);
    MOVAE_CHECK_LAUNCH("sumsq_partial");
    hipLaunchKernelGGL(sumsq_final, dim3(1), dim3(256), 0, (hipStream_t)stream, part, nb, out);
    MOVAE_CHECK_LAUNCH("sumsq_final");
    return MOVAE_OK;
}

int movae_scale_by_clip(float* g, size_t n, const float* sumsq_dev, float max_norm, movae_stream_t stream) {
    MOVAE_CHECK_ARG(g && sumsq_dev && n > 0 && max_norm > 0.f, "movae_scale_by_clip: bad argument");
    hipLaunchKernelGGL(clip_scale_k, dim3(blocks_for(n)), dim3(256), 0, (hipStream_t)stream, g, (long)n, sumsq_dev, max_norm);
    MOVAE_CHECK_LAUNCH("clip_scale");
    return MOVAE_OK;
}

}
```

mo-vae_amd/optim.py:

```python
import ctypes as C

import torch

from . import _lib as L


def _dense(t):
    return t.is_contiguous() or (t.dim() == 4 and t.is_contiguous(memory_format=torch.channels_last))


def _layout_differs(a, p):
    return a.shape != p.shape or any(n > 1 and x != y for n, x, y in zip(p.shape, a.stride(), p.stride()))


class FusedAdam(torch.optim.Adam):

    def __init__(self, params, lr=1e-3, betas=(0.9, 0.999), eps=1e-8, weight_decay=0.0, decoupled_weight_decay=False,
                 device_step=False):
        super().__init__(params, lr=lr, betas=betas, eps=eps, weight_decay=weight_decay, foreach=False, capturable=False)
        self._decoupled = bool(decoupled_weight_decay)
        self._device_step = bool(device_step)
        self._hyper = {}
        self._hyper_lr = {}

    def _group_hyper(self, gi, group, device):
        h = self._hyper.get(gi)
        if h is None:
            h = torch.tensor([0.0, float(group["lr"])], dtype=torch.float32, device=device)
            self._hyper[gi] = h
            self._hyper_lr[gi] = float(group["lr"])
        return h

    def sync_hyper(self):
        for gi, group in enumerate(self.param_groups):
            h = self._hyper.get(gi)
            if h is not None and self._hyper_lr[gi] != float(group["lr"]):
                h[1].fill_(float(group["lr"]))
                self._hyper_lr[gi] = float(group["lr"])

    @torch.no_grad()
    def step(self, closure=None):
        loss = None
        if closure is not None:
            with torch.enable_grad():
                loss = closure()
        for gi, group in enumerate(self.param_groups):
            if group.get("amsgrad") or group.get("maximize"):
                raise NotImplementedError("FusedAdam: amsgrad / maximize are not part of the reference's configuration")
            beta1, beta2 = group["betas"]
            buckets = {}
            hyper = None
            for p in group["params"]:
                g = p.grad
                if g is None:
                    continue
                L.require_gpu(p)
                if g.is_sparse:
                    raise RuntimeError("Adam does not support sparse gradients")
                if p.dtype != torch.float32 or not _dense(p):
                    raise NotImplementedError("FusedAdam: parameters must be dense fp32 tensors")
                if g.dtype != p.dtype or _layout_differs(g, p):
                    g = torch.empty_like(p).copy_(g)
                st = self.state[p]
                if len(st) == 0:
                    if self._device_step:
                        hyper = self._group_hyper(gi, group, p.device)
                        st["step"] = hyper[0]
                    else:
                        st["step"] = torch.tensor(0.0, dtype=torch.float32)
                    st["exp_avg"] = torch.zeros_like(p, memory_format=torch.preserve_format)
                    st["exp_avg_sq"] = torch.zeros_like(p, memory_format=torch.preserve_format)
                m, v = st["exp_avg"], st["exp_avg_sq"]
                if _layout_differs(m, p) or _layout_differs(v, p):
                    m = st["exp_avg"] = torch.empty_like(p).copy_(m)
                    v = st["exp_avg_sq"] = torch.empty_like(p).copy_(v)
                if self._device_step:
                    key = 0
                    if hyper is None:
                        hyper = self._group_hyper(gi, group, p.device)
                    if st["step"].data_ptr() != hyper.data_ptr():
                        hyper[0].copy_(st["step"])
                        st["step"] = hyper[0]
                else:
                    st["step"] += 1
                    key = int(st["step"].item())
                buckets.setdefault(key, []).append((p, g, m, v))
            for key, rows in buckets.items():
                n = len(rows)
                arr = C.c_void_p * n
                ps = arr(*[r[0].data_ptr() for r in rows])
                gs = arr(*[r[1].data_ptr() for r in rows])
                ms = arr(*[r[2].data_ptr() for r in rows])
                vs = arr(*[r[3].data_ptr() for r in rows])
                ns = (C.c_size_t * n)(*[r[0].numel() for r in rows])
                dev = rows[0][0].device
                if self._device_step and not torch.cuda.is_current_stream_capturing():
                    self.sync_hyper()
                L.call("movae_adam_multi", n, ps, gs, ms, vs, ns, float(group["lr"]), float(beta1), float(beta2),
                       float(group["eps"]), float(group["weight_decay"]), 1 if self._decoupled else 0,
                       max(1, key), L.ptr(hyper) if self._device_step else 0, L.stream_ptr(dev))
        return loss


class FusedAdamW(FusedAdam):

    def __init__(self, params, lr=1e-3, betas=(0.9, 0.999), eps=1e-8, weight_decay=1e-2, device_step=False):
        super().__init__(params, lr=lr, betas=betas, eps=eps, weight_decay=weight_decay, decoupled_weight_decay=True,
                         device_step=device_step)


def clip_grad_norm_(parameters, max_norm, norm_type=2.0):
    if float(norm_type) != 2.0:
        raise NotImplementedError("clip_grad_norm_: only the L2 norm of the reference's call is implemented")
    if isinstance(parameters, torch.Tensor):
        parameters = [parameters]
    grads = [p.grad for p in parameters if p.grad is not None]
    if not grads:
        return torch.tensor(0.0)
    for g in grads:
        L.require_gpu(g)
        if g.dtype != torch.float32 or not _dense(g):
            raise NotImplementedError("clip_grad_norm_: gradients must be dense fp32 tensors")
    dev = grads[0].device
    n = len(grads)
    sumsq = torch.empty((), dtype=torch.float32, device=dev)
    ws = L.workspace(dev)
    L.call("movae_clip_grad_norm_multi", n, (C.c_void_p * n)(*[g.data_ptr() for g in grads]),
           (C.c_size_t * n)(*[g.numel() for g in grads]), float(max_norm), sumsq.data_ptr(), ws.data_ptr(), ws.numel(),
           L.stream_ptr(dev))
    return sumsq.sqrt()
```

mo-vae_amd/parallel.py:

```python
import os

import torch
import torch.distributed as dist


def flatten_grads(params, out=None):
    chunks = []
    for p in params:
        if p.grad is None:
            chunks.append(torch.zeros(p.numel(), dtype=p.dtype, device=p.device))
            continue
        g = p.grad
        if g.shape != p.shape:
            raise RuntimeError(f"gradient shape {tuple(g.shape)} does not match its parameter {tuple(p.shape)}")
        if any(n > 1 and a != b for n, a, b in zip(p.shape, g.stride(), p.stride())):
            g = torch.empty_like(p).copy_(g)
        if g.dim() == 4 and not g.is_contiguous() and g.permute(0, 2, 3, 1).is_contiguous():
            chunks.append(g.permute(0, 2, 3, 1).reshape(-1))
        else:
            chunks.append(g.contiguous().reshape(-1))
    if out is not None:
        return torch.cat(chunks, out=out)
    return torch.cat(chunks)


def unflatten_into_grads(flat, params):
    off = 0
    for p in params:
        n = p.numel()
        p.grad = flat[off: off + n].as_strided(p.shape, p.stride())
        off += n


class DataParallelGrads:
    def __init__(self, rank, world_size, local_rank, backend):
        self.rank, self.world_size, self.local_rank, self.backend = rank, world_size, local_rank, backend
        self.params = []
        self.flat, self.views, self._arena_sig = None, None, None

    def _arena(self):
        if self.flat is None or self.flat.device != self.params[0].device or self._arena_sig != [(id(p), p.numel()) for p in self.params]:
            n = sum(p.numel() for p in self.params)
            self.flat = torch.zeros(n, dtype=torch.float32, device=self.params[0].device)
            self.views, off = [], 0
            for p in self.params:
                self.views.append(self.flat[off: off + p.numel()].as_strided(p.shape, p.stride()))
                off += p.numel()
            self._arena_sig = [(id(p), p.numel()) for p in self.params]
        return self.flat, self.views

    @classmethod
    def from_env(cls, backend=None):
        ws = int(os.environ.get("WORLD_SIZE", "1"))
        if ws <= 1 and not os.environ.get("MOVAE_FORCE_DP"):
            return None
        os.environ.setdefault("RANK", "0")
        os.environ.setdefault("MASTER_PORT", "29533")
        rank, local_rank = int(os.environ["RANK"]), int(os.environ.get("LOCAL_RANK", os.environ["RANK"]))
        backend = backend or os.environ.get("MOVAE_DIST_BACKEND") or ("nccl" if torch.cuda.is_available() else "gloo")
        if torch.cuda.is_available():
            local_rank = local_rank % torch.cuda.device_count()
            torch.cuda.set_device(local_rank)
        if not dist.is_initialized():
            os.environ.setdefault("MASTER_ADDR", "127.0.0.1")
            dist.init_process_group(backend=backend, rank=rank, world_size=ws)
        return cls(rank, ws, local_rank, backend)

    def attach(self, net):
        self.params = [p for p in net.parameters() if p.requires_grad]
        for t in list(net.parameters()) + list(net.buffers()):
            dist.broadcast(t.data, src=0)

    @torch.no_grad()
    def all_reduce_grads(self):
        flat, views = self._arena()
        src, dst = [], []
        for p, v in zip(self.params, views):
            if p.grad is None:
                v.zero_()
            elif p.grad.data_ptr() != v.data_ptr():
                if p.grad.shape != p.shape:
                    raise RuntimeError(f"gradient shape {tuple(p.grad.shape)} does not match its parameter {tuple(p.shape)}")
                src.append(p.grad)
                dst.append(v)
        if src:
            torch._foreach_copy_(dst, src)
        if self.backend == "nccl":
            dist.all_reduce(flat, op=dist.ReduceOp.AVG)
        else:
            dist.all_reduce(flat, op=dist.ReduceOp.SUM)
            flat.div_(self.world_size)
        for p, v in zip(self.params, views):
            p.grad = v
        return flat

    def barrier(self):
        dist.barrier()

    def shutdown(self):
        if dist.is_initialized():
            dist.destroy_process_group()
```

mo-vae_amd/train.py:

```python
import json
import math
import os
import time
from argparse import ArgumentParser

import torch
import torch.optim as optim

from . import _lib as L
from . import aggregation
from . import autojac
from . import ops
from .aggregation import COMFORT, MGDA
from .data import ALIASES, NPY_SETS, DeviceBatchLoader, ResidentImages, get_real_dataset
from .metrics import ReconMetricAccumulator, build_hv_indicator
from .models import get_network
from .optim import FusedAdam, FusedAdamW, clip_grad_norm_
from .parallel import DataParallelGrads

_current_step = 0
_hook_values = {}


class AverageMeter:

    def __init__(self):
        self.reset()

    def reset(self):
        self.val = self.avg = self.sum = 0.0
        self.count = 0

    def update(self, val, n=1):
        self.val = val
        self.sum += val * n
        self.count += n
        self.avg = self.sum / self.count


def set_seed(seed):
    import numpy as np

    np.random.seed(seed)
    torch.manual_seed(seed)
    if torch.cuda.is_available():
        torch.cuda.manual_seed(seed)
        torch.cuda.manual_seed_all(seed)


def print_weights(_, __, weights):
    _hook_values["weights"] = weights


def print_gd_similarity(_, inputs, weights):
    _hook_values["similarity"] = aggregation.gd_similarity(inputs[0], weights)


def _stacked(losses):
    first = losses[0]
    if all(c.dim() == 0 and c.dtype == first.dtype and c.untyped_storage().data_ptr() == first.untyped_storage().data_ptr()
           and c.storage_offset() == first.storage_offset() + i for i, c in enumerate(losses)):
        return first.detach().as_strided((len(losses),), (1,))
    return torch.stack([c.detach() for c in losses])


def forward_backward_begin(net, images, optimizer, aggregator):
    optimizer.zero_grad()
    outputs = net(images)
    loss_dict = net.loss_function(images, args=outputs)
    if aggregator is None or aggregator == "sum":
        loss_dict["total_loss"].backward()
        return loss_dict, outputs, None
    features = [outputs[f] for f in net.features] if net.features is not None else None
    component_losses = [v for k, v in loss_dict.items() if k != "total_loss"]
    if isinstance(aggregator, (MGDA, COMFORT)):
        aggregator.set_losses(_stacked(component_losses))
    if features is None:
        if getattr(net, "_jacobian_from_loss_op", False):
            autojac.backward_through(component_losses, aggregator)
        else:
            autojac.backward(component_losses, aggregator=aggregator)
        return loss_dict, outputs, None
    pending = autojac.mtl_backward_begin(component_losses, features, aggregator)
    pending.device = images.device
    return loss_dict, outputs, pending


def forward_backward_finish(pending):
    if pending is not None:
        autojac.mtl_backward_finish(pending)


def forward_backward(net, images, optimizer, aggregator):
    loss_dict, outputs, pending = forward_backward_begin(net, images, optimizer, aggregator)
    forward_backward_finish(pending)
    return loss_dict, outputs


def train_step(net, images, optimizer, aggregator, args, dp=None):
    loss_dict, outputs = forward_backward(net, images, optimizer, aggregator)
    if dp is not None:
        dp.all_reduce_grads()
    if getattr(args, "max_grad_norm", None) is not None:
        clip_grad_norm_(net.parameters(), max_norm=args.max_grad_norm)
    optimizer.step()
    return loss_dict, outputs




DP_OVERLAP_MIN_BYTES = 32 << 20


def _state_tensors(net):
    extra = [t for t in (getattr(net, "_iter_dev", None), getattr(net, "_noise_state_t", None)) if isinstance(t, torch.Tensor)]
    return list(net.parameters()) + list(net.buffers()) + extra


def _snapshot_state(net, optimizer, device):
    return {"tensors": [t.detach().clone() for t in _state_tensors(net)],
            "opt": {id(p): {k: v.detach().clone() for k, v in st.items() if torch.is_tensor(v)} for p, st in optimizer.state.items()},
            "cuda_rng": torch.cuda.get_rng_state(device), "cpu_rng": torch.get_rng_state()}


@torch.no_grad()
def _restore_state(snap, net, optimizer, device):
    torch.cuda.synchronize(device)
    for t, s in zip(_state_tensors(net), snap["tensors"]):
        t.copy_(s)
    for p, st in optimizer.state.items():
        old = snap["opt"].get(id(p), {})
        for k, v in st.items():
            if torch.is_tensor(v):
                if k in old:
                    v.copy_(old[k])
                else:
                    v.zero_()
    torch.cuda.set_rng_state(snap["cuda_rng"], device)
    torch.set_rng_state(snap["cpu_rng"])


class GraphedTrainStep:

    def __init__(self, net, optimizer, aggregator, args, example, warmup=3, dp=None, record_calls=False, preserve_state=False):
        if not getattr(net, "graph_safe", False):
            raise NotImplementedError(f"{type(net).__name__}: forward syncs with the host; use the eager train_step")
        if dp is not None and getattr(net, "features", ()) is None:
            raise NotImplementedError(f"{type(net).__name__}: the data-parallel graphed step is not supported for models whose Jacobian "
                                      "spans all parameters (features is None); use the eager step")
        net.prepare_for_graph()
        snap = _snapshot_state(net, optimizer, example.device) if preserve_state else None
        try:
            self._build(net, optimizer, aggregator, args, example, warmup, dp, record_calls)
        finally:
            if snap is not None:
                _restore_state(snap, net, optimizer, example.device)

    def _build(self, net, optimizer, aggregator, args, example, warmup, dp, record_calls):
        self.net, self.opt, self.agg, self.args, self.dp = net, optimizer, aggregator, args, dp
        self.static_x = example.clone()
        from . import _lib as L
        from .parallel import flatten_grads, unflatten_into_grads

        L.workspace(example.device)
        side = torch.cuda.Stream()
        side.wait_stream(torch.cuda.current_stream())
        with torch.cuda.stream(side):
            for _ in range(warmup):
                train_step(net, self.static_x, optimizer, aggregator, args, dp)
        torch.cuda.current_stream().wait_stream(side)
        torch.cuda.synchronize()
        self.graph = torch.cuda.CUDAGraph()
        self.graph2 = None
        self.dp_form = "single device"
        optimizer.zero_grad(set_to_none=True)
        self.calls = []
        if record_calls:
            L.TRACE = lambda name, cargs: self.calls.append((name, cargs))
        try:
            if dp is None:
                ops.forget_nhwc()
                with torch.cuda.graph(self.graph):
                    self.loss_dict, self.outputs = train_step(net, self.static_x, optimizer, aggregator, args)
                ops.forget_nhwc()
                return
        finally:
            L.TRACE = None
        params = [p for p in net.parameters() if p.requires_grad]
        self.flat = torch.zeros(sum(p.numel() for p in params) + 64, dtype=torch.float32, device=example.device)
        self._avg = dp.backend == "nccl"
        cap = dict(capture_error_mode="thread_local")
        torch.cuda.synchronize()
        mode = os.environ.get("MOVAE_DP_OVERLAP", "auto")
        overlap = mode == "1" or (mode == "auto" and self.flat.numel() * 4 >= DP_OVERLAP_MIN_BYTES)
        cc_mode = os.environ.get("MOVAE_DP_CAPTURE_COLLECTIVE", "auto")
        self.dp_form = "graph | all-reduce | graph"
        if not overlap and dp.backend == "nccl" and cc_mode != "0":
            err = None
            try:
                ops.forget_nhwc()
                whole = torch.cuda.CUDAGraph()
                with torch.cuda.graph(whole, **cap):
                    self.loss_dict, self.outputs = forward_backward(net, self.static_x, optimizer, aggregator)
                    self.flat_a = self.flat[: sum(p.numel() for p in params)]
                    flatten_grads(params, out=self.flat_a)
                    self.reduce(self.flat_a)
                    unflatten_into_grads(self.flat_a, params)
                    if getattr(args, "max_grad_norm", None) is not None:
                        clip_grad_norm_(params, max_norm=args.max_grad_norm)
                    optimizer.step()
                ops.forget_nhwc()
            except Exception as e:
                if cc_mode != "auto":
                    raise
                err = e
            ok = torch.tensor([0 if err is not None else 1], device=example.device, dtype=torch.int32)
            if cc_mode == "auto":
                torch.cuda.synchronize()
                torch.distributed.all_reduce(ok, op=torch.distributed.ReduceOp.MIN)
            if int(ok.item()) == 1:
                self.graph, self.graph_b, self.flat_b = whole, None, None
                self.dp_form = "1 graph + captured all-reduce"
                return
            print(f"[movae] capturing the all-reduce failed on some rank ({type(err).__name__ if err else 'peer'}: {err}); "
                  "all ranks use graph / all-reduce / graph", flush=True)
            torch.cuda.synchronize()
            optimizer.zero_grad(set_to_none=True)
            self.graph = torch.cuda.CUDAGraph()
        ops.forget_nhwc()
        with torch.cuda.graph(self.graph, **cap):
            self.loss_dict, self.outputs, pending = forward_backward_begin(net, self.static_x, optimizer, aggregator)
            if pending is not None and overlap:
                shared = {id(p) for p in pending.shared_params}
                early = [p for p in params if p.grad is not None and id(p) not in shared]
            else:
                forward_backward_finish(pending)
                pending, early = None, list(params)
            n_early = sum(p.numel() for p in early)
            self.flat_a = self.flat[:n_early]
            flatten_grads(early, out=self.flat_a)
        ops.forget_nhwc()
        taken = {id(p) for p in early}
        late = [p for p in params if id(p) not in taken]
        self.graph_b, self.flat_b = None, None
        if late:
            self.dp_form = "3 graphs, two overlapped all-reduces"
            off = (n_early + 63) // 64 * 64
            self.flat_b = self.flat[off: off + sum(p.numel() for p in late)]
            self.graph_b = torch.cuda.CUDAGraph()
            with torch.cuda.graph(self.graph_b, pool=self.graph.pool(), **cap):
                forward_backward_finish(pending)
                flatten_grads(late, out=self.flat_b)
        self._reduced_replay()
# ... 535 lines not shown
```

Measured before the change: 334,900.

## Defer UPGrad aggregation and fuse weight solve and gradient combine into Adam

After the Jacobian is built, only the Gram partial sums are launched. The UPGrad weight solve, the combine of Jacobian rows into a gradient, and the Adam update are deferred into one multi-tensor kernel that reads J directly. This removes separate gram-finalize/solve, combine and Adam launches, plus a write and re-read of the full gradient vector. The cost is added complexity: pending-state bookkeeping, finish() fallbacks in zero_grad, clip, DP and state_dict, and an in-kernel solve that every block repeats. It applies only to k<=4, a single param group, no clipping and no DP.

```diff
diff --git a/include/movae.h b/include/movae.h
--- a/include/movae.h
+++ b/include/movae.h
@@ -172,6 +172,8 @@
                               movae_stream_t stream);
 int movae_gram_upgrad(const float* J, size_t ldj, int k, size_t m, float* G, int norm_mode, float norm_eps, float reg_eps,
                       const float* pref, float* w, int dual, void* ws, size_t ws_bytes, movae_stream_t stream);
+int movae_gram_partials(const float* J, size_t ldj, int k, size_t m, double* part, size_t part_bytes, int* n_blocks,
+                        movae_stream_t stream);
 int movae_weights_mgda(const float* G, int k, int norm, const float* losses, float epsilon, int max_iters,
                        float* w, int32_t* info, movae_stream_t stream);
 int movae_weights_mgda_stable(const float* G, int k, int norm, const float* losses, float epsilon, int max_iters,
@@ -191,6 +193,11 @@
 int movae_adam_multi(int n_tensors, float* const* p, const float* const* g, float* const* m, float* const* v,
                      const size_t* numel, float lr, float beta1, float beta2, float eps, float weight_decay,
                      int decoupled_wd, int step, float* hyper_dev, movae_stream_t stream);
+int movae_adam_multi_agg(int n_tensors, float* const* p, float* const* g, float* const* m, float* const* v, const size_t* numel,
+                         float lr, float beta1, float beta2, float eps, float weight_decay, int decoupled_wd, int step,
+                         float* hyper_dev, const float* J, size_t ldj, size_t m_cols, int k, const long long* joff, const double* gram_part,
+                         int gram_blocks, int norm_mode, float norm_eps, float reg_eps, const float* pref, int dual, float* wout,
+                         float* Gout, movae_stream_t stream);
 int movae_clip_grad_norm_multi(int n_tensors, float* const* g, const size_t* numel, float max_norm, float* total_sumsq_dev,
                                void* ws, size_t ws_bytes, movae_stream_t stream);
 int movae_sumsq(const float* x, size_t n, float* out, void* ws, size_t ws_bytes, movae_stream_t stream);
diff --git a/mo-vae_amd/_lib.py b/mo-vae_amd/_lib.py
--- a/mo-vae_amd/_lib.py
+++ b/mo-vae_amd/_lib.py
@@ -95,6 +95,7 @@
     "movae_weights_upgrad": ([_p, _i, _f, _f, _p, _p, _p], _i),
     "movae_weights_upgrad_norm": ([_p, _i, _i, _f, _f, _p, _p, _p], _i),
     "movae_gram_upgrad": ([_p, _z, _i, _z, _p, _i, _f, _f, _p, _p, _i, _p, _z, _p], _i),
+    "movae_gram_partials": ([_p, _z, _i, _z, _p, _z, _p, _p], _i),
     "movae_weights_mgda": ([_p, _i, _i, _p, _f, _i, _p, _p, _p], _i),
     "movae_weights_mgda_stable": ([_p, _i, _i, _p, _f, _i, _f, _p, _p, _p], _i),
     "movae_weights_amtl": ([_p, _i, _i, _p, _p, _p], _i),
@@ -107,6 +108,8 @@
     "movae_gd_similarity": ([_p, _z, _i, _z, _p, _p, _p, _z, _p], _i),
     "movae_adam_step": ([_p, _p, _p, _p, _z, _f, _f, _f, _f, _f, _i, _i, _p], _i),
     "movae_adam_multi": ([_i, _p, _p, _p, _p, _p, _f, _f, _f, _f, _f, _i, _i, _p, _p], _i),
+    "movae_adam_multi_agg": ([_i, _p, _p, _p, _p, _p, _f, _f, _f, _f, _f, _i, _i, _p, _p, _z, _z, _i, _p, _p, _i, _i, _f, _f, _p, _i, _p,
+                              _p, _p], _i),
     "movae_clip_grad_norm_multi": ([_i, _p, _p, _f, _p, _p, _z, _p], _i),
     "movae_sumsq": ([_p, _z, _p, _p, _z, _p], _i),
     "movae_scale_by_clip": ([_p, _z, _p, _f, _p], _i),
diff --git a/mo-vae_amd/aggregation.py b/mo-vae_amd/aggregation.py
--- a/mo-vae_amd/aggregation.py
+++ b/mo-vae_amd/aggregation.py
@@ -80,6 +80,52 @@
         return gw(self.last_gramian)
 
 
+class PendingAggregation:
+
+    def __init__(self, J, part, n_blocks, norm_mode, norm_eps, reg_eps, pref):
+        self.J, self.part, self.n_blocks = J, part, n_blocks
+        self.norm_mode, self.norm_eps, self.reg_eps, self.pref = norm_mode, norm_eps, reg_eps, pref
+        k, m = J.shape
+        self.k, self.m, self.ldj = k, m, J.stride(0) if k > 1 else max(J.stride(0), m)
+        self.g = torch.empty(m, dtype=torch.float32, device=J.device)
+        self.w = torch.empty(k, dtype=torch.float32, device=J.device)
+        self.G = torch.empty((k, k), dtype=torch.float32, device=J.device)
+        self.offsets = {}
+        self.done = False
+
+    def finish(self):
+        if self.done:
+            return
+        self.done = True
+        ws = L.workspace(self.J.device)
+        L.call("movae_gram_upgrad", self.J.data_ptr(), self.ldj, self.k, self.m, self.G.data_ptr(), self.norm_mode, self.norm_eps,
+               self.reg_eps, L.ptr(self.pref), self.w.data_ptr(), 0, ws.data_ptr(), ws.numel(), _st(self.J))
+        L.call("movae_combine", self.J.data_ptr(), self.ldj, self.k, self.m, self.w.data_ptr(), self.g.data_ptr(), 0, _st(self.J))
+
+
+_PENDING = [None]
+
+
+def pending():
+    return _PENDING[0]
+
+
+def consumed(rec):
+    rec.done = True
+    if _PENDING[0] is rec:
+        _PENDING[0] = None
+
+
+def finish():
+    rec, _PENDING[0] = _PENDING[0], None
+    if rec is not None:
+        rec.finish()
+
+
+DEFER_MAX_K = 2
+DEFER_MAX_COLS = 1 << 22
+
+
 class GramianWeightedAggregator(tnn.Module):
     def __init__(self, gramian_weighting):
         super().__init__()
@@ -89,6 +135,31 @@
     def forward(self, J):
         w = self.weighting(J)
         return combine(J, w)
+
+    def unhooked(self):
+        return not any(mod._forward_hooks or mod._forward_pre_hooks for mod in (self, self.weighting, self.gramian_weighting))
+
+    def deferred(self, J):
+        gw = self.gramian_weighting
+        if type(gw) is not UPGradWeighting or gw.norm not in ("trace", "min_l2") or not FUSE_GRAM or not self.unhooked():
+            return None
+        _check_matrix(J)
+        k, m = J.shape
+        if k > DEFER_MAX_K or m > DEFER_MAX_COLS:
+            return None
+        finish()
+        import ctypes as C
+
+        nbytes = L.load().movae_gram_ws_bytes(k, m) - L.WS_HEADER_BYTES
+        part = torch.empty(nbytes, dtype=torch.uint8, device=J.device)
+        nb = C.c_int(0)
+        L.call("movae_gram_partials", J.data_ptr(), J.stride(0) if k > 1 else max(J.stride(0), m), k, m, part.data_ptr(), nbytes,
+               C.byref(nb), _st(J))
+        rec = PendingAggregation(J, part, nb.value, L.UPGRAD_NORM[gw.norm], float(gw.norm_eps), float(gw.reg_eps),
+                                 _pref_tensor(gw.pref_vector, J.device))
+        self.weighting.last_gramian = rec.G
+        _PENDING[0] = rec
+        return rec
 
 
 class UPGradWeighting(Weighting):
diff --git a/mo-vae_amd/autojac.py b/mo-vae_amd/autojac.py
--- a/mo-vae_amd/autojac.py
+++ b/mo-vae_amd/autojac.py
@@ -286,7 +286,18 @@
         ops.GRAD_SINK_ROWS = None
 
 
+DEFER_AGGREGATION = [False]
+
+
 def _aggregate_into_grads(jb, aggregator):
+    rec = None
+    if DEFER_AGGREGATION[0] and hasattr(aggregator, "deferred") and all(p.grad is None for p in jb.params):
+        rec = aggregator.deferred(jb.J)
+    if rec is not None:
+        for p, off in zip(jb.params, jb.offsets):
+            rec.offsets[id(p)] = off
+            p.grad = _view_like(rec.g[off: off + p.numel()], p)
+        return rec.g
     g = aggregator(jb.J)
     for p, off in zip(jb.params, jb.offsets):
         _accumulate(p, _view_like(g[off: off + p.numel()], p))
diff --git a/mo-vae_amd/csrc/agg.hip b/mo-vae_amd/csrc/agg.hip
--- a/mo-vae_amd/csrc/agg.hip
+++ b/mo-vae_amd/csrc/agg.hip
@@ -1,4 +1,5 @@
 #include "common.h"
+#include "agg_solve.h"
 #include <stdlib.h>
 
 namespace {
@@ -86,23 +87,25 @@
     if (VEC) {
         const long nv = m / 4;
         for (long c = (long)blockIdx.x * blockDim.x + threadIdx.x; c < nv; c += stride) {
-            f32x4 s = accumulate ? reinterpret_cast<const f32x4*>(g)[c] : f32x4{0.f, 0.f, 0.f, 0.f};
-#pragma unroll
-            for (int i = 0; i < K; ++i) s += wv[i] * reinterpret_cast<const f32x4*>(J + i * ldj)[c];
-            reinterpret_cast<f32x4*>(g)[c] = s;
+            const f32x4 s = accumulate ? reinterpret_cast<const f32x4*>(g)[c] : f32x4{0.f, 0.f, 0.f, 0.f};
+            f32x4 j[K];
+#pragma unroll
+            for (int i = 0; i < K; ++i) j[i] = reinterpret_cast<const f32x4*>(J + i * ldj)[c];
+            reinterpret_cast<f32x4*>(g)[c] = combine_fma<K>(s, wv, j);
         }
         if (blockIdx.x == 0 && threadIdx.x == 0)
             for (long c = nv * 4; c < m; ++c) {
-                float s = accumulate ? g[c] : 0.f;
-                for (int i = 0; i < K; ++i) s += wv[i] * J[i * ldj + c];
-                g[c] = s;
+                float j[K];
+#pragma unroll
+                for (int i = 0; i < K; ++i) j[i] = J[i * ldj + c];
+                g[c] = combine_pairs<K>(accumulate ? g[c] : 0.f, wv, j);
             }
     } else {
         for (long c = (long)blockIdx.x * blockDim.x + threadIdx.x; c < m; c += stride) {
-            float s = accumulate ? g[c] : 0.f;
-#pragma unroll
-            for (int i = 0; i < K; ++i) s += wv[i] * J[i * ldj + c];
-            g[c] = s;
+            float j[K];
+#pragma unroll
+            for (int i = 0; i < K; ++i) j[i] = J[i * ldj + c];
+            g[c] = combine_pairs<K>(accumulate ? g[c] : 0.f, wv, j);
         }
     }
 }
@@ -154,17 +157,7 @@
     const int lane = threadIdx.x;
     float Gin[K * K];
     if (gpart) {
-        constexpr int NP = K * (K + 1) / 2;
-        int q = 0;
-#pragma unroll
-        for (int i = 0; i < K; ++i)
-#pragma unroll
-            for (int j = i; j < K; ++j, ++q) {
-                double s = 0.0;
-                for (int b = lane; b < gnb; b += 64) s += gpart[(long)b * NP + q];
-                s = wave_sum(s);
-                Gin[i * K + j] = Gin[j * K + i] = (float)s;
-            }
+        gram_fold<K>(gpart, gnb, lane, Gin);
         if (lane == 0 && Gout)
 #pragma unroll
             for (int i = 0; i < K * K; ++i) Gout[i] = Gin[i];
@@ -172,134 +165,8 @@
 #pragma unroll
         for (int i = 0; i < K * K; ++i) Gin[i] = Gptr[i];
     }
-    double G[K][K];
-    if (norm_mode == 0) {
-        double tr = 0.0;
-#pragma unroll
-        for (int i = 0; i < K; ++i) tr += (double)Gin[i * K + i];
-        const bool zero = tr < (double)norm_eps;
-#pragma unroll
-        for (int i = 0; i < K; ++i)
-#pragma unroll
-            for (int j = 0; j < K; ++j) G[i][j] = zero ? 0.0 : (double)Gin[i * K + j] / tr;
-    } else {
-        float l2[K], sf[K];
-        float amin = 0.f;
-        bool any = false;
-#pragma unroll
-        for (int i = 0; i < K; ++i) {
-            l2[i] = sqrtf(fmaxf(Gin[i * K + i], norm_eps));
-            if (l2[i] > norm_eps && (!any || l2[i] < amin)) {
-                amin = l2[i];
-                any = true;
-            }
-        }
-#pragma unroll
-        for (int i = 0; i < K; ++i) sf[i] = (any && l2[i] > norm_eps) ? amin / l2[i] : 0.f;
-#pragma unroll
-        for (int i = 0; i < K; ++i)
-#pragma unroll
-            for (int j = 0; j < K; ++j) {
-                const float g = Gin[i * K + j];
-                G[i][j] = norm_mode == 1 ? (double)(g * (sf[i] * sf[j])) : (double)(g / (l2[i] * l2[j]));
-            }
-    }
-#pragma unroll
-    for (int i = 0; i < K; ++i) G[i][i] += (double)reg_eps;
-    double u[K], wsum[K];
-#pragma unroll
-    for (int i = 0; i < K; ++i) {
-        u[i] = pref ? (double)pref[i] : 1.0 / K;
-        wsum[i] = 0.0;
-    }
-    constexpr int nsub = 1 << K;
-    for (int row = 0; row < (dual ? 1 : K); ++row) {
-        double c[K];
-#pragma unroll
-        for (int i = 0; i < K; ++i) {
-            double acc = 0.0;
-#pragma unroll
-            for (int j = 0; j < K; ++j) acc += G[i][j] * ((dual || j == row) ? u[j] : 0.0);
-            c[i] = acc;
-        }
-        double best_viol = 1e300;
-        int best_mask = 0;
-        double best_v[K];
-#pragma unroll
-        for (int i = 0; i < K; ++i) best_v[i] = 0.0;
-        for (int mask = lane; mask < nsub; mask += 64) {
-            double L[K][K], y[K], v[K];
-            bool ok = true;
-#pragma unroll
-            for (int a = 0; a < K; ++a) {
-                const bool fa = mask >> a & 1;
-#pragma unroll
-                for (int b = 0; b <= a; ++b) {
-                    const bool fb = mask >> b & 1;
-                    double s = (fa && fb) ? G[a][b] : (a == b ? 1.0 : 0.0);
-#pragma unroll
-                    for (int q = 0; q < b; ++q) s -= L[a][q] * L[b][q];
-                    if (a == b) {
-                        if (s <= 0.0) {
-                            ok = false;
-                            s = 1.0;
-                        }
-                        L[a][a] = sqrt(s);
-                    } else {
-                        L[a][b] = s / L[b][b];
-                    }
-                }
-            }
-#pragma unroll
-            for (int a = 0; a < K; ++a) {
-                double s = (mask >> a & 1) ? -c[a] : 0.0;
-#pragma unroll
-                for (int q = 0; q < a; ++q) s -= L[a][q] * y[q];
-                y[a] = s / L[a][a];
-            }
-#pragma unroll
-            for (int a = K - 1; a >= 0; --a) {
-                double s = y[a];
-#pragma unroll
-                for (int q = a + 1; q < K; ++q) s -= L[q][a] * v[q];
-                v[a] = s / L[a][a];
-            }
-            double viol = ok ? 0.0 : 1e200;
-#pragma unroll
-            for (int i = 0; i < K; ++i) {
-                if (mask >> i & 1) {
-                    viol = fmax(viol, -v[i]);
-                } else {
-                    v[i] = 0.0;
-                    double gr = c[i];
-#pragma unroll
-                    for (int j = 0; j < K; ++j) gr += G[i][j] * ((mask >> j & 1) ? v[j] : 0.0);
-                    viol = fmax(viol, -gr);
-                }
-            }
-            if (viol < best_viol) {
-                best_viol = viol;
-                best_mask = mask;
-#pragma unroll
-                for (int i = 0; i < K; ++i) best_v[i] = v[i];
-            }
-        }
-        for (int o = 32; o > 0; o >>= 1) {
-            const double ov = __shfl_xor(best_viol, o, 64);
-            const int om = __shfl_xor(best_mask, o, 64);
-            double tmp[K];
-#pragma unroll
-            for (int i = 0; i < K; ++i) tmp[i] = __shfl_xor(best_v[i], o, 64);
-            if (ov < best_viol || (ov == best_viol && om < best_mask)) {
-                best_viol = ov;
-                best_mask = om;
-#pragma unroll
-                for (int i = 0; i < K; ++i) best_v[i] = tmp[i];
-            }
-        }
-#pragma unroll
-        for (int i = 0; i < K; ++i) wsum[i] += best_v[i] + ((dual || i == row) ? u[i] : 0.0);
-    }
+    double wsum[K];
+    upgrad_solve<K>(Gin, norm_mode, norm_eps, reg_eps, pref, dual, lane, wsum);
     if (lane == 0)
 #pragma unroll
         for (int i = 0; i < K; ++i) wout[i] = (float)wsum[i];
@@ -796,6 +663,23 @@
     return MOVAE_OK;
 }
 
+int movae_gram_partials(const float* J, size_t ldj, int k, size_t m, double* part, size_t part_bytes, int* n_blocks,
+                        movae_stream_t stream) {
+    MOVAE_CHECK_ARG(J && part && n_blocks && m > 0 && ldj >= m, "movae_gram_partials: bad argument");
+    MOVAE_CHECK_ARG(k >= 1 && k <= MAXK, "movae_gram_partials: k=%d outside 1..%d", k, MAXK);
+    const int nb = gram_blocks(m);
+    MOVAE_CHECK_ARG(part_bytes >= (size_t)nb * (size_t)(k * (k + 1) / 2) * sizeof(double), "movae_gram_partials: buffer too small");
+    hipStream_t st = (hipStream_t)stream;
+    const bool vec = (ldj % 4 == 0) && (reinterpret_cast<uintptr_t>(J) & 15) == 0;
+    int rc = MOVAE_EINVAL;
+#define CALL_GRAM(KK) launch_gram_k<KK>(J, ldj, m, part, nb, vec, st)
+    rc = [&]() -> int { DISPATCH_K(k, CALL_GRAM) return MOVAE_EINVAL; }();
+#undef CALL_GRAM
+    if (rc) return rc;
+    *n_blocks = nb;
+    return MOVAE_OK;
+}
+
 int movae_weights_dualproj(const float* G, int k, float norm_eps, float reg_eps, const float* pref, float* w, movae_stream_t stream) {
     MOVAE_CHECK_ARG(G && w, "movae_weights_dualproj: null pointer");
     MOVAE_CHECK_ARG(k >= 1 && k <= MAXK, "movae_weights_dualproj: k=%d outside 1..%d", k, MAXK);
diff --git a/mo-vae_amd/csrc/agg_solve.h b/mo-vae_amd/csrc/agg_solve.h
--- /dev/null
+++ b/mo-vae_amd/csrc/agg_solve.h
@@ -0,0 +1,175 @@
+#pragma once
+#include "common.h"
+
+template <int K>
+__device__ __forceinline__ void gram_fold(const double* __restrict__ gpart, int gnb, int lane, float (&Gin)[K * K]) {
+    constexpr int NP = K * (K + 1) / 2;
+    double s[NP];
+#pragma unroll
+    for (int q = 0; q < NP; ++q) s[q] = 0.0;
+#pragma unroll 2
+    for (int b = lane; b < gnb; b += 64)
+#pragma unroll
+        for (int q = 0; q < NP; ++q) s[q] += gpart[(long)b * NP + q];
+    int q = 0;
+#pragma unroll
+    for (int i = 0; i < K; ++i)
+#pragma unroll
+        for (int j = i; j < K; ++j, ++q) {
+            const double t = wave_sum(s[q]);
+            Gin[i * K + j] = Gin[j * K + i] = (float)t;
+        }
+}
+
+template <int K>
+__device__ __forceinline__ void upgrad_solve(const float (&Gin)[K * K], int norm_mode, float norm_eps, float reg_eps,
+                                             const float* __restrict__ pref, int dual, int lane, double (&wsum)[K]) {
+    double G[K][K];
+    if (norm_mode == 0) {
+        double tr = 0.0;
+#pragma unroll
+        for (int i = 0; i < K; ++i) tr += (double)Gin[i * K + i];
+        const bool zero = tr < (double)norm_eps;
+#pragma unroll
+        for (int i = 0; i < K; ++i)
+#pragma unroll
+            for (int j = 0; j < K; ++j) G[i][j] = zero ? 0.0 : (double)Gin[i * K + j] / tr;
+    } else {
+        float l2[K], sf[K];
+        float amin = 0.f;
+        bool any = false;
+#pragma unroll
+        for (int i = 0; i < K; ++i) {
+            l2[i] = sqrtf(fmaxf(Gin[i * K + i], norm_eps));
+            if (l2[i] > norm_eps && (!any || l2[i] < amin)) {
+                amin = l2[i];
+                any = true;
+            }
+        }
+#pragma unroll
+        for (int i = 0; i < K; ++i) sf[i] = (any && l2[i] > norm_eps) ? amin / l2[i] : 0.f;
+#pragma unroll
+        for (int i = 0; i < K; ++i)
+#pragma unroll
+            for (int j = 0; j < K; ++j) {
+                const float g = Gin[i * K + j];
+                G[i][j] = norm_mode == 1 ? (double)(g * (sf[i] * sf[j])) : (double)(g / (l2[i] * l2[j]));
+            }
+    }
+#pragma unroll
+    for (int i = 0; i < K; ++i) G[i][i] += (double)reg_eps;
+    double u[K];
+#pragma unroll
+    for (int i = 0; i < K; ++i) {
+        u[i] = pref ? (double)pref[i] : 1.0 / K;
+        wsum[i] = 0.0;
+    }
+    constexpr int nsub = 1 << K;
+    for (int row = 0; row < (dual ? 1 : K); ++row) {
+        double c[K];
+#pragma unroll
+        for (int i = 0; i < K; ++i) {
+            double acc = 0.0;
+#pragma unroll
+            for (int j = 0; j < K; ++j) acc += G[i][j] * ((dual || j == row) ? u[j] : 0.0);
+            c[i] = acc;
+        }
+        double best_viol = 1e300;
+        int best_mask = 0;
+        double best_v[K];
+#pragma unroll
+        for (int i = 0; i < K; ++i) best_v[i] = 0.0;
+        for (int mask = lane; mask < nsub; mask += 64) {
+            double L[K][K], y[K], v[K];
+            bool ok = true;
+#pragma unroll
+            for (int a = 0; a < K; ++a) {
+                const bool fa = mask >> a & 1;
+#pragma unroll
+                for (int b = 0; b <= a; ++b) {
+                    const bool fb = mask >> b & 1;
+                    double s = (fa && fb) ? G[a][b] : (a == b ? 1.0 : 0.0);
+#pragma unroll
+                    for (int q = 0; q < b; ++q) s -= L[a][q] * L[b][q];
+                    if (a == b) {
+                        if (s <= 0.0) {
+                            ok = false;
+                            s = 1.0;
+                        }
+                        L[a][a] = sqrt(s);
+                    } else {
+                        L[a][b] = s / L[b][b];
+                    }
+                }
+            }
+#pragma unroll
+            for (int a = 0; a < K; ++a) {
+                double s = (mask >> a & 1) ? -c[a] : 0.0;
+#pragma unroll
+                for (int q = 0; q < a; ++q) s -= L[a][q] * y[q];
+                y[a] = s / L[a][a];
+            }
+#pragma unroll
+            for (int a = K - 1; a >= 0; --a) {
+                double s = y[a];
+#pragma unroll
+                for (int q = a + 1; q < K; ++q) s -= L[q][a] * v[q];
+                v[a] = s / L[a][a];
+            }
+            double viol = ok ? 0.0 : 1e200;
+#pragma unroll
+            for (int i = 0; i < K; ++i) {
+                if (mask >> i & 1) {
+                    viol = fmax(viol, -v[i]);
+                } else {
+                    v[i] = 0.0;
+                    double gr = c[i];
+#pragma unroll
+                    for (int j = 0; j < K; ++j) gr += G[i][j] * ((mask >> j & 1) ? v[j] : 0.0);
+                    viol = fmax(viol, -gr);
+                }
+            }
+            if (viol < best_viol) {
+                best_viol = viol;
+                best_mask = mask;
+#pragma unroll
+                for (int i = 0; i < K; ++i) best_v[i] = v[i];
+            }
+        }
+        for (int o = 32; o > 0; o >>= 1) {
+            const double ov = __shfl_xor(best_viol, o, 64);
+            const int om = __shfl_xor(best_mask, o, 64);
+            double tmp[K];
+#pragma unroll
+            for (int i = 0; i < K; ++i) tmp[i] = __shfl_xor(best_v[i], o, 64);
+            if (ov < best_viol || (ov == best_viol && om < best_mask)) {
+                best_viol = ov;
+                best_mask = om;
+#pragma unroll
+                for (int i = 0; i < K; ++i) best_v[i] = tmp[i];
+            }
+        }
+#pragma unroll
+        for (int i = 0; i < K; ++i) wsum[i] += best_v[i] + ((dual || i == row) ? u[i] : 0.0);
+    }
+}
+
+template <int K, typename T>
+__device__ __forceinline__ T combine_fma(T s, const float (&w)[K], const T (&j)[K]) {
+#pragma unroll
+    for (int i = 0; i < K; ++i) s = __builtin_elementwise_fma((T)w[i], j[i], s);
+    return s;
+}
+template <int K>
+__device__ __forceinline__ float combine_pairs(float s, const float (&w)[K], const float (&j)[K]) {
+    if (K & 1) s = __builtin_fmaf(w[0], j[0], s);
+    {
+#pragma clang fp contract(off)
+#pragma unroll
+        for (int i = K & 1; i < K; ++i) {
+            const float p = w[i] * j[i];
+            s = s + p;
+        }
+    }
+    return s;
+}
diff --git a/mo-vae_amd/csrc/conv_thin.h b/mo-vae_amd/csrc/conv_thin.h
--- a/mo-vae_amd/csrc/conv_thin.h
+++ b/mo-vae_amd/csrc/conv_thin.h
@@ -1069,7 +1069,13 @@
                                                          float* __restrict__ slab, int Hw, int Ww, int Cw, int Ht, int Wt,
                                                          int stride, int pad, int TH, int TW, int tiles_h, int tiles_w,
                                                          int Cs, int Cb, long wide_gs, long thin_gs, long slab_gs, Norm nrm, int ntiles,
-                                                         FastDiv fd_tw, FastDiv fd_bw, int cs_on, long row_stride) {
+                                                         FastDiv fd_tw, FastDiv fd_bw, int cs_on, long row_stride, RSide sd, int gz) {
+    if ((int)blockIdx.z >= gz) {
+        extern __shared__ __attribute__((aligned(16))) float lds[];
+        const int bid = (((int)blockIdx.z - gz) * (int)gridDim.y + (int)blockIdx.y) * (int)gridDim.x + (int)blockIdx.x;
+        if (bid < sd.nblk) side_reduce(sd, bid, lds);
+        return;
+    }
     thin_wgrad_mfma_body<TC, KH, KW, REV>(Wide, Thin, slab, Hw, Ww, Cw, Ht, Wt, stride, pad, TH, TW, tiles_h, tiles_w, Cs, Cb, wide_gs,
                                           thin_gs, slab_gs, nrm, ntiles, fd_tw, fd_bw, cs_on, row_stride, blockIdx.x, blockIdx.y,
                                           blockIdx.z, gridDim.x);
@@ -1309,7 +1315,10 @@
             const size_t per1 = (size_t)row * sizeof(float);
             if (lds_bytes(TH, TW) <= 60 * 1024 && ntiles <= 0x7fffffffL && per1 * (size_t)nblk * G <= ws_bytes) {
                 float* slab = static_cast<float*>(ws);
-                const dim3 grid((unsigned)nblk, wide / 32, G);
+                dim3 grid((unsigned)nblk, wide / 32, G);
+                int gz = G;
+                RSide sd{};
+                if (use_mfma) sd = defer_take_3d(st, &grid, &gz);
                 const long slab_gs = (long)nblk * row;
                 const long wide_gs = thin_small ? b_gs : s_gs, thin_gs = thin_small ? s_gs : b_gs;
                 const size_t shb = (size_t)lds_bytes(TH, TW);
@@ -1333,7 +1342,7 @@
     do {                                                                                                                                               \
         hipLaunchKernelGGL((thin_wgrad_mfma_k<3, K, K, REVV>), grid, dim3(256), shb, st, Wd, Tn, slab, Hw, Ww, wide, Ht, Wt, g.stride,                 \
                            g.pad, TH, TW, tiles_h, tiles_w, g.Cs, g.Cb, wide_gs, thin_gs, slab_gs, wide_nrm, (int)ntiles, fastdiv_make(TW),            \
-                           fastdiv_make(thin_small ? TW + g.KW - 1 : (TW - 1) * g.stride + g.KW), cs_on ? 1 : 0, row);                                 \
+                           fastdiv_make(thin_small ? TW + g.KW - 1 : (TW - 1) * g.stride + g.KW), cs_on ? 1 : 0, row, sd, gz);                         \
         g_last_kernel = "thin_wgrad_mfma_k<3," #K "," #K "," #REVV ">";                                                                                \
     } while (0)
                 if (use_mfma) {
diff --git a/mo-vae_amd/csrc/optim.hip b/mo-vae_amd/csrc/optim.hip
--- a/mo-vae_amd/csrc/optim.hip
+++ b/mo-vae_amd/csrc/optim.hip
@@ -1,4 +1,5 @@
 #include "common.h"
+#include "agg_solve.h"
 
 namespace {
 
@@ -46,34 +47,49 @@
 
 __device__ unsigned g_adam_done = 0;
 
+__device__ __forceinline__ void adam_bias_corrections(float b1, float b2, float step_f, int wave, float* sh) {
+    if ((int)(threadIdx.x >> 6) == wave) {
+        const double step = (double)step_f;
+        const float c1 = (float)(1.0 - pow((double)b1, step));
+        const float c2 = (float)sqrt(1.0 - pow((double)b2, step));
+        if ((threadIdx.x & 63) == 0) sh[0] = c1, sh[1] = c2;
+    }
+}
+
 __global__ __launch_bounds__(256) void adam_multi_k(AdamTable tab, int cnt, float lr, float b1, float b2, float eps, float wd,
                                                     int decoupled, float bc1, float bc2_sqrt, float* __restrict__ hyper, int tick) {
+    __shared__ float sh_bc[2];
     int t = 0;
     while (t + 1 < cnt && blockIdx.x >= tab.first[t + 1]) ++t;
     const unsigned n = tab.n[t], base = (blockIdx.x - tab.first[t]) * ADAM_BLK;
     float step_f = 0.f;
     if (hyper) {
         step_f = hyper[0] + 1.f;
-        const double step = (double)step_f;
         lr = hyper[1];
-        bc1 = (float)(1.0 - pow((double)b1, step));
-        bc2_sqrt = (float)sqrt(1.0 - pow((double)b2, step));
-    }
-    const float step_size = lr / bc1;
+        adam_bias_corrections(b1, b2, step_f, 0, sh_bc);
+    }
     float* __restrict__ p = tab.p[t];
     const float* __restrict__ g = tab.g[t];
     float* __restrict__ m = tab.m[t];
     float* __restrict__ v = tab.v[t];
     const bool vec = ((reinterpret_cast<uintptr_t>(p) | reinterpret_cast<uintptr_t>(g) | reinterpret_cast<uintptr_t>(m) |
                        reinterpret_cast<uintptr_t>(v)) & 15) == 0;
-    if (vec && base + ADAM_BLK <= n) {
-        f32x4 pv[4], mv[4], vv[4], gv[4];
+    const bool whole = vec && base + ADAM_BLK <= n;
+    f32x4 pv[4], mv[4], vv[4], gv[4];
+    if (whole) {
 #pragma unroll
         for (int u = 0; u < 4; ++u) {
             const unsigned i = base + u * 1024u + threadIdx.x * 4;
             pv[u] = *reinterpret_cast<f32x4*>(p + i), mv[u] = *reinterpret_cast<f32x4*>(m + i), vv[u] = *reinterpret_cast<f32x4*>(v + i);
             gv[u] = *reinterpret_cast<const f32x4*>(g + i);
         }
+    }
+    if (hyper) {
+        __syncthreads();
+        bc1 = sh_bc[0], bc2_sqrt = sh_bc[1];
+    }
+    const float step_size = lr / bc1;
+    if (whole) {
 #pragma unroll
         for (int u = 0; u < 4; ++u) {
             const unsigned i = base + u * 1024u + threadIdx.x * 4;
@@ -109,6 +125,168 @@
                 float pj = p[k], mj = m[k], vj = v[k];
                 adam_one(pj, g[k], mj, vj, lr, b1, b2, eps, wd, decoupled, step_size, bc2_sqrt);
                 p[k] = pj; m[k] = mj; v[k] = vj;
+            }
+        }
+    }
+    if (hyper) {
+        __syncthreads();
+        if (threadIdx.x == 0) {
+            const unsigned done = atomicAdd(&g_adam_done, 1u);
+            if (done == gridDim.x - 1) {
+                g_adam_done = 0;
+                if (tick) hyper[0] = step_f;
+            }
+        }
+    }
+}
+
+struct AggOffsets {
+    long long off[ADAM_MT];
+};
+
+template <int K>
+__device__ __forceinline__ f32x4 agg_combine4(const float (&wv)[K], const f32x4 (&j4)[K], long long col, long fma_cols) {
+    if (col < fma_cols) return combine_fma<K>(f32x4{0.f, 0.f, 0.f, 0.f}, wv, j4);
+    f32x4 r;
+#pragma unroll
+    for (int e = 0; e < 4; ++e) {
+        float j1[K];
+#pragma unroll
+        for (int k = 0; k < K; ++k) j1[k] = j4[k][e];
+        r[e] = combine_pairs<K>(0.f, wv, j1);
+    }
+    return r;
+}
+
+template <int K>
+__global__ __launch_bounds__(256) void adam_agg_k(AdamTable tab, AggOffsets jo, int cnt, float lr, float b1, float b2, float eps, float wd,
+                                                  int decoupled, float bc1, float bc2_sqrt, float* __restrict__ hyper, int tick,
+                                                  const float* __restrict__ J, long ldj, long fma_cols,
+                                                  const double* __restrict__ gpart, int gnb,
+                                                  int norm_mode, float norm_eps, float reg_eps, const float* __restrict__ pref, int dual,
+                                                  float* __restrict__ wout, float* __restrict__ Gout) {
+    __shared__ float sh_bc[2];
+    __shared__ float sh_w[K];
+    int t = 0;
+    while (t + 1 < cnt && blockIdx.x >= tab.first[t + 1]) ++t;
+    const unsigned n = tab.n[t], base = (blockIdx.x - tab.first[t]) * ADAM_BLK;
+    const long long off = jo.off[t];
+    const bool jb = off >= 0;
+    const bool solve = jb || blockIdx.x == 0;
+    float step_f = 0.f;
+    if (hyper) {
+        step_f = hyper[0] + 1.f;
+        lr = hyper[1];
+    }
+    float* __restrict__ p = tab.p[t];
+    float* __restrict__ g = const_cast<float*>(tab.g[t]);
+    float* __restrict__ m = tab.m[t];
+    float* __restrict__ v = tab.v[t];
+    const float* __restrict__ Jt = jb ? J + off : nullptr;
+    const bool vec = ((reinterpret_cast<uintptr_t>(p) | reinterpret_cast<uintptr_t>(g) | reinterpret_cast<uintptr_t>(m) |
+                       reinterpret_cast<uintptr_t>(v)) & 15) == 0 &&
+                     (!jb || ((reinterpret_cast<uintptr_t>(Jt) & 15) == 0 && ldj % 4 == 0));
+    const bool whole = vec && base + ADAM_BLK <= n;
+    f32x4 pv[4], mv[4], vv[4], gv[4], jv[K][4];
+    if (whole) {
+#pragma unroll
+        for (int u = 0; u < 4; ++u) {
+            const unsigned i = base + u * 1024u + threadIdx.x * 4;
+            pv[u] = *reinterpret_cast<f32x4*>(p + i), mv[u] = *reinterpret_cast<f32x4*>(m + i), vv[u] = *reinterpret_cast<f32x4*>(v + i);
+            if (jb) {
+#pragma unroll
+                for (int k = 0; k < K; ++k) jv[k][u] = *reinterpret_cast<const f32x4*>(Jt + k * ldj + i);
+            } else {
+                gv[u] = *reinterpret_cast<const f32x4*>(g + i);
+            }
+        }
+    }
+    if (solve && threadIdx.x < 64) {
+        const int lane = threadIdx.x;
+        float Gin[K * K];
+        double wsum[K];
+        gram_fold<K>(gpart, gnb, lane, Gin);
+        upgrad_solve<K>(Gin, norm_mode, norm_eps, reg_eps, pref, dual, lane, wsum);
+        if (lane == 0) {
+#pragma unroll
+            for (int i = 0; i < K; ++i) sh_w[i] = (float)wsum[i];
+            if (blockIdx.x == 0) {
+#pragma unroll
+                for (int i = 0; i < K; ++i) wout[i] = (float)wsum[i];
+#pragma unroll
+                for (int i = 0; i < K * K; ++i) Gout[i] = Gin[i];
+            }
+        }
+    }
+    if (hyper) adam_bias_corrections(b1, b2, step_f, solve ? 1 : 0, sh_bc);
+    __syncthreads();
+    if (hyper) bc1 = sh_bc[0], bc2_sqrt = sh_bc[1];
+    float wv[K];
+#pragma unroll
+    for (int k = 0; k < K; ++k) wv[k] = jb ? sh_w[k] : 0.f;
+    const float step_size = lr / bc1;
+    if (whole) {
+#pragma unroll
+        for (int u = 0; u < 4; ++u) {
+            const unsigned i = base + u * 1024u + threadIdx.x * 4;
+            if (jb) {
+                f32x4 j4[K];
+#pragma unroll
+                for (int k = 0; k < K; ++k) j4[k] = jv[k][u];
+                gv[u] = agg_combine4<K>(wv, j4, off + i, fma_cols);
+                *reinterpret_cast<f32x4*>(g + i) = gv[u];
+            }
+#pragma unroll
+            for (int j = 0; j < 4; ++j) {
+                float pj = pv[u][j], mj = mv[u][j], vj = vv[u][j];
+                adam_one(pj, gv[u][j], mj, vj, lr, b1, b2, eps, wd, decoupled, step_size, bc2_sqrt);
+                pv[u][j] = pj; mv[u][j] = mj; vv[u][j] = vj;
+            }
+            *reinterpret_cast<f32x4*>(p + i) = pv[u];
+            *reinterpret_cast<f32x4*>(m + i) = mv[u];
+            *reinterpret_cast<f32x4*>(v + i) = vv[u];
+        }
+    } else
+    for (unsigned u = 0; u < 4; ++u) {
+        const unsigned i = base + u * 1024u + threadIdx.x * 4;
+        if (i >= n) break;
+        if (vec && i + 4 <= n) {
+            f32x4 p4 = *reinterpret_cast<f32x4*>(p + i), m4 = *reinterpret_cast<f32x4*>(m + i), v4 = *reinterpret_cast<f32x4*>(v + i);
+            f32x4 g4;
+            if (jb) {
+                f32x4 j4[K];
+#pragma unroll
+                for (int k = 0; k < K; ++k) j4[k] = *reinterpret_cast<const f32x4*>(Jt + k * ldj + i);
+                g4 = agg_combine4<K>(wv, j4, off + i, fma_cols);
+                *reinterpret_cast<f32x4*>(g + i) = g4;
+            } else {
+                g4 = *reinterpret_cast<const f32x4*>(g + i);
+            }
+#pragma unroll
+            for (int j = 0; j < 4; ++j) {
+                float pj = p4[j], mj = m4[j], vj = v4[j];
+                adam_one(pj, g4[j], mj, vj, lr, b1, b2, eps, wd, decoupled, step_size, bc2_sqrt);
+                p4[j] = pj; m4[j] = mj; v4[j] = vj;
+            }
+            *reinterpret_cast<f32x4*>(p + i) = p4;
+            *reinterpret_cast<f32x4*>(m + i) = m4;
+            *reinterpret_cast<f32x4*>(v + i) = v4;
+        } else {
+            const unsigned e = min(i + 4, n);
+            for (unsigned c = i; c < e; ++c) {
+                float gc;
+                if (jb) {
+                    float j1[K];
+#pragma unroll
+                    for (int k = 0; k < K; ++k) j1[k] = Jt[k * ldj + c];
+                    gc = off + c < fma_cols ? combine_fma<K>(0.f, wv, j1) : combine_pairs<K>(0.f, wv, j1);
+                    g[c] = gc;
+                } else {
+                    gc = g[c];
+                }
+                float pj = p[c], mj = m[c], vj = v[c];
+                adam_one(pj, gc, mj, vj, lr, b1, b2, eps, wd, decoupled, step_size, bc2_sqrt);
+                p[c] = pj; m[c] = mj; v[c] = vj;
             }
         }
     }
@@ -225,6 +403,66 @@
         hipLaunchKernelGGL(adam_multi_k, dim3(nblk), dim3(256), 0, (hipStream_t)stream, tab, cnt, lr, beta1, beta2, eps, weight_decay,
                            decoupled_wd, bc1, bc2_sqrt, hyper_dev, t0 + ADAM_MT >= n_tensors ? 1 : 0);
         MOVAE_CHECK_LAUNCH("adam_multi");
+    }
+    return MOVAE_OK;
+}
+
+int movae_adam_multi_agg(int n_tensors, float* const* p, float* const* g, float* const* m, float* const* v, const size_t* numel,
+                         float lr, float beta1, float beta2, float eps, float weight_decay, int decoupled_wd, int step,
+                         float* hyper_dev, const float* J, size_t ldj, size_t m_cols, int k, const long long* joff, const double* gram_part,
+                         int gram_blocks, int norm_mode, float norm_eps, float reg_eps, const float* pref, int dual, float* wout,
+                         float* Gout, movae_stream_t stream) {
+    MOVAE_CHECK_ARG(n_tensors >= 1 && p && g && m && v && numel && joff, "movae_adam_multi_agg: null table");
+    MOVAE_CHECK_ARG(hyper_dev || step >= 1, "movae_adam_multi_agg: step must be >= 1 when no device counter is given");
+    MOVAE_CHECK_ARG(J && gram_part && gram_blocks >= 1 && wout && Gout && k >= 1 && m_cols > 0 && ldj >= m_cols,
+                    "movae_adam_multi_agg: bad aggregation argument");
+    MOVAE_CHECK_ARG(norm_mode >= 0 && norm_mode <= 2, "movae_adam_multi_agg: unknown normalisation %d", norm_mode);
+    if (k > 4) {
+        movae_set_error("movae_adam_multi_agg: k=%d; the in-launch solve is built for k <= 4 (use movae_gram_upgrad, movae_combine "
+                        "and movae_adam_multi)", k);
+        return MOVAE_EUNSUPPORTED;
+    }
+    for (int i = 0; i < n_tensors; ++i) {
+        MOVAE_CHECK_ARG(p[i] && g[i] && m[i] && v[i], "movae_adam_multi_agg: null tensor");
+        MOVAE_CHECK_ARG(numel[i] > 0 && numel[i] < 0xffffffffUL, "movae_adam_multi_agg: tensor size out of range");
+        MOVAE_CHECK_ARG(joff[i] < 0 || (size_t)joff[i] + numel[i] <= m_cols, "movae_adam_multi_agg: tensor %d leaves its Jacobian row", i);
+    }
+    float bc1 = 1.f, bc2_sqrt = 1.f;
+    if (!hyper_dev) {
+        bc1 = (float)(1.0 - pow((double)beta1, step));
+        bc2_sqrt = (float)sqrt(1.0 - pow((double)beta2, step));
+    }
+    const long fma_cols = (ldj % 4 == 0 && (reinterpret_cast<uintptr_t>(J) & 15) == 0) ? (long)(m_cols / 4 * 4) : 0;
+    for (int t0 = 0; t0 < n_tensors; t0 += ADAM_MT) {
+        AdamTable tab;
+        AggOffsets jo;
+        const int cnt = n_tensors - t0 < ADAM_MT ? n_tensors - t0 : ADAM_MT;
+        unsigned nblk = 0;
+        for (int i = 0; i < cnt; ++i) {
+            tab.p[i] = p[t0 + i]; tab.g[i] = g[t0 + i]; tab.m[i] = m[t0 + i]; tab.v[i] = v[t0 + i];
+            tab.n[i] = (unsigned)numel[t0 + i];
+            tab.first[i] = nblk;
+            jo.off[i] = joff[t0 + i];
+            nblk += (unsigned)((numel[t0 + i] + ADAM_BLK - 1) / ADAM_BLK);
+        }
+        for (int i = cnt; i < ADAM_MT; ++i) {
+            tab.p[i] = nullptr; tab.g[i] = nullptr; tab.m[i] = nullptr; tab.v[i] = nullptr; tab.n[i] = 0;
+            jo.off[i] = -1;
+        }
+        for (int i = cnt; i <= ADAM_MT; ++i) tab.first[i] = nblk;
+        const int tick = t0 + ADAM_MT >= n_tensors ? 1 : 0;
+#define MOVAE_ADAM_AGG(KV)                                                                                                        \
+    hipLaunchKernelGGL((adam_agg_k<KV>), dim3(nblk), dim3(256), 0, (hipStream_t)stream, tab, jo, cnt, lr, beta1, beta2, eps,          \
+                       weight_decay, decoupled_wd, bc1, bc2_sqrt, hyper_dev, tick, J, (long)ldj, fma_cols, gram_part, gram_blocks, norm_mode, \
+                       norm_eps, reg_eps, pref, dual ? 1 : 0, wout, Gout)
+        switch (k) {
+            case 1: MOVAE_ADAM_AGG(1); break;
+            case 2: MOVAE_ADAM_AGG(2); break;
+            case 3: MOVAE_ADAM_AGG(3); break;
+            default: MOVAE_ADAM_AGG(4); break;
+        }
+#undef MOVAE_ADAM_AGG
+        MOVAE_CHECK_LAUNCH("adam_agg");
     }
     return MOVAE_OK;
 }
diff --git a/mo-vae_amd/optim.py b/mo-vae_amd/optim.py
--- a/mo-vae_amd/optim.py
+++ b/mo-vae_amd/optim.py
@@ -3,6 +3,7 @@
 import torch
 
 from . import _lib as L
+from . import aggregation as _agg
 
 
 def _dense(t):
@@ -38,12 +39,39 @@
                 h[1].fill_(float(group["lr"]))
                 self._hyper_lr[gi] = float(group["lr"])
 
+    def _takes(self, rec):
+        if len(self.param_groups) != 1:
+            return False
+        live = [p for p in self.param_groups[0]["params"] if p.grad is not None]
+        if not live or not all(p.dtype == torch.float32 and _dense(p) for p in live):
+            return False
+        ids = {id(p): p for p in live}
+        for pid, off in rec.offsets.items():
+            p = ids.get(pid)
+            if p is None or p.grad.data_ptr() != rec.g.data_ptr() + 4 * off or p.grad.dtype != p.dtype or _layout_differs(p.grad, p):
+                return False
+        if not self._device_step:
+            return len({int(self.state[p]["step"]) if len(self.state[p]) else 0 for p in live}) == 1
+        return True
+
+    def zero_grad(self, set_to_none=True):
+        _agg.finish()
+        return super().zero_grad(set_to_none=set_to_none)
+
+    def state_dict(self):
+        _agg.finish()
+        return super().state_dict()
+
     @torch.no_grad()
     def step(self, closure=None):
         loss = None
         if closure is not None:
             with torch.enable_grad():
                 loss = closure()
+        rec = _agg.pending()
+        if rec is not None and not self._takes(rec):
+            _agg.finish()
+            rec = None
         for gi, group in enumerate(self.param_groups):
             if group.get("amsgrad") or group.get("maximize"):
                 raise NotImplementedError("FusedAdam: amsgrad / maximize are not part of the reference's configuration")
@@ -96,9 +124,18 @@
                 dev = rows[0][0].device
                 if self._device_step and not torch.cuda.is_current_stream_capturing():
                     self.sync_hyper()
-                L.call("movae_adam_multi", n, ps, gs, ms, vs, ns, float(group["lr"]), float(beta1), float(beta2),
-                       float(group["eps"]), float(group["weight_decay"]), 1 if self._decoupled else 0,
-                       max(1, key), L.ptr(hyper) if self._device_step else 0, L.stream_ptr(dev))
+                adam = (n, ps, gs, ms, vs, ns, float(group["lr"]), float(beta1), float(beta2), float(group["eps"]),
+                        float(group["weight_decay"]), 1 if self._decoupled else 0, max(1, key), L.ptr(hyper) if self._device_step else 0)
+                if rec is not None and len(buckets) == 1:
+                    joff = (C.c_longlong * n)(*[rec.offsets.get(id(r[0]), -1) for r in rows])
+                    L.call("movae_adam_multi_agg", *adam, rec.J.data_ptr(), rec.ldj, rec.m, rec.k, joff, rec.part.data_ptr(), rec.n_blocks,
+                           rec.norm_mode, rec.norm_eps, rec.reg_eps, L.ptr(rec.pref), 0, rec.w.data_ptr(), rec.G.data_ptr(),
+                           L.stream_ptr(dev))
+                    _agg.consumed(rec)
+                    rec = None
+                    continue
+                _agg.finish()
+                L.call("movae_adam_multi", *adam, L.stream_ptr(dev))
         return loss
 
 
@@ -114,6 +151,7 @@
         raise NotImplementedError("clip_grad_norm_: only the L2 norm of the reference's call is implemented")
     if isinstance(parameters, torch.Tensor):
         parameters = [parameters]
+    _agg.finish()
     grads = [p.grad for p in parameters if p.grad is not None]
     if not grads:
         return torch.tensor(0.0)
diff --git a/mo-vae_amd/parallel.py b/mo-vae_amd/parallel.py
--- a/mo-vae_amd/parallel.py
+++ b/mo-vae_amd/parallel.py
@@ -5,6 +5,9 @@
 
 
 def flatten_grads(params, out=None):
+    from . import aggregation
+
+    aggregation.finish()
     chunks = []
     for p in params:
         if p.grad is None:
diff --git a/mo-vae_amd/train.py b/mo-vae_amd/train.py
--- a/mo-vae_amd/train.py
+++ b/mo-vae_amd/train.py
@@ -97,8 +97,17 @@
     return loss_dict, outputs
 
 
+def fused_tail_ok(optimizer, aggregator, args, dp=None):
+    return (type(aggregator) in (aggregation.UPGrad, aggregation.NUPGrad) and aggregator.unhooked()
+            and isinstance(optimizer, FusedAdam) and dp is None and getattr(args, "max_grad_norm", None) is None)
+
+
 def train_step(net, images, optimizer, aggregator, args, dp=None):
-    loss_dict, outputs = forward_backward(net, images, optimizer, aggregator)
+    autojac.DEFER_AGGREGATION[0] = fused_tail_ok(optimizer, aggregator, args, dp)
+    try:
+        loss_dict, outputs = forward_backward(net, images, optimizer, aggregator)
+    finally:
+        autojac.DEFER_AGGREGATION[0] = False
     if dp is not None:
         dp.all_reduce_grads()
     if getattr(args, "max_grad_norm", None) is not None:
```

Measured after the change: 341,400 (median of 6 runs). +1.9%, better.
